# YaqiangCao/cLoops

Hardware: AMD Instinct MI355X
Metric: PETs clustered/sec (whole node) + wall-clock for mode-3 eps x minPts sweep (higher is better)
Workload: dtype int32; 1 GPU; synthetic-200M-23chr-mode3 (BASELINE.json configs[3]); variant=cDBSCAN2, pets=200000000, chromosomes=23, chained_cut=True, final_cut=3871, candidate_loops=3651369, parallelism=23 chromosomes LPT-sharded over 1 GPU(s)

## Files before the change

### cloops_amd/_lib.py

```python
import ctypes
import os

_HERE = os.path.dirname(os.path.abspath(__file__))
SO_PATH = os.path.join(_HERE, "libcloops_hip.so")

CL_OK = 0
CL_ERR_ARG = -1
CL_ERR_HIP = -2
CL_ERR_EMPTY = -3
CL_ERR_DOMAIN = -4
CL_ERR_GRID = -5
CL_ERR_NODEVICE = -6
CL_ERR_HASH = -7
CL_ERR_PARSE = -8

VARIANT_CDBSCAN1 = 1
VARIANT_CDBSCAN2 = 2
VARIANT_BLOCK = 3

CL_TRACK_WASHU, CL_TRACK_JUICE = 0, 1
CL_TRACK_NAME_MAX = 64
CL_CONV_HICPRO, CL_CONV_JUICER, CL_CONV_PAIRS = 0, 1, 2
CL_CONV_E_FIELDS, CL_CONV_E_INT, CL_CONV_E_RANGE, CL_CONV_E_LONG = 1, 2, 3, 4
CL_INGEST_TIMES = 6
CL_INGEST_BEDPE, CL_INGEST_PAIRS = 0, 1
DIST_LOGBINS = 3840
CL_KDE_MAX_GRID = 1024
CL_KDIS_KMAX = 64
CL_KDIS_BINS = 3968
CL_MAT_WMAX = 8192
CL_MAT_CELLS_MAX = 16777216
CL_BAL_BINS_MAX = 16777216
CL_EIG_MAX = 6
CL_EIG_BLOCK = 8
CL_EIG_BINS_MAX = 1048576


class ClBox(ctypes.Structure):
    _fields_ = [("min_x", ctypes.c_int32), ("max_x", ctypes.c_int32), ("min_y", ctypes.c_int32),
                ("max_y", ctypes.c_int32), ("count", ctypes.c_int32)]


class ClTiming(ctypes.Structure):
    _fields_ = [("ms_keys", ctypes.c_float), ("ms_sort", ctypes.c_float), ("ms_region", ctypes.c_float),
                ("ms_union", ctypes.c_float), ("ms_border", ctypes.c_float), ("ms_table", ctypes.c_float),
                ("ms_d2h", ctypes.c_float), ("ms_total", ctypes.c_float), ("n_in", ctypes.c_int64),
                ("n_strips", ctypes.c_int64), ("ms_bracket", ctypes.c_float), ("ms_band", ctypes.c_float),
                ("n_queried", ctypes.c_int64)]


class ClIngestName(ctypes.Structure):
    _fields_ = [("hash", ctypes.c_uint64), ("first", ctypes.c_uint32), ("off", ctypes.c_uint32), ("len", ctypes.c_uint32),
                ("pad", ctypes.c_uint32)]


class ClDsummary(ctypes.Structure):
    _fields_ = [("n_all", ctypes.c_int64 * 2), ("n_pos", ctypes.c_int64 * 2), ("sumx", ctypes.c_double * 2),
                ("sumxx", ctypes.c_double * 2), ("xshift", ctypes.c_double), ("loghist", ctypes.c_uint64 * DIST_LOGBINS),
                ("fine_lo", ctypes.c_int64), ("fine", ctypes.c_uint64 * 2048)]


_int, _i32, _u32, _i64, _vp, _cp = ctypes.c_int, ctypes.c_int32, ctypes.c_uint32, ctypes.c_int64, ctypes.c_void_p, ctypes.c_char_p
_i32p, _i64p, _u64p, _f32p, _vpp = (ctypes.POINTER(t) for t in (_i32, _i64, ctypes.c_uint64, ctypes.c_float, _vp))
_f64, _f64p = ctypes.c_double, ctypes.POINTER(ctypes.c_double)

PROTOTYPES = {
    "cl_last_error": (_cp, []),
    "cl_device_count": (_int, []),
    "cl_version": (_int, []),
    "cl_chrom_create": (_int, [_int, _vp, _vp, _vp, _i64, _int, _vpp]),
    "cl_chrom_destroy": (None, [_vp]),
    "cl_chrom_size": (_i64, [_vp]),
    "cl_chrom_subsample": (_int, [_vp, _vp, _i64, _vpp]),
    "cl_chrom_set_stream": (_int, [_vp, _vp]),
    "cl_chrom_drop_indexes": (_int, [_vp]),
    "cl_cluster": (_int, [_vp, _int, _i32, _i32, _i32, _vp, _i32p, _i32p]),
    "cl_cluster_weighted": (_int, [_vp, _i32, _i32, _i32, _i32, _vp, _i32p, _i32p]),
    "cl_cluster_async": (_int, [_vp, _int, _i32, _i32, _i32, _vp]),
    "cl_cluster_pairs_async": (_int, [_vp, _int, _i32, _i32, _i32, _vp, _i64]),
    "cl_cluster_rowmask_async": (_int, [_vp, _int, _i32, _i32, _i32, _vp, _i64]),
    "cl_cluster_step_async": (_int, [_vp, _int, _i32, _i32, _i32, _i32, _i64]),
    "cl_wait": (_int, [_vp, _i32p, _i32p]),
    "cl_step_result": (_int, [_vp, _i64p, _i64p, ctypes.POINTER(ClDsummary)]),
    "cl_set_pairs_defer": (None, [_vp, _int]),
    "cl_pairs_sync": (_int, [_vp]),
    "cl_last_n_labelled": (_i64, [_vp]),
    "cl_last_n_in": (_i64, [_vp]),
    "cl_last_region_mode": (_int, [_vp]),
    "cl_get_boxes": (_int, [_vp, _vp]),
    "cl_boxes_host": (_vp, [_vp]),
    "cl_labels_device": (_vp, [_vp]),
    "cl_neighbor_counts": (_int, [_vp, _i32, _i32, _vp]),
    "cl_dist_summary": (_int, [_vp, _i32, ctypes.POINTER(ClDsummary)]),
    "cl_dist_bin_hist": (_int, [_vp, _i32, _u32, _u32, _int, _u64p]),
    "cl_dist_collect": (_int, [_vp, _i32, _i64p, _i64p, _i64p]),
    "cl_dist_kde": (_int, [_vp, _int, _f64, _f64, _f64, _int, _f64p]),
    "cl_kde_array": (_int, [_int, _vp, _i64, _f64, _f64, _f64, _int, _f64p]),
    "cl_sig_counts": (_int, [_vp, _i32, _i32, _vp, _vp, _i64p]),
    "cl_quant_counts": (_int, [_vp, _i32, _i32, _vp, _vp, _i64p]),
    "cl_contact_hist": (_int, [_vp, _i32, _i32, _i64, _vp, _vp, _i64p, _i64p, _i64p, _i32p]),
    "cl_anchor_mask": (_int, [_vp, _i64, _vp, _vp, _vp, _i64p, _i64p]),
    "cl_agg_loops": (_int, [_vp, _i32, _i32, _i32, _i32, _i64, _vp, _vp, _vp, _vp, _vp, _i64p]),
    "cl_track_build": (_int, [_vp, _i32, _i64, _i64, _vp, _cp, _cp, _i64p, _i64p]),
    "cl_track_chunks": (_int, [_vp, _i64, _i64, _vp, _vp, _i64p]),
    "cl_track_render": (_int, [_vp, _i64, _vp, _i64, _i64p]),
    "cl_track_free": (_int, [_vp]),
    "cl_cov_build": (_int, [_vp, _i64, _i32, _i64, _i64, _i64p, ctypes.POINTER(_u32), _i64p, _i64p]),
    "cl_cov_runs": (_int, [_vp, _i64, _i64, _vp, _vp, _vp]),
    "cl_cov_text": (_int, [_vp, _cp, _i64, _i64, _i64p]),
    "cl_cov_chunks": (_int, [_vp, _i64, _i64, _vp, _vp, _i64p]),
    "cl_cov_render": (_int, [_vp, _i64, _vp, _i64, _i64p]),
    "cl_cov_free": (_int, [_vp]),
    "cl_peak_sort": (_int, [_vp, _i64, _i32, _i64p, _i64p, _i64p]),
    "cl_peak_call": (_int, [_vp, _i64, _i64, _i64p, _i64p, _i64p]),
    "cl_peak_get": (_int, [_vp, _i64, _i64, _vp, _vp, _vp, _vp]),
    "cl_peak_count": (_int, [_vp, _vp, _vp, _i64, _vp]),
    "cl_peak_summits": (_int, [_vp, _vp, _vp, _i64, _i64, _vp, _vp]),
    "cl_peak_free": (_int, [_vp]),
    "cl_dom_tracks": (_int, [_vp, _i64, _i64, _i64, _i64p, _i64p, _i64p]),
    "cl_dom_get": (_int, [_vp, _i64, _i64, _vp, _vp, _vp]),
    "cl_dom_count": (_int, [_vp, _vp, _vp, _i64, _vp, _vp, _vp]),
    "cl_dom_free": (_int, [_vp]),
    "cl_kdis_build": (_int, [_vp, _i64, _vp, _i32, _i64p]),
    "cl_kdis_get": (_int, [_vp, _i32, _i64, _i64, _vp, _vp, _vp]),
    "cl_kdis_hist": (_int, [_vp, _i32, _vp, _u64p, _u64p]),
    "cl_kdis_free": (_int, [_vp]),
    "cl_mat_window": (_int, [_vp, _i64, _i64, _i64, _i64, _i64, _i64, _i32, _vp, _i64p, _i64p]),
    "cl_mat_cells": (_int, [_vp, _i64, _i64, _i32, _i64p, _i64p, _i64p]),
    "cl_mat_cells_get": (_int, [_vp, _i64, _i64, _vp, _vp, _vp]),
    "cl_mat_v4c": (_int, [_vp, _i64, _i64, _i64, _i64, _i64, _i64, _vp, _i64p, _i64p, _i64p]),
    "cl_mat_free": (_int, [_vp]),
    "cl_bal_marginals": (_int, [_vp, _i32, _i64p, _i64p, _i64p]),
    "cl_bal_marginals_get": (_int, [_vp, _i64, _i64, _vp, _vp]),
    "cl_bal_iterate": (_int, [_vp, _vp, _i32, _f64, _i32p, _i32p, _f64p, _f64p]),
    "cl_bal_weights_get": (_int, [_vp, _i64, _i64, _vp]),
    "cl_bal_cells_get": (_int, [_vp, _i64, _i64, _vp]),
    "cl_bal_free": (_int, [_vp]),
    "cl_exp_diagonals": (_int, [_vp, _vp, _i32, _i64p, _i64p]),
    "cl_exp_diagonals_get": (_int, [_vp, _i64, _i64, _vp, _vp, _vp]),
    "cl_exp_set": (_int, [_vp, _vp, _i64]),
    "cl_exp_cells_get": (_int, [_vp, _i64, _i64, _vp]),
    "cl_exp_free": (_int, [_vp]),
    "cl_eig_build": (_int, [_vp, _f64, _i64, _i64p, _i64p]),
    "cl_eig_apply": (_int, [_vp, _vp, _i32, _vp]),
    "cl_eig_iterate": (_int, [_vp, _i32, _i32, _f64, _i32p, _i32p, _vp, _vp]),
    "cl_eig_vectors_get": (_int, [_vp, _i32, _i64, _i64, _vp]),
    "cl_eig_free": (_int, [_vp]),
    "cl_conv_create": (_int, [_int, _vp, _i32, _i64, _i64, _vpp]),
    "cl_conv_feed": (_int, [_vp, _vp, _i64, _i32, _i64p, _i64p, _i64p]),
    "cl_conv_render": (_int, [_vp, _vp, _i64, _i64p]),
    "cl_conv_error": (_int, [_vp, _i64p, _i32p]),
    "cl_conv_timing": (_int, [_vp, _f32p]),
    "cl_conv_destroy": (_int, [_vp]),
    "cl_ingest_create": (_int, [_int, _vp, _i64, _i64, _i32, _vpp]),
    "cl_ingest_set_format": (_int, [_vp, _i32, _i64]),
    "cl_ingest_feed": (_int, [_vp, _vp, _i64, _i64p, _i64p, _i64p]),
    "cl_ingest_error": (_int, [_vp, _i64p, _i32p]),
    "cl_ingest_headers": (_int, [_vp, _i64p]),
    "cl_ingest_names": (_int, [_vp, _vp, _i64, _i64p]),
    "cl_ingest_commit": (_int, [_vp, _i64, _i64, _vp, _vp, _vp, _vp, _i32, _vp, _i64, _i32, _vp, _i32p]),
    "cl_ingest_finish": (_int, [_vp, _vp, _i32, _i32, _vp, _i64p]),
    "cl_ingest_rows": (_int, [_vp, _i32, _vp, _vp, _i64]),
    "cl_ingest_chrom_arrays": (_int, [_vp, _i32, _i64p, _vpp, _vpp]),
    "cl_ingest_distances": (_int, [_vp, _vp, _i64]),
    "cl_ingest_timing": (_int, [_vp, _f32p]),
    "cl_ingest_destroy": (_int, [_vp]),
    "cl_cand_reset": (_int, [_vp]),
    "cl_cand_append": (_int, [_vp, _i32, _i64p, _i64p]),
    "cl_cand_finish": (_int, [_vp, _i32, _vp, _i64, _i64p]),
    "cl_cand_finish_device": (_int, [_vp, _i32, _vpp, _i64p]),
    "cl_set_table_export": (None, [_vp, _int]),
    "cl_set_device_labels": (None, [_vp, _int]),
    "cl_set_profiling": (None, [_vp, _int]),
    "cl_get_timing": (_int, [_vp, ctypes.POINTER(ClTiming)]),
    "cl_sweep_plan": (_int, [_vp, _i32p, _i32, _i32p, _i32]),
    "cl_set_layout_reuse": (None, [_vp, _int]),
    "cl_set_sort_index": (None, [_vp, _int]),
    "cl_set_count_reuse": (None, [_vp, _int]),
    "cl_set_count_floor": (None, [_vp, _i32]),
    "cl_set_count_thresholds": (None, [_vp, _i32p, _i32]),
    "cl_set_eps_list": (None, [_vp, _i32p, _i32]),
    "cl_set_traversal": (None, [_vp, _int]),
    "cl_stream_create": (_vp, [_int]),
    "cl_stream_destroy": (None, [_vp]),
    "cl_host_alloc": (_vp, [_i64]),
    "cl_host_free": (None, [_vp]),
    "cl_debug_arena_overcommit": (None, [_i64]),
}
SYMBOLS = list(PROTOTYPES)


def bind(lib, table):
    for name, (restype, argtypes) in table.items():
        fn = getattr(lib, name)
        fn.restype, fn.argtypes = restype, argtypes
    return lib


class CloopsHipError(RuntimeError):
    def __init__(self, code, msg):
        RuntimeError.__init__(self, "libcloops_hip error %d: %s" % (code, msg))
        self.code = code


_lib = None


def load():
    global _lib
    if _lib is not None:
        return _lib
    path = SO_PATH
    if os.environ.get("CLOOPS_DEVEL_LIB") == "1":
        path = SO_PATH.replace(".so", "_devel.so")
    if not os.path.exists(path):
        raise ImportError(
            "libcloops_hip.so is missing (%s). Build it with `python -m cloops_amd.build` "
            "(needs hipcc); there is no CPU fallback." % path)
    _lib = bind(ctypes.CDLL(path), PROTOTYPES)
    return _lib


def check(rc):
    if rc != CL_OK:
        msg = load().cl_last_error()
        raise CloopsHipError(rc, msg.decode() if msg else "")


def host_alloc(nbytes):
    p = load().cl_host_alloc(int(nbytes))
    if not p:
        raise MemoryError("no page-locked host memory of %d bytes" % nbytes)
    return p


def stream_create(device):
    s = load().cl_stream_create(int(device))
    if not s:
        raise CloopsHipError(CL_ERR_HIP, (load().cl_last_error() or b"").decode())
    return s
```

### cloops_amd/api.py

```python
import ctypes
import math
import os

import numpy as np

from . import _lib

VARIANTS = {"v1": _lib.VARIANT_CDBSCAN1, "cDBSCAN": _lib.VARIANT_CDBSCAN1, 1: 1,
            "v2": _lib.VARIANT_CDBSCAN2, "cDBSCAN2": _lib.VARIANT_CDBSCAN2, 2: 2,
            "block": _lib.VARIANT_BLOCK, "blockDBSCAN": _lib.VARIANT_BLOCK, 3: 3}

BOX_DTYPE = np.dtype([("min_x", "<i4"), ("max_x", "<i4"), ("min_y", "<i4"), ("max_y", "<i4"), ("count", "<i4")])


TRAVERSAL_OVERRIDE = int(os.environ["CLOOPS_TRAVERSAL"]) if os.environ.get("CLOOPS_TRAVERSAL", "") != "" else None


def device_count():
    return _lib.load().cl_device_count()


def _vp(a):
    return a.ctypes.data_as(ctypes.c_void_p)

# ... 28 lines not shown

    def _open(self, create, *args):
        self._lib = _lib.load()
        self._h = ctypes.c_void_p()
        _lib.check(getattr(self._lib, create)(*args, ctypes.byref(self._h)))

    def close(self):
        if getattr(self, "_h", None) is not None and self._h.value:
            getattr(self._lib, self._DESTROY)(self._h)
            self._h = ctypes.c_void_p()

    def __del__(self):
        try:
            self.close()
        except Exception:
            pass


class Chromosome(_Handle):
    _DESTROY = "cl_chrom_destroy"

    def __init__(self, X, Y, device=0, stream=None):
        X = _as_i32(X, "X")
        Y = _as_i32(Y, "Y")
        if X.shape != Y.shape:
            raise ValueError("X and Y differ in length")
        self._create(X.shape[0], device, "cl_chrom_create", int(device), ctypes.c_void_p(stream), X.ctypes.data_as(ctypes.c_void_p),
                     Y.ctypes.data_as(ctypes.c_void_p), int(X.shape[0]), 0)

    def _create(self, n, device, create, *args):
        self.n = int(n)
        self.device = device
        self._profiling = False
        self._pins = {}
        self._inflight = []
        self._enq = 0
        self._open(create, *args)
        if TRAVERSAL_OVERRIDE is not None:
            self._lib.cl_set_traversal(self._h, int(TRAVERSAL_OVERRIDE))

    @classmethod
    def from_device_pointers(cls, x_ptr, y_ptr, n, device=0, stream=None, keepalive=None):
        self = cls.__new__(cls)
        self._keepalive = keepalive
        self._create(n, device, "cl_chrom_create", int(device), ctypes.c_void_p(stream), ctypes.c_void_p(x_ptr), ctypes.c_void_p(y_ptr),
                     int(n), 1)
        return self

    def subsample(self, rows):
        rows = np.ascontiguousarray(rows, dtype=np.int64)
        new = Chromosome.__new__(Chromosome)
        new._create(rows.shape[0], self.device, "cl_chrom_subsample", self._h, rows.ctypes.data_as(ctypes.c_void_p), int(rows.shape[0]))
        return new

    def close(self):
        _Handle.close(self)
        pins, self._pins = getattr(self, "_pins", {}), {}
        for p, _ in pins.values():
            self._lib.cl_host_free(ctypes.c_void_p(p))

    def _pin(self, kind, slot, nbytes, shape=None):
        e = self._pins.get((kind, slot))
        if e is None:
            p = _lib.host_alloc(nbytes)
            view = None if shape is None else np.ctypeslib.as_array(ctypes.cast(p, ctypes.POINTER(ctypes.c_int32)), shape=shape)
            e = self._pins[kind, slot] = (p, view)
        return e

    def _pinned_labels(self, which=0):
        return self._pin("labels", which, max(4, self.n * 4), (self.n,))[1]

    def set_profiling(self, on=True):
        self._profiling = bool(on)
        self._lib.cl_set_profiling(self._h, 1 if on else 0)

    def set_device_labels(self, on=True):
        self._lib.cl_set_device_labels(self._h, 1 if on else 0)

    def set_table_export(self, on=True):
        if getattr(self, "_export", True) != bool(on):
            self._lib.cl_set_table_export(self._h, 1 if on else 0)
            self._export = bool(on)

    def cand_reset(self):
        _lib.check(self._lib.cl_cand_reset(self._h))

    def cand_append(self, step):
        ni, ns = ctypes.c_int64(0), ctypes.c_int64(0)
        _lib.check(self._lib.cl_cand_append(self._h, int(step), ctypes.byref(ni), ctypes.byref(ns)))
        return int(ni.value), int(ns.value)

    def step_async(self, variant, eps, minPts, cut, step, fine_lo=-1):
        _lib.check(self._lib.cl_cluster_step_async(self._h, VARIANTS[variant], int(eps), int(minPts), int(cut), int(step), int(fine_lo)))
        self._export = False
        self._inflight.append((None, False))
        self._enq += 1

    def step_result(self):
        ni, ns = ctypes.c_int64(0), ctypes.c_int64(0)
        st = _lib.ClDsummary()
        _lib.check(self._lib.cl_step_result(self._h, ctypes.byref(ni), ctypes.byref(ns), ctypes.byref(st)))
        return int(ni.value), int(ns.value), self._summary_dict(st)

    def cand_finish(self, final_cut, capacity):
        buf = getattr(self, "_cand_buf", None)
        if buf is None or len(buf) < capacity:
            buf = self._cand_buf = np.zeros((max(int(capacity) + int(capacity) // 4, 1), 4), dtype=np.int32)
        k = ctypes.c_int64(0)
        _lib.check(self._lib.cl_cand_finish(self._h, int(final_cut), buf.ctypes.data_as(ctypes.c_void_p), int(capacity), ctypes.byref(k)))
        return buf[: int(k.value)].copy()

    def cand_finish_device(self, final_cut):
        ptr, k = ctypes.c_void_p(), ctypes.c_int64(0)
        _lib.check(self._lib.cl_cand_finish_device(self._h, int(final_cut), ctypes.byref(ptr), ctypes.byref(k)))
        return (ptr.value or 0), int(k.value)

    def set_sort_index(self, mode=1):
        self._lib.cl_set_sort_index(self._h, int(mode))

    def set_count_reuse(self, on=True):
        self._lib.cl_set_count_reuse(self._h, 1 if on else 0)

    def sweep_plan(self, eps_list, min_pts_list):
        ev = sorted(set(int(e) for e in eps_list))
        mv = sorted(set(int(m) for m in min_pts_list))
        ea = (ctypes.c_int32 * max(len(ev), 1))(*ev)
        ma = (ctypes.c_int32 * max(len(mv), 1))(*mv)
        _lib.check(self._lib.cl_sweep_plan(self._h, ea, len(ev), ma, len(mv)))

    def drop_indexes(self):
        _lib.check(self._lib.cl_chrom_drop_indexes(self._h))

    def set_traversal(self, level=4):
        self._lib.cl_set_traversal(self._h, int(level))

    def set_count_floor(self, min_pts):
        self._lib.cl_set_count_floor(self._h, int(min_pts))

    def set_count_thresholds(self, min_pts_list):
        vals = [int(m) for m in min_pts_list]
        arr = (ctypes.c_int32 * max(1, len(vals)))(*vals)
        self._lib.cl_set_count_thresholds(self._h, arr, len(vals))

    def set_stream(self, stream):
        _lib.check(self._lib.cl_chrom_set_stream(self._h, ctypes.c_void_p(stream)))

    def set_eps_list(self, eps_list):
        vals = [int(e) for e in eps_list]
        arr = (ctypes.c_int32 * max(1, len(vals)))(*vals)
        self._lib.cl_set_eps_list(self._h, arr, len(vals))

    def last_region_mode(self):
        return int(self._lib.cl_last_region_mode(self._h))

    def set_layout_reuse(self, on=True):
        self._lib.cl_set_layout_reuse(self._h, 1 if on else 0)

    def timing(self):
        t = _lib.ClTiming()
        _lib.check(self._lib.cl_get_timing(self._h, ctypes.byref(t)))
        return {k: getattr(t, k) for k, _ in _lib.ClTiming._fields_}

    def _boxes(self, max_label, copy):
        k = max_label + 1
        if k <= 0:
            return np.zeros(0, dtype=BOX_DTYPE)
        ptr = self._lib.cl_boxes_host(self._h)
        if not ptr:
            raise _lib.CloopsHipError(_lib.CL_ERR_ARG, "the last run has no exported cluster table")
        view = np.ctypeslib.as_array(ctypes.cast(ptr, ctypes.POINTER(ctypes.c_int32)), shape=(k * 5,)).view(BOX_DTYPE)
        return view.copy() if copy else view

    def cluster_async(self, variant, eps, minPts, cut=0, want_labels=True, want_boxes=True):
        v = VARIANTS[variant]
        self.set_table_export(want_boxes)
        labels = self._pinned_labels(self._enq & 1) if want_labels else None
        _lib.check(self._lib.cl_cluster_async(self._h, v, int(eps), int(minPts), int(cut),
                                              labels.ctypes.data_as(ctypes.c_void_p) if want_labels else None))
        self._inflight.append((labels, bool(want_boxes)))
        self._enq += 1

    def cluster_pairs_async(self, variant, eps, minPts, cut=0, want_boxes=True):
        v = VARIANTS[variant]
        self.set_table_export(want_boxes)
        buf = self._pin("pairs", self._enq & 1, max(8, self.n * 8), (self.n, 2))[1]
        _lib.check(self._lib.cl_cluster_pairs_async(self._h, v, int(eps), int(minPts), int(cut), buf.ctypes.data_as(ctypes.c_void_p), self.n))
        self._inflight.append((buf, bool(want_boxes)))
        self._enq += 1

    def wait_pairs(self, copy=False, defer=False):
        buf, exported = self._inflight.pop(0)
        nc, ml = ctypes.c_int32(0), ctypes.c_int32(-1)
        self._lib.cl_set_pairs_defer(self._h, 1 if defer else 0)
        _lib.check(self._lib.cl_wait(self._h, ctypes.byref(nc), ctypes.byref(ml)))
        k = int(self._lib.cl_last_n_labelled(self._h))
        pairs = buf[:k].copy() if copy else buf[:k]
        boxes = self._boxes(ml.value, copy) if exported else None
        return ClusterResult(None, nc.value, ml.value, boxes, self.timing() if self._profiling else None), pairs

    def pairs_sync(self):
        _lib.check(self._lib.cl_pairs_sync(self._h))

    def cluster_rowmask_async(self, variant, eps, minPts, cut=0, want_boxes=True):
        v = VARIANTS[variant]
        self.set_table_export(want_boxes)
        p = self._pin("rowmask", self._enq & 1, 8 * ((self.n + 63) // 64) + 4 * max(self.n, 1))[0]
        _lib.check(self._lib.cl_cluster_rowmask_async(self._h, v, int(eps), int(minPts), int(cut), ctypes.c_void_p(p), max(self.n, 1)))
        self._inflight.append((p, bool(want_boxes)))
        self._enq += 1

    def wait_rowmask(self, copy=False, defer=False):
        p, exported = self._inflight.pop(0)
        nc, ml = ctypes.c_int32(0), ctypes.c_int32(-1)
        self._lib.cl_set_pairs_defer(self._h, 1 if defer else 0)
        _lib.check(self._lib.cl_wait(self._h, ctypes.byref(nc), ctypes.byref(ml)))
        k = int(self._lib.cl_last_n_labelled(self._h))
        nw = (self.n + 63) // 64
        mask = np.ctypeslib.as_array(ctypes.cast(p, ctypes.POINTER(ctypes.c_uint64)), shape=(nw,))
        labels = np.ctypeslib.as_array(ctypes.cast(p + 8 * nw, ctypes.POINTER(ctypes.c_int32)), shape=(max(k, 1),))[:k]
        if copy:
            mask, labels = mask.copy(), labels.copy()
        boxes = self._boxes(ml.value, copy) if exported else None
        return ClusterResult(None, nc.value, ml.value, boxes, self.timing() if self._profiling else None), mask, labels

    def rows_of_mask(self, mask):
        bits = np.unpackbits(np.ascontiguousarray(mask).view(np.uint8), bitorder="little")[: self.n]
        return np.flatnonzero(bits)

    def wait(self, copy=False):
        labels, exported = self._inflight.pop(0)
        nc = ctypes.c_int32(0)
        ml = ctypes.c_int32(-1)
        _lib.check(self._lib.cl_wait(self._h, ctypes.byref(nc), ctypes.byref(ml)))
        boxes = self._boxes(ml.value, copy) if exported else None
        if labels is not None and copy:
            labels = labels.copy()
        return ClusterResult(labels, nc.value, ml.value, boxes, self.timing() if self._profiling else None)

    def cluster(self, variant, eps, minPts, cut=0, want_labels=True, want_boxes=True, pinned=False):
        v = VARIANTS[variant]
        if self._inflight:
            raise RuntimeError("asynchronous runs in flight: call wait() first")
        self.set_table_export(True)
        if want_labels:
            labels = self._pinned_labels(0) if pinned else np.empty(self.n, dtype=np.int32)
        else:
            labels = None
        nc = ctypes.c_int32(0)
        ml = ctypes.c_int32(-1)
        lp = labels.ctypes.data_as(ctypes.c_void_p) if want_labels else None
        _lib.check(self._lib.cl_cluster(self._h, v, int(eps), int(minPts), int(cut), lp,
                                        ctypes.byref(nc), ctypes.byref(ml)))
        boxes = self._boxes(ml.value, copy=not pinned) if want_boxes else None
        return ClusterResult(labels, nc.value, ml.value, boxes, self.timing() if self._profiling else None)

    def cluster_weighted(self, eps, minPts, wx=1, wy=1):
        if self._inflight:
            raise RuntimeError("asynchronous runs in flight: call wait() first")
        self.set_table_export(True)
        labels = np.empty(self.n, dtype=np.int32)
        nc = ctypes.c_int32(0)
        ml = ctypes.c_int32(-1)
        _lib.check(self._lib.cl_cluster_weighted(self._h, int(eps), int(minPts), int(wx), int(wy),
                                                 labels.ctypes.data_as(ctypes.c_void_p), ctypes.byref(nc), ctypes.byref(ml)))
        return ClusterResult(labels, nc.value, ml.value, self._boxes(ml.value, copy=True), self.timing() if self._profiling else None)

    def last_n_in(self):
        return int(self._lib.cl_last_n_in(self._h))

    def dist_summary(self, cut=0):
        st = _lib.ClDsummary()
        _lib.check(self._lib.cl_dist_summary(self._h, int(cut), ctypes.byref(st)))
        return self._summary_dict(st)

    @staticmethod
    def _summary_dict(st):
        return {"n_all": [int(st.n_all[0]), int(st.n_all[1])], "n_pos": [int(st.n_pos[0]), int(st.n_pos[1])],
                "sumx": [float(st.sumx[0]), float(st.sumx[1])], "sumxx": [float(st.sumxx[0]), float(st.sumxx[1])],
                "xshift": float(st.xshift), "loghist": np.ctypeslib.as_array(st.loghist).astype(np.int64),
                "fine_lo": int(st.fine_lo), "fine": np.ctypeslib.as_array(st.fine).astype(np.int64) if st.fine_lo >= 0 else None}

    def dist_bin_hist(self, cut, lo, hi, shift):
        out = np.zeros(2048, dtype=np.uint64)
        _lib.check(self._lib.cl_dist_bin_hist(self._h, int(cut), int(lo), int(hi), int(shift),
                                              out.ctypes.data_as(ctypes.POINTER(ctypes.c_uint64))))
        return out.astype(np.int64)

    def dist_collect(self, cut=0):
        out = [(ctypes.c_int64 * 2)() for _ in range(3)]
        _lib.check(self._lib.cl_dist_collect(self._h, int(cut), *out))
        return {k: [int(a[0]), int(a[1])] for k, a in zip(("n_pos", "dmin", "dmax"), out)}

    def dist_kde(self, group, lo, step, inv_h, gridsize):
        out = np.zeros(max(int(gridsize), 1), dtype=np.float64)
        _lib.check(self._lib.cl_dist_kde(self._h, int(group), float(lo), float(step), float(inv_h), int(gridsize),
                                         out.ctypes.data_as(ctypes.POINTER(ctypes.c_double))))
        return out

    def sig_counts(self, windows, cut=0):
        w = np.ascontiguousarray(windows, dtype=np.int32).reshape(-1, 44)
        out = np.zeros((len(w), 144), dtype=np.int32)
        npets = ctypes.c_int64(0)
        _lib.check(self._lib.cl_sig_counts(self._h, int(cut), len(w), w.ctypes.data_as(ctypes.c_void_p),
                                           out.ctypes.data_as(ctypes.c_void_p), ctypes.byref(npets)))
        return out, int(npets.value)

# ... 552 lines not shown
```

### cloops_amd/csrc/cl_chrom.h

```cpp
#pragma once
#include "cl_common.h"
#include "cl_table.h"
#include "cl_prim.h"
#include "cl_textout.h"

#define BIGTPB 1024
#define AGG_H 512
__device__ __forceinline__ int agg_slot(int* keys, int key)
{
    unsigned h = ((unsigned)key * 2654435761u) >> 23;
    for (int probe = 0; probe < 24; ++probe) {
        const int old = atomicCAS(&keys[h], -1, key);
        if (old == -1 || old == key) return (int)h;
        h = (h + 1) & (AGG_H - 1);
    }
    return -1;
}
#define FLAT_PER 4
struct Stats { int amin, amax, vmin, vmax, xmin, xmax, ymin, ymax; };
__device__ __forceinline__ int je_minus(const int* __restrict__ cstart, int j) { return cstart[j + 1] - cstart[j]; }
static inline int bits_for(unsigned v) { int b = 0; while (v) { ++b; v >>= 1; } return b; }


#define CL_FINE_KMAX 8
#define K7_BLOCKS 2048
#define K7_STEP_BLOCKS 256
#define K7_STEP_THREADS 1024
#define K7_LOGBINS 3840
__device__ __forceinline__ int k7_logbin(unsigned d)
{
    const int e = 31 - __clz((int)d);
    const unsigned m = e >= 7 ? ((d >> (e - 7)) & 127u) : ((d << (7 - e)) & 127u);
    return e * 128 + (int)m;
}
#define K7_FINE 2048
#define K7_XSHIFT 11.0
#define CAND_BLOCK 2048

struct K7Src {
    int sorted;
    int n; int M; int v0;
    const int* dM;
    const int* X; const int* Y; const int* labels;
    const int* sv; const int* slab;
    const int* dh;
};

struct K7Part { double sx[2]; double sxx[2]; long long n_all[2]; long long n_pos[2]; };

struct RunRequest {
    int variant = CL_VARIANT_CDBSCAN1, eps = 0, minPts = 0, cut = 0;
    int32_t* labels_out = nullptr;
    int2* pairs_out = nullptr;
    long long pairs_cap = 0;
    void* mask_out = nullptr;
    long long mask_cap = 0;
    int step = -1;
    long long fine_lo = -1;
    int wx = 0, wy = 0;
};

struct cl_chrom {
    long long tmp_n = -1;
    DevBuf arena;
    int device = 0;
    hipStream_t stream = nullptr;
    bool own_stream = false;
    int64_t n = 0;
    int *d_x = nullptr, *d_y = nullptr;
    bool own_xy = false;
    Stats st{};
    DevBuf keys_in, keys_out, vals_in, vals_out, sort_tmp, scan_tmp;
    DevBuf qb_key, qb_val;
    int qindex_layout = -1;
    struct Fine {
        DevBuf q, sp, row, strip;
        int w = 0;
        int valid_w = 0, layout = -1;
        GridParams g;
        void invalidate() { valid_w = 0; layout = -1; }
    } fine;
    int sort_index_mode = 0;
    long long n_sorts = 0;
    DevBuf sv, sa, strip, cnt, parent, root, head, headidx, cellfirst, compkey, ncore, bsize, owner, state;
    DevBuf flag, rankscan, ulist, lo, hi, recs, counters, chainflag, chainhead, usize, b_cstart, b_ckey, b_nb, b_cx, b_cy, tile_s0;
    int* h_pinned = nullptr;
    struct StripPlan { int layout, eps, maxlen; };
    std::vector<StripPlan> plans;
    struct Run {
        u32* srow = nullptr;
        int *sv = nullptr, *sa = nullptr, *strip = nullptr, *tile = nullptr;
        int* cnt = nullptr;
        WordSrc ws{};
        int init_nclr = 0;
        int level = 0;
        const int* dM = nullptr;
        int m = 0;
        bool m_exact = false;
        bool rows = true;
        bool l4_make_base = false;
        bool l4_cut = false;
        bool l4_band = false;
        bool k2_make = false;
        const int* k_total = nullptr;
        bool hdr_packed = false;
    } run;
    struct Base {
        DevBuf q, sp, row, strip, tile, key;
        bool valid = false; int layout = -1, eps = 0;
        bool key_valid = false;
        void invalidate() { valid = false; key_valid = false; }
    } base;
    DevBuf sel_tmp;
    struct Counts {
        bool valid = false;
        bool cut_on_base = false;
        bool base_space = false;
        int layout = -1, eps = 0, thr = 0 , cap = 0;
        u32 tmask[4] = {0, 0, 0, 0};
        DevBuf cnt, pre, poff, dpre, D, blen;
        void invalidate() { valid = false; }
    } rc;
    bool reuse_counts = true;
    int count_floor = 0;
    u32 count_tmask[4] = {0, 0, 0, 0};
    DevBuf blk_tmp;
    DevBuf rootlist, cflag8;
    DevBuf l_mask, l_rank, l_blk, l_cstrip, l_wpos, l_wenc, l_dist, l_aux;
    DevBuf l_tab, l_fix;
    bool pairs_defer = false, pairs_copy_pending = false;
    bool fuse_chains = true;
    bool l_sup_dirty = false;
    GridParams dbg_g{}; int dbg_nm = 0;
    int traversal = 4;
    int last_k2_mode = 0;
    std::vector<long long> dcum;
    DevBuf dhist;
    long long n_neg = 0;
    bool reuse_layout = true;
    struct Slot {
        DevBuf labels, table;
        bool pending = false;
        int n_strips = 0;
        hipEvent_t ev_done = nullptr, ev_copied = nullptr;
        hipEvent_t ev[10]{};
        bool band_timed = false;
        long long n_queried = 0;
        int* h_hdr = nullptr;
        cl_box* h_boxes = nullptr;
        size_t h_boxes_cap = 0;
        int32_t* labels_out = nullptr;
        DevBuf slab;
        DevBuf pairs;
        int2* pairs_host = nullptr;
        long long pairs_host_cap = 0;
        void* mask_host = nullptr;
        long long mask_host_cap = 0;
        bool exported = true;
        bool step_valid = false;
        bool host_written = false;
        bool wait_done = false;
        long long fine_lo = -1;
        int kmax = 0;
        DevBuf d_step;
        char* h_step = nullptr;
        bool rows_valid = false;
        bool sorted_src = false;
        const int* k7_sv = nullptr;
        const int* k7_lcnt = nullptr;
        int k7_v0 = 0;
    } slot[2];
    bool device_labels = true;
    bool export_table = true;
    struct Cand { DevBuf box, step, keep, out; long long n = 0, cap = 0; } cand;
    DevBuf hdr;
    DevBuf k7_cls, k7_parts;
    struct Kde {
        DevBuf ent, sorted, ctr, tmp, part;
        int run = -1;
        long long cap = 0, cnt[2] = {0, 0};
    } kde;
    struct Sig { DevBuf tx, ty, tmp, sorttmp, m, win, out; bool ready = false; int cut = 0; } sig;
    struct Fp { DevBuf small, keys, sorted, tmp, pairs; } fp;
    struct Anchor { DevBuf s, e, dir, mask, wsum; } an;
    struct Agg {
        DevBuf kin, vin, sx, sy, tmp, m, cx, cy, lkin, lkout, lvin, order, ltmp, sum, stats, mats;
        bool ready = false; int cut = 0, kept = 0;
    } ag;
    struct Track {
        DevBuf tcnt, toff, row, keys, sorted, tmp, ids, names;
        TextOut txt;
        struct State {
            bool built = false, ids = false;
            int kind = 0, la = 0, lb = 0, gbits = 0;
            long long cut = 0, ext = 0;
        } st;
    } tk;
    struct Cov {
        DevBuf kin, key, tmp, dcur, dprev, xr, flag, scan, ctr, start, end, depth, name;
        TextOut txt;
        struct State {
            bool built = false, text = false;
            int la = 0;
            long long R = 0, num = 0, den = 0;
        } st;
    } cv;
    struct Peak {
        DevBuf kin, key, tmp, lo, hi, flag, C, head, H, a, b, start, end, np, nc, ctr, ivs, ive, best, opos, ocnt;
        struct State {
            bool sorted = false, called = false;
            int base = 0;
            long long m = 0, P = 0;
        } st;
    } pk;
    struct Dom {
        DevBuf diff, trk, tmp, rng, ivs, ive, cnt;
        struct State {
            bool ready = false;
            int cut = 0, res = 0, w = 0;
            int pmin = 0, pmax = 0;
            long long bmin = 0, n_bins = 0, n_kept = 0;
        } st;
    } dm;
    struct Kdis {
        DevBuf x, y, d, hist;
        struct State {
            bool ready = false;
            int cut = 0, n_k = 0;
            int ks[8] = {0, 0, 0, 0, 0, 0, 0, 0};
            long long n_kept = 0;
        } st;
    } kd;
    struct Mat {
        DevBuf out, ctr, key, sorted, tmp, flag, scan, start, bx, by, cnt;
        struct State {
            bool ready = false;
            long long n_cells = 0, n_kept = 0, max_count = 0;
            int res = 0; bool fold = false;
        } st;
    } mx;
    struct Bal {
        DevBuf kin, kout, vin, vout, tmp, tby, tbx, tcnt, sum, nnz, valid, w, s, icar, dcar, part, rec, out;
        struct State {
            bool ready = false, iterated = false;
            int ignore_diags = 0;
            long long b0 = 0, nb = 0, n_used = 0, n_cells = 0;
        } st;
    } bl;
    struct Exp {
        DevBuf valid, w, mask, kin, kout, vin, vout, tmp, dk, dx, dc, car, ctr, pairs, cnt, val, exp, out;
        struct State {
            bool ready = false, expected = false;
            int balanced = 0;
            long long nd = 0, n_used = 0;
        } st;
    } ex;
    struct Eig {
        DevBuf val, rows, pl, tot, ctr, q, part, sm, vec, io, ax;
        struct State {
            bool built = false, iterated = false;
            double clip = 0.0;
            long long dmax = 0, n_valid = 0, n_in = 0;
            int n_eigs = 0;
        } st;
    } eg;
    bool k7_classified = false;
    hipStream_t copy_stream = nullptr, aux_stream = nullptr;
    int copy_mode = 0;
    hipStream_t shared_copy = nullptr;
    int enq = 0, deq = 0;
    int cur = 0;
    int last_slot = -1;
    int last_K = 0;
    bool have_result = false;
    long long refused_labelled = -1;
    bool profiling = false;
    cl_timing timing{};
    bool ev_ready = false;
    float ev_bracket_ms = 0.f;
};


#define LAUNCH(kernel, nthreads, ...) \
    hipLaunchKernelGGL(kernel, dim3(nblocks(nthreads)), dim3(TPB), 0, c->stream, __VA_ARGS__)

static inline void run_begin(cl_chrom* c) { c->run = cl_chrom::Run(); }

struct RunGuard {
    cl_chrom* c; bool armed = true;
    explicit RunGuard(cl_chrom* cc) : c(cc) {}
    ~RunGuard()
    {
        if (!armed) return;
        c->rc.invalidate();
        c->l_sup_dirty = true;
        if (c->counters.p) (void)hipMemsetAsync(c->counters.as<int>() + CTR_TICKET_A, 0, 8, c->stream);
        (void)hipGetLastError();
    }
};

static inline bool range_ok(int64_t first, int64_t count, int64_t size)
{
    return first >= 0 && count >= 0 && first <= size && count <= size - first;
}
struct CopyOut { void* dst; const void* src; size_t bytes; };
static inline int read_back(cl_chrom* c, const char* who, std::initializer_list<CopyOut> parts)
{
    hipError_t e = hipSuccess;
    for (const CopyOut& p : parts)
        if (e == hipSuccess) e = hipMemcpyAsync(p.dst, p.src, p.bytes, hipMemcpyDeviceToHost, c->stream);
    const hipError_t e2 = hipStreamSynchronize(c->stream);
    if (e != hipSuccess || e2 != hipSuccess) return fail_at(CL_ERR_HIP, who, "copy", hipGetErrorString(e != hipSuccess ? e : e2));
    return CL_OK;
}

int ensure_workspace(cl_chrom* c, int S);
int ensure_events(cl_chrom* c);
void ev_record(cl_chrom* c, int k);
int ensure_cand_capacity(cl_chrom* c, long long need);
Table make_table_slot(cl_chrom* c, int slot);
Table make_table(cl_chrom* c);
const int* k7_hist_for(cl_chrom* c, int cut);
int finish_enqueue(cl_chrom* c, const RunRequest& req, int n_strips, const int* d_M);
static inline void track_release(cl_chrom* c) { c->tk = cl_chrom::Track(); }
static inline void cov_release(cl_chrom* c) { c->cv = cl_chrom::Cov(); }
static inline void peak_release(cl_chrom* c) { c->pk = cl_chrom::Peak(); }
static inline void dom_release(cl_chrom* c) { c->dm = cl_chrom::Dom(); }
static inline void kdis_release(cl_chrom* c) { c->kd = cl_chrom::Kdis(); }
static inline void eig_release(cl_chrom* c) { c->eg = cl_chrom::Eig(); }
static inline void exp_release(cl_chrom* c) { eig_release(c); c->ex = cl_chrom::Exp(); }
static inline void bal_release(cl_chrom* c) { exp_release(c); c->bl = cl_chrom::Bal(); }
static inline void mat_release(cl_chrom* c) { c->mx = cl_chrom::Mat(); bal_release(c); }
static inline int unit_free(cl_chrom* c, const char* who, void (*release)(cl_chrom*))
{
    if (!c) return fail(CL_ERR_ARG, "null chromosome handle");
    if (c->enq != c->deq) return fail(CL_ERR_ARG, who, "asynchronous runs still in flight");
    HIP_TRY(hipSetDevice(c->device));
    HIP_TRY(hipStreamSynchronize(c->stream));
    release(c);
    return CL_OK;
}
int run_block(cl_chrom* c, const RunRequest& req);
int run_weighted(cl_chrom* c, const RunRequest& req);

__global__ void k_init_table(Table t, const int* __restrict__ rankscan, int n);
__global__ void k_init_arrays(int n, int* __restrict__ parent, int* __restrict__ compkey, int* __restrict__ ncore,
                              int* __restrict__ bsize, int* __restrict__ usize, int* __restrict__ cellfirst,
                              int* __restrict__ flag, int* __restrict__ state, int* __restrict__ counters);
__global__ void k_strip_table(const u64* __restrict__ skeys, int n, int S, int shift, int* __restrict__ strip_start);
__global__ void k_root_labels(GridParams g, const int* __restrict__ strip_start, const int* __restrict__ root,
                              const int* __restrict__ compkey, const int* __restrict__ ncore, const int* __restrict__ bsize,
                              const int* __restrict__ state, const int* __restrict__ rankscan, int* __restrict__ rlabel);
__global__ void k_rank_flags(GridParams g, const int* __restrict__ strip_start, const int* __restrict__ root,
                             const int* __restrict__ compkey, const int* __restrict__ state, int* __restrict__ flag);
__global__ void __launch_bounds__(BIGTPB)
k_flatten(GridParams g, const int* __restrict__ strip_start, const int* __restrict__ cnt,
          const int* __restrict__ chainid, int* parent, const u32* __restrict__ srow,
          const int* __restrict__ head, const int* __restrict__ cellfirst,
          int* __restrict__ root, int* __restrict__ compkey, int* __restrict__ ncore,
          int* __restrict__ rootlist , int* __restrict__ counters);

struct Rec { int pt; int r[4]; };
#define OWNER_CONTESTED 0x40000000
__device__ __forceinline__ int owner_root(int o) { return o < 0 ? -1 : (o & (OWNER_CONTESTED - 1)); }

struct ListRun {
    int npos;
    const int* pstrip;
    const int* lcnt;
    const unsigned long long* cmask; const unsigned long long* wmask;
    const int* cgrank; const int* wgrank;
    int2* cpair; int* cpos; int* ckey; int2* wpair; int* wpos; int* wenc; int* cstrip;
};
int lists_build(cl_chrom* c, const GridParams& g, int nm, ListRun* out);
int lists_build_base(cl_chrom* c, const GridParams& g, int nm, ListRun* out);
int lists_base_keys(cl_chrom* c, const GridParams& g);
int lists_words_to_base(cl_chrom* c, const GridParams& g);
int lists_union_flatten(cl_chrom* c, const GridParams& g, int nm, const ListRun& L);
int lists_scatter_root(cl_chrom* c, int nm, const ListRun& L);
int lists_border(cl_chrom* c, const GridParams& g, int nm, const ListRun& L);
int lists_emit_records(cl_chrom* c, const GridParams& g, int nm, const ListRun& L);
int lists_scatter_owner(cl_chrom* c, int nm, const ListRun& L);
int lists_final(cl_chrom* c, const RunRequest& req, const GridParams& g, int nm, const ListRun& L, bool rows, int* pair_count);
int lists_rowmask(cl_chrom* c, const RunRequest& req, int* total);

__global__ void __launch_bounds__(256)
k_step_classify_count(const int* __restrict__ dK, Table t, signed char* __restrict__ cls, int* __restrict__ bcount, int nb,
                      unsigned long long* __restrict__ zero, int nzero);
__global__ void __launch_bounds__(256)
k_cand_append(const int* __restrict__ dK, const signed char* __restrict__ cls, Table t, const int* __restrict__ boff ,
              const int* __restrict__ bcount, int base, int step, int cap, int4* __restrict__ cbox, int* __restrict__ cstep);
__global__ void __launch_bounds__(TPB)
k7_summary(K7Src s, int cut, const signed char* __restrict__ cls, K7Part* __restrict__ parts, unsigned long long* __restrict__ loghist,
           unsigned fine_lo, unsigned long long* __restrict__ fine );
__global__ void __launch_bounds__(256)
k7_reduce_parts(const K7Part* __restrict__ parts, int nparts, K7Part* out, const int* __restrict__ bcount , int nb,
                long long* totals, const volatile unsigned long long* dev_step , int step_words,
                unsigned long long* __restrict__ host_step, const int* __restrict__ dev_hdr, int* __restrict__ host_hdr);

#define SIG_W 11
struct SigWin { int lo[2 * SIG_W]; int hi[2 * SIG_W]; };

__device__ __forceinline__ int k8_lb(const u64* __restrict__ t, int m, long long v)
{
    const u64 target = v <= -(1ll << 30) ? 0ull : ((u64)(u32)(v + (1 << 30)) << 32);
    int lo = 0, hi = m;
    while (lo < hi) { int mid = (lo + hi) >> 1; if (t[mid] < target) lo = mid + 1; else hi = mid; }
    return lo;
}
__device__ __forceinline__ int k8_ub(const u64* __restrict__ t, int m, long long v)
{
    return k8_lb(t, m, v + 1);
}
int sig_tables(cl_chrom* c, int cut);
int agg_table(cl_chrom* c, int cut);

__device__ __forceinline__ int k19_lb_wave(const u32* __restrict__ sx, int m, u32 t)
{
    const int lane = threadIdx.x & 63;
    int lo = 0, len = m;
    while (len > 0) {
        const int step = len / 65 + 1;
        const long long pos = (long long)lo + (long long)(lane + 1) * step - 1;
        const bool below = pos < (long long)lo + len && sx[pos] < t;
        const int nb = __popcll(__ballot(below));
        const long long nlo = (long long)lo + (long long)nb * step;
        const long long end = (long long)lo + len, nhi = nlo + step - 1 < end ? nlo + step - 1 : end;
        lo = (int)nlo; len = (int)(nhi - nlo);
    }
    return lo;
}


struct K12Div { u32 magic; int sh1, sh2; };
__device__ __forceinline__ u32 k12_div(const K12Div& d, u32 v)
{
    const u32 t1 = __umulhi(d.magic, v);
    return (t1 + ((v - t1) >> d.sh1)) >> d.sh2;
}
// ... 22 lines not shown
```

### cloops_amd/csrc/cloops_hip.hip

```cpp
#include <map>
#include <mutex>
#include "cl_chrom.h"
#include "cl_band.h"

thread_local std::string g_err;



extern "C" const char* cl_last_error(void) { return g_err.c_str(); }
extern "C" int cl_version(void) { return CL_VERSION_NUM; }

extern "C" void* cl_host_alloc(int64_t bytes)
{
    void* p = nullptr;
    if (bytes <= 0) return nullptr;
    if (hipHostMalloc(&p, (size_t)bytes, hipHostMallocDefault) != hipSuccess) { fail(CL_ERR_HIP, "hipHostMalloc"); return nullptr; }
    return p;
}
extern "C" void cl_host_free(void* p) { if (p) (void)hipHostFree(p); }

static std::mutex g_pair_mu;
static std::map<hipStream_t, hipStream_t> g_copy_of;
extern "C" void* cl_stream_create(int device)
{
// ... 59 lines not shown
        amin = min(amin, __shfl_down(amin, off)); amax = max(amax, __shfl_down(amax, off));
        vmin = min(vmin, __shfl_down(vmin, off)); vmax = max(vmax, __shfl_down(vmax, off));
        xmin = min(xmin, __shfl_down(xmin, off)); xmax = max(xmax, __shfl_down(xmax, off));
        ymin = min(ymin, __shfl_down(ymin, off)); ymax = max(ymax, __shfl_down(ymax, off));
    }
    __shared__ int red[TPB / 64][8];
    const int wv = threadIdx.x >> 6;
    if ((threadIdx.x & 63) == 0) {
        red[wv][0] = amin; red[wv][1] = amax; red[wv][2] = vmin; red[wv][3] = vmax;
        red[wv][4] = xmin; red[wv][5] = xmax; red[wv][6] = ymin; red[wv][7] = ymax;
    }
    __syncthreads();
    if (threadIdx.x < 8) {
        const bool is_min = (threadIdx.x & 1) == 0;
        int v = red[0][threadIdx.x];
        for (int w = 1; w < TPB / 64; ++w) v = is_min ? min(v, red[w][threadIdx.x]) : max(v, red[w][threadIdx.x]);
        int* dst = &out->amin + threadIdx.x;
        if (is_min) atomicMin(dst, v); else atomicMax(dst, v);
    }
}

#define DCUM_BINS 65537
#define DH_LOCAL 8192
__global__ void __launch_bounds__(TPB)
k_dhist(const int* __restrict__ X, const int* __restrict__ Y, long long n, int* __restrict__ hist)
{
    __shared__ int lh[DH_LOCAL];
    for (int k = threadIdx.x; k < DH_LOCAL; k += blockDim.x) lh[k] = 0;
    __syncthreads();
    for (long long i = (long long)blockIdx.x * blockDim.x + threadIdx.x; i < n; i += (long long)gridDim.x * blockDim.x) {
        const long long d = (long long)Y[i] - X[i];
        if (d >= 0 && d < DH_LOCAL) atomicAdd(&lh[(int)d], 1);
        else if (d < DCUM_BINS - 1) atomicAdd(&hist[d < 0 ? DCUM_BINS : (int)d], 1);
    }
    __syncthreads();
    for (int k = threadIdx.x; k < DH_LOCAL; k += blockDim.x) { const int v = lh[k]; if (v) atomicAdd(&hist[k], v); }
}

__global__ void k_make_keys(const int* __restrict__ X, const int* __restrict__ Y, int n, GridParams g,
                            u64* __restrict__ keys, u32* __restrict__ vals)
{
    int r = blockIdx.x * blockDim.x + threadIdx.x;
    if (r >= n) return;
    int x = X[r], y = Y[r];
    int a = y - x;
    bool valid = (g.cut <= 0) || (a >= g.cut);
    int v = x + y;
    int prel = (g.swap ? v : a) - g.A0;
    u32 qrel = (u32)((g.swap ? a : v) - g.V0);
    const int sabs = div_eps(g, prel);
    const u32 rem = (u32)(prel - sabs * g.eps);
    const int sh = g.qbits + g.rbits;
    u64 key = valid ? (((u64)(u32)(sabs - g.s0) << sh) | ((u64)qrel << g.rbits) | rem) : ((u64)(u32)g.S << sh);
    keys[r] = key;
    vals[r] = (u32)r;
}

__global__ void k_decode_sorted(int n, GridParams g, const u64* __restrict__ skeys,
                                int* __restrict__ sv, int* __restrict__ sa, int* __restrict__ tile_s0,
                                const u32* __restrict__ rows_in, u32* __restrict__ rows_out)
{
    int i = blockIdx.x * blockDim.x + threadIdx.x;
    if (i >= n) return;
    const u64 k = skeys[i];
    if (rows_out) rows_out[i] = rows_in[i];
    const int sh = g.qbits + g.rbits;
    const int strip = (int)(k >> sh);
    if ((i & 255) == 0) tile_s0[i >> 8] = min(strip, g.S);
    if (strip >= g.S) { sv[i] = INT_MAX; sa[i] = g.S << g.rbits; return; }
    sv[i] = (int)((k >> g.rbits) & ((1ull << g.qbits) - 1ull));
    sa[i] = (strip << g.rbits) | (int)(k & ((1ull << g.rbits) - 1ull));
}

__global__ void k_make_qkeys(const int* __restrict__ X, const int* __restrict__ Y, int n, GridParams g,
                             u32* __restrict__ keyq, u64* __restrict__ val)
{
    int r = blockIdx.x * blockDim.x + threadIdx.x;
    if (r >= n) return;
    const int x = X[r], y = Y[r];
    const int a = y - x, v = x + y;
    const u32 prel = (u32)((g.swap ? v : a) - g.A0);
    keyq[r] = (u32)((g.swap ? a : v) - g.V0);
    val[r] = ((u64)prel << 32) | (u32)r;
}
__global__ void k_make_spkeys(int n, GridParams g, const u32* __restrict__ keyq, const u64* __restrict__ valq,
                              u32* __restrict__ key, u64* __restrict__ val)
{
    int i = blockIdx.x * blockDim.x + threadIdx.x;
    if (i >= n) return;
    const u32 q = keyq[i];
    const u64 pv = valq[i];
    const int prel = (int)(pv >> 32);
    const int a = (g.swap ? (int)q + g.V0 : prel + g.A0);
    const bool valid = (g.cut <= 0) || (a >= g.cut);
    const int sabs = div_eps(g, prel);
    const u32 rem = (u32)(prel - sabs * g.eps);
    key[i] = valid ? (((u32)(sabs - g.s0) << g.rbits) | rem) : ((u32)g.S << g.rbits);
    val[i] = ((u64)q << 32) | (u32)pv;
}
__global__ void k_decode_sp(int n, GridParams g, const u32* __restrict__ skey, const u64* __restrict__ sval,
                            int* __restrict__ sv, int* __restrict__ sa, int* __restrict__ tile_s0, u32* __restrict__ rows_out)
{
    int i = blockIdx.x * blockDim.x + threadIdx.x;
    if (i >= n) return;
    const u32 k = skey[i];
    const u64 v = sval[i];
    rows_out[i] = (u32)v;
    const int strip = (int)(k >> g.rbits);
    if ((i & 255) == 0) tile_s0[i >> 8] = min(strip, g.S);
    if (strip >= g.S) { sv[i] = INT_MAX; sa[i] = g.S << g.rbits; return; }
    sv[i] = (int)(v >> 32);
    sa[i] = (int)k;
}
struct SpKeyOfIndex {
    const u32* keyq; const u64* valq; GridParams g;
    __device__ __forceinline__ u32 operator()(int i) const
    {
        const int prel = (int)(valq[i] >> 32);
        const int sabs = div_eps(g, prel);
        return ((u32)(sabs - g.s0) << g.rbits) | (u32)(prel - sabs * g.eps);
    }
};
struct SpValOfIndex {
    const u32* keyq; const u64* valq;
    __device__ __forceinline__ u64 operator()(int i) const { return ((u64)keyq[i] << 32) | (u32)valq[i]; }
};
struct SplitRef {
    int* q; u32* row;
    __device__ __forceinline__ const SplitRef& operator=(u64 v) const { *q = (int)(v >> 32); *row = (u32)v; return *this; }
    __device__ __forceinline__ operator u64() const { return ((u64)(u32)*q << 32) | *row; }
    __device__ __forceinline__ const SplitRef& operator=(const SplitRef& o) const { *q = *o.q; *row = *o.row; return *this; }
};
struct SplitOut {
    using iterator_category = std::random_access_iterator_tag;
    using value_type = u64;
    using difference_type = std::ptrdiff_t;
    using pointer = void;
    using reference = SplitRef;
    int* q; u32* row;
    __host__ __device__ __forceinline__ SplitRef operator*() const { return SplitRef{q, row}; }
    __host__ __device__ __forceinline__ SplitRef operator[](difference_type i) const { return SplitRef{q + i, row + i}; }
    __host__ __device__ __forceinline__ SplitOut operator+(difference_type d) const { return SplitOut{q + d, row + d}; }
    __host__ __device__ __forceinline__ SplitOut operator-(difference_type d) const { return SplitOut{q - d, row - d}; }
    __host__ __device__ __forceinline__ difference_type operator-(const SplitOut& o) const { return q - o.q; }
    __host__ __device__ __forceinline__ SplitOut& operator+=(difference_type d) { q += d; row += d; return *this; }
    __host__ __device__ __forceinline__ SplitOut& operator-=(difference_type d) { q -= d; row -= d; return *this; }
    __host__ __device__ __forceinline__ SplitOut& operator++() { ++q; ++row; return *this; }
    __host__ __device__ __forceinline__ SplitOut operator++(int) { SplitOut t = *this; ++q; ++row; return t; }
    __host__ __device__ __forceinline__ bool operator==(const SplitOut& o) const { return q == o.q; }
    __host__ __device__ __forceinline__ bool operator!=(const SplitOut& o) const { return q != o.q; }
    __host__ __device__ __forceinline__ bool operator<(const SplitOut& o) const { return q < o.q; }
};

__global__ void k_strips_from_fine(int S, int s0, int k, int F, int f0, const int* __restrict__ fstrip, int n, int* __restrict__ strip_start)
{
    const int s = blockIdx.x * blockDim.x + threadIdx.x;
    if (s > S + 1) return;
    const long long f = (long long)k * ((long long)s + s0) - f0;
    strip_start[s] = s >= S ? n : fstrip[(int)std::min<long long>(std::max<long long>(f, 0), F)];
}
#define LFF_T 1024
#define LFF_CAP 4096
#define LFF_NST 127
#define LFF_PAD 512
__global__ void __launch_bounds__(256)
k_layout_from_fine(int n, GridParams g, GridParams gf, int k, unsigned kmagic, int qb, const int* __restrict__ fq, const int* __restrict__ fsp, const u32* __restrict__ frow,
                   const int* __restrict__ fstrip, int* __restrict__ dq, int* __restrict__ dsp, u32* __restrict__ drow, int* __restrict__ dtile)
{
    __shared__ int lq[LFF_CAP + LFF_PAD];
    const int t0 = blockIdx.x * LFF_T, t1 = min(n, t0 + LFF_T);
    if (t0 >= n) return;
    constexpr int E = LFF_T / 256;
    int q[E], spf[E], fbase[E], r[E], dst[E];
    u32 row[E];
    bool in[E];
#pragma unroll
    for (int e = 0; e < E; ++e) {
        const int i = t0 + e * 256 + (int)threadIdx.x;
        in[e] = i < t1;
        const int ic = in[e] ? i : t0;
        q[e] = fq[ic]; row[e] = frow[ic]; spf[e] = fsp[ic];
    }
    const int sb_first = (((fsp[t0] >> gf.rbits) + gf.s0) / k) * k - gf.s0, sb_last = (((fsp[t1 - 1] >> gf.rbits) + gf.s0) / k) * k - gf.s0;
    const int f_first = max(sb_first, 0), f_end = min(sb_last + k, gf.S);
    const int a = fstrip[f_first], b = fstrip[f_end];
    const bool staged = b - a <= LFF_CAP;
    const bool keyed = staged && qb > 0 && (f_end - f_first) < (1 << (32 - qb)) - 1;
    __shared__ int lst[LFF_NST + 1];
    const bool slice = f_end - f_first <= LFF_NST;
    if (slice) for (int j = threadIdx.x; j <= f_end - f_first; j += 256) lst[j] = fstrip[f_first + j];
    if (keyed) {
        for (int j0 = 0; j0 < b - a; j0 += 8 * 256) {
            int vq[8], vs[8];
#pragma unroll
            for (int u = 0; u < 8; ++u) { const int j = j0 + u * 256 + (int)threadIdx.x; const bool ok = j < b - a; vq[u] = ok ? fq[a + j] : 0; vs[u] = ok ? fsp[a + j] : 0; }
#pragma unroll
            for (int u = 0; u < 8; ++u) { const int j = j0 + u * 256 + (int)threadIdx.x; if (j < b - a) lq[j] = (int)((unsigned)vq[u] | ((unsigned)((vs[u] >> gf.rbits) - f_first) << qb)); }
        }
        for (int j = threadIdx.x; j < LFF_PAD; j += 256) lq[b - a + j] = -1;
    } else if (staged) for (int j = threadIdx.x; j < b - a; j += 256) lq[j] = fq[a + j];
    __syncthreads();
    auto fst = [&](int f) { return slice ? lst[f - f_first] : fstrip[f]; };
#pragma unroll
    for (int e = 0; e < E; ++e) {
        const int i = t0 + e * 256 + (int)threadIdx.x;
        const int f = spf[e] >> gf.rbits;
        const int fabs = f + gf.s0;
        const int sabs = k == 1 ? fabs : (int)__umulhi((unsigned)fabs, kmagic);
        r[e] = fabs - sabs * k;
        fbase[e] = sabs * k - gf.s0;
        dst[e] = in[e] ? fst(max(fbase[e], 0)) + (i - fst(f)) : 0;
    }
#ifdef CLOOPS_DEVEL
    const int kk_abl = (g.dbg2 & (1 << 12)) ? 0 : k;
#else
    const int kk_abl = k;
#endif
    for (int rr = 0; rr < kk_abl; ++rr) {
        int lo[E], len[E], key[E], pos[E];
        int nmax = 0;
#pragma unroll
        for (int e = 0; e < E; ++e) {
            const int ff = fbase[e] + rr;
            const bool on = in[e] && rr != r[e] && ff >= 0 && ff < gf.S;
            lo[e] = on ? fst(ff) : 0; len[e] = on ? fst(ff + 1) - lo[e] : 0;
            key[e] = q[e] + (rr < r[e] ? 1 : 0);
            pos[e] = 0;
            nmax = max(nmax, len[e]);
        }
        nmax = wave_max_i(nmax);
        int nsteps = 0;
        while ((1 << nsteps) <= nmax) ++nsteps;
        if (keyed && (1 << nsteps) <= LFF_PAD) {
            unsigned tk[E];
            int p4[E];
#pragma unroll
            for (int e = 0; e < E; ++e) {
                const bool on = len[e] > 0;
                tk[e] = on ? ((unsigned)key[e] | ((unsigned)(fbase[e] + rr - f_first) << qb)) : 0u;
                p4[e] = on ? (lo[e] - a) * 4 : 0;
            }
            const char* lb = reinterpret_cast<const char*>(lq);
#define LFF_STEP(ST) _Pragma("unroll") for (int e = 0; e < E; ++e) { const unsigned v = *reinterpret_cast<const unsigned*>(lb + p4[e] + ((ST) - 1) * 4); p4[e] = v < tk[e] ? p4[e] + (ST) * 4 : p4[e]; }
            switch (nsteps) {
            case 9: LFF_STEP(256)
            case 8: LFF_STEP(128)
            case 7: LFF_STEP(64)
            case 6: LFF_STEP(32)
            case 5: LFF_STEP(16)
            case 4: LFF_STEP(8)
            case 3: LFF_STEP(4)
            case 2: LFF_STEP(2)
            case 1: LFF_STEP(1)
            default: break;
            }
#undef LFF_STEP
#pragma unroll
            for (int e = 0; e < E; ++e) pos[e] = len[e] > 0 ? (p4[e] >> 2) - (lo[e] - a) : 0;
        } else if (staged && !keyed) {
            for (int step = nsteps > 0 ? 1 << (nsteps - 1) : 0; step >= 1; step >>= 1) {
#pragma unroll
                for (int e = 0; e < E; ++e) {
                    const int p = pos[e] + step - 1;
                    const int v = lq[lo[e] - a + min(p, max(len[e] - 1, 0))];
                    pos[e] = (p < len[e] && v < key[e]) ? pos[e] + step : pos[e];
                }
            }
        } else {
            for (int step = nsteps > 0 ? 1 << (nsteps - 1) : 0; step >= 1; step >>= 1) {
#pragma unroll
                for (int e = 0; e < E; ++e) {
                    const int p = pos[e] + step - 1;
                    const int v = fq[lo[e] + min(p, max(len[e] - 1, 0))];
                    pos[e] = (p < len[e] && v < key[e]) ? pos[e] + step : pos[e];
                }
            }
        }
#pragma unroll
        for (int e = 0; e < E; ++e) dst[e] += pos[e];
    }
#pragma unroll
    for (int e = 0; e < E; ++e) {
        if (!in[e]) continue;
#ifdef CLOOPS_DEVEL
        if (g.dbg2 & (1 << 13)) { if (dst[e] == 0x7fffffff) dq[0] = 1; continue; }
#endif
        const int sabs = k == 1 ? fbase[e] + gf.s0 : (int)__umulhi((unsigned)(fbase[e] + gf.s0), kmagic);
        dq[dst[e]] = q[e];
        dsp[dst[e]] = ((sabs - g.s0) << g.rbits) | (r[e] * gf.eps + (spf[e] & (gf.peps - 1)));
        drow[dst[e]] = row[e];
        if ((dst[e] & 255) == 0) dtile[dst[e] >> 8] = min(sabs - g.s0, g.S);
    }
}

__global__ void k_strip_table32(const u32* __restrict__ skeys, int n, int S, int shift, int* __restrict__ strip_start, int* __restrict__ tile_s0 = nullptr)
{
    int t = blockIdx.x * blockDim.x + threadIdx.x;
    if (tile_s0) for (int u = t; u < (n + 255) / 256; u += gridDim.x * blockDim.x) tile_s0[u] = min((int)(skeys[u * 256] >> shift), S);
    if (t > S + 1) return;
    if (t == S + 1) { strip_start[t] = n; return; }
    const u32 target = (u32)t << shift;
    int lo = 0, hi = n;
    while (lo < hi) {
        int mid = (int)(((unsigned)lo + (unsigned)hi) >> 1);
        if (skeys[mid] < target) lo = mid + 1; else hi = mid;
    }
    strip_start[t] = lo;
}

__global__ void k_strip_table(const u64* __restrict__ skeys, int n, int S, int shift, int* __restrict__ strip_start)
{
    int t = blockIdx.x * blockDim.x + threadIdx.x;
    if (t > S + 1) return;
    if (t == S + 1) { strip_start[t] = n; return; }
    u64 target = (u64)(u32)t << shift;
    int lo = 0, hi = n;
    while (lo < hi) {
        int mid = (int)(((unsigned)lo + (unsigned)hi) >> 1);
        if (skeys[mid] < target) lo = mid + 1; else hi = mid;
    }
    strip_start[t] = lo;
}

#define HS_TPB 256
#define HS_HALO 256
#define HS_WIN (HS_TPB + 2 * HS_HALO)
#define HS_LMAX 256
enum { CTR_MAXLEN = 48, CTR_M = 49 };

__global__ void k_strip_hist(const int* __restrict__ X, const int* __restrict__ Y, int n, GridParams g, int* __restrict__ hist)
{
    int r = blockIdx.x * blockDim.x + threadIdx.x;
    if (r >= n) return;
    const int x = X[r], y = Y[r];
    const int prel = (g.swap ? x + y : y - x) - g.A0;
    atomicAdd(&hist[div_eps(g, prel) - g.s0], 1);
}
__global__ void k_max_int(const int* __restrict__ v, int n, int* __restrict__ out)
{
    __shared__ int red[TPB / 64];
    int m = 0;
    for (int i = blockIdx.x * blockDim.x + threadIdx.x; i < n; i += gridDim.x * blockDim.x) m = max(m, v[i]);
    for (int o = 32; o > 0; o >>= 1) m = max(m, __shfl_down(m, o));
    if ((threadIdx.x & 63) == 0) red[threadIdx.x >> 6] = m;
    __syncthreads();
    if (threadIdx.x == 0) {
        for (int w = 1; w < TPB / 64; ++w) m = max(m, red[w]);
        atomicMax(out, m);
    }
}

__global__ void __launch_bounds__(HS_TPB)
k_strip_sort(int n, GridParams g, const u64* __restrict__ keys, const u32* __restrict__ rows,
             const int* __restrict__ strip_start, int* __restrict__ sv, int* __restrict__ sa, u32* __restrict__ srow,
             int* __restrict__ tile_s0, int* __restrict__ counters)
{
    __shared__ u32 lq[HS_WIN];
    const int t0 = blockIdx.x * HS_TPB, base = t0 - HS_HALO;
    const u64 qmask = (1ull << g.qbits) - 1ull;
    u64 kk[3];
#pragma unroll
    for (int u = 0; u < 3; ++u) {
        const int gi = base + (int)threadIdx.x + u * HS_TPB;
        kk[u] = (gi >= 0 && gi < n) ? keys[gi] : 0ull;
// ... 1241 lines not shown
    flag[compkey[i]] = 1;
}


__global__ void k_root_labels(GridParams g, const int* __restrict__ strip_start, const int* __restrict__ root,
                              const int* __restrict__ compkey, const int* __restrict__ ncore, const int* __restrict__ bsize,
                              const int* __restrict__ state, const int* __restrict__ rankscan, int* __restrict__ rlabel)
{
    const int M = strip_start[g.S];
    int i = blockIdx.x * blockDim.x + threadIdx.x;
    if (i >= M) return;
    if (root[i] != i) return;
    const bool keep = (g.variant == CL_VARIANT_CDBSCAN2) ? (state[i] != ST_DEAD)
                                                         : (ncore[i] + bsize[i] >= g.minPts);
    rlabel[i] = keep ? rankscan[compkey[i]] : -1;
}

__global__ void k_init_table(Table t, const int* __restrict__ rankscan, int n)
{
    const int K = rankscan[n];
    int k = blockIdx.x * blockDim.x + threadIdx.x;
    if (k >= K) return;
    t.count[k] = 0; t.minx[k] = INT_MAX; t.maxx[k] = INT_MIN; t.miny[k] = INT_MAX; t.maxy[k] = INT_MIN;
}

__global__ void __launch_bounds__(256)
k_rank_scan(int nw, const unsigned* __restrict__ bits, int* __restrict__ wloc, int* __restrict__ bsum, int* __restrict__ wboff, int* ticket)
{
    __shared__ int red[4];
    const int w0 = (blockIdx.x * 256 + threadIdx.x) * 4;
    int c[4];
#pragma unroll
    for (int k = 0; k < 4; ++k) c[k] = w0 + k < nw ? __popc(bits[w0 + k]) : 0;
    const int mine = c[0] + c[1] + c[2] + c[3];
    int tot;
    int run = wg256_inclusive_scan(mine, red, tot) - mine;
#pragma unroll
    for (int k = 0; k < 4; ++k) { if (w0 + k < nw) wloc[w0 + k] = run; run += c[k]; }
    scan_tail_last_block(tot, bsum, wboff, ticket, red);
}

__global__ void k_root_labels_bits_l(GridParams g, const int* __restrict__ rootlist, const int* __restrict__ counters,
                                     const int* __restrict__ compkey, const int* __restrict__ ncore, const int* __restrict__ bsize,
                                     const int* __restrict__ state, const unsigned* __restrict__ bits,
                                     const int* __restrict__ wloc, const int* __restrict__ wboff ,
                                     int* __restrict__ rlabel, Table t, int nblkw, int* __restrict__ hdr, const int* __restrict__ d_M)
{
    const int ids = wboff[nblkw];
    if (blockIdx.x == 0 && threadIdx.x == 0) {
        hdr[0] = ids; hdr[1] = counters[CTR_OVERFLOW]; hdr[2] = d_M[0]; hdr[3] = 0; hdr[4] = -1; hdr[5] = 0; hdr[6] = 0;
    }
    const int K = counters[CTR_NROOT];
    for (int k = blockIdx.x * blockDim.x + threadIdx.x; k < K; k += gridDim.x * blockDim.x) {
        const int i = rootlist[k];
        const bool keep = (g.variant == CL_VARIANT_CDBSCAN2) ? (state[i] != ST_DEAD)
                                                             : (ncore[i] + bsize[i] >= g.minPts);
        const int key = compkey[i];
        const int w = key >> 5;
        rlabel[i] = keep ? wloc[w] + wboff[w >> 10] + __popc(bits[w] & ((1u << (key & 31)) - 1u)) : -1;
    }
    for (int k = blockIdx.x * blockDim.x + threadIdx.x; k < ids; k += gridDim.x * blockDim.x) {
        t.count[k] = 0; t.minx[k] = INT_MAX; t.maxx[k] = INT_MIN; t.miny[k] = INT_MAX; t.maxy[k] = INT_MIN;
    }
}

#define FINAL_CHUNKS 4
__global__ void __launch_bounds__(BIGTPB)
k_final_labels(GridParams g, const int* __restrict__ strip_start, const int* __restrict__ sv,
               const int* __restrict__ sa, const u32* __restrict__ srow, const int* __restrict__ owner,
               const int* __restrict__ rlabel, int* __restrict__ labels, int* __restrict__ slab, Table t)
{
    __shared__ TableLds h;
    table_lds_init(h);
    const int M = strip_start[g.S];
    int idx[FINAL_CHUNKS], own[FINAL_CHUNKS], lab[FINAL_CHUNKS], x[FINAL_CHUNKS], y[FINAL_CHUNKS];
#pragma unroll
    for (int ch = 0; ch < FINAL_CHUNKS; ++ch) {
        idx[ch] = (blockIdx.x * FINAL_CHUNKS + ch) * BIGTPB + threadIdx.x;
        own[ch] = idx[ch] < M ? owner_root(owner[idx[ch]]) : -1;
    }
#pragma unroll
    for (int ch = 0; ch < FINAL_CHUNKS; ++ch) lab[ch] = own[ch] >= 0 ? rlabel[own[ch]] : -1;
#ifdef CLOOPS_DEVEL
    if (g.dbg2 & 16) { if (lab[0] == 123456789) slab[0] = 0; return; }
#endif
#pragma unroll
    for (int ch = 0; ch < FINAL_CHUNKS; ++ch) {
        const int i = idx[ch];
        x[ch] = 0; y[ch] = 0;
        if (i < M) {
            slab[i] = lab[ch];
            if (labels) labels[srow[i]] = lab[ch];
            if (lab[ch] >= 0) {
                const int spv = sa[i];
                int pp = ((spv >> g.rbits) + g.s0) * g.eps + (spv & (g.peps - 1)) + g.A0, qq = sv[i] + g.V0;
                int a = g.swap ? qq : pp, v = g.swap ? pp : qq;
                x[ch] = (v - a) / 2; y[ch] = (v + a) / 2;
            }
        }
    }
#ifdef CLOOPS_DEVEL
    if (g.dbg2 & 32) return;
#endif
#pragma unroll
    for (int ch = 0; ch < FINAL_CHUNKS; ++ch) table_accumulate(t, h, lab[ch], x[ch], y[ch]);
    table_flush(t, h);
}


int ensure_cand_capacity(cl_chrom* c, long long need)
{
    if (need <= c->cand.cap) return CL_OK;
    const long long cap = std::max<long long>(std::max<long long>(need, 2 * c->cand.cap), 1 << 20);
    DevBuf nb, ns;
    int rc;
    if ((rc = nb.ensure((size_t)cap * 16)) || (rc = ns.ensure((size_t)cap * 4))) return rc;
    if (c->cand.n > 0) {
        HIP_TRY(hipMemcpyAsync(nb.p, c->cand.box.p, (size_t)c->cand.n * 16, hipMemcpyDeviceToDevice, c->stream));
        HIP_TRY(hipMemcpyAsync(ns.p, c->cand.step.p, (size_t)c->cand.n * 4, hipMemcpyDeviceToDevice, c->stream));
        HIP_TRY(hipStreamSynchronize(c->stream));
    }
    c->cand.box = std::move(nb); c->cand.step = std::move(ns);
    c->cand.cap = cap;
    return CL_OK;
}

static void free_chrom(cl_chrom* c)
{
    if (!c) return;
    (void)hipSetDevice(c->device);
    std::vector<void*> dev, pinned{c->h_pinned};
    std::vector<hipEvent_t> events;
    const hipStream_t streams[3] = {c->copy_stream, c->aux_stream, c->own_stream ? c->stream : nullptr};
    if (c->own_xy) dev = {c->d_x, c->d_y};
    for (auto& sl : c->slot) {
        pinned.push_back(sl.h_boxes);
        events.insert(events.end(), {sl.ev_done, sl.ev_copied});
        if (c->ev_ready) events.insert(events.end(), std::begin(sl.ev), std::end(sl.ev));
    }
    delete c;
    for (void* p : dev) if (p) (void)hipFree(p);
    for (void* p : pinned) if (p) (void)hipHostFree(p);
    for (hipEvent_t e : events) if (e) (void)hipEventDestroy(e);
    for (hipStream_t st : streams) if (st) (void)hipStreamDestroy(st);
}

extern "C" void cl_chrom_destroy(cl_chrom* c) { free_chrom(c); }
extern "C" int64_t cl_chrom_size(const cl_chrom* c) { return c ? c->n : -1; }
extern "C" void cl_set_profiling(cl_chrom* c, int enabled) { if (c) c->profiling = enabled != 0; }
extern "C" void cl_set_layout_reuse(cl_chrom* c, int enabled) { if (c) { c->reuse_layout = enabled != 0; c->base.invalidate(); c->rc.invalidate(); } }
extern "C" void cl_set_count_reuse(cl_chrom* c, int enabled) { if (c) { c->reuse_counts = enabled != 0; c->rc.invalidate(); } }
extern "C" void cl_set_traversal(cl_chrom* c, int level) { if (c) { c->traversal = level < 0 ? 0 : (level > 4 ? 4 : level); c->rc.invalidate(); } }
extern "C" int cl_last_region_mode(const cl_chrom* c) { return c ? c->last_k2_mode : 0; }
extern "C" int cl_chrom_drop_indexes(cl_chrom* c)
{
    if (!c) return fail(CL_ERR_ARG, "null chromosome handle");
    if (c->slot[0].pending || c->slot[1].pending) return fail(CL_ERR_ARG, "cl_chrom_drop_indexes: a run is in flight");
    c->qindex_layout = -1;
    c->fine.invalidate();
    c->base.invalidate();
    c->rc.invalidate();
    return CL_OK;
}
extern "C" void cl_set_count_floor(cl_chrom* c, int32_t min_pts)
{
    if (!c) return;
    c->count_floor = min_pts > 0 ? min_pts : 0;
    for (auto& w : c->count_tmask) w = 0;
}
extern "C" int cl_chrom_set_stream(cl_chrom* c, void* stream)
{
    if (!c || !stream || c->own_stream) return fail(CL_ERR_ARG, "cl_chrom_set_stream: needs a handle on a caller's stream and a stream");
    if (c->slot[0].pending || c->slot[1].pending) return fail(CL_ERR_ARG, "cl_chrom_set_stream: a run is in flight");
    if ((hipStream_t)stream == c->stream) return CL_OK;
    HIP_TRY(hipSetDevice(c->device));
    HIP_TRY(hipStreamSynchronize(c->stream));
    c->stream = (hipStream_t)stream;
    c->shared_copy = nullptr;
    c->copy_mode = library_made_stream(c->stream) ? 2 : 1;
    return CL_OK;
}

extern "C" void cl_set_eps_list(cl_chrom* c, const int32_t* eps, int32_t n)
{
    if (!c) return;
    long long gcd = 0, mx = 0;
    int distinct = 0;
    for (int k = 0; eps && k < n; ++k) {
        if (eps[k] <= 0) { gcd = 0; distinct = 0; break; }
        bool seen = false;
        for (int j = 0; j < k; ++j) seen |= eps[j] == eps[k];
        distinct += seen ? 0 : 1;
        long long a = eps[k], b = gcd;
        while (b) { const long long t = a % b; a = b; b = t; }
        gcd = a; mx = std::max<long long>(mx, eps[k]);
    }
    c->fine.w = (distinct >= 2 && gcd >= 16 && mx / gcd <= CL_FINE_KMAX) ? (int)gcd : 0;
}

extern "C" void cl_set_count_thresholds(cl_chrom* c, const int32_t* min_pts, int32_t n)
{
    if (!c) return;
    c->count_floor = 0;
    for (auto& w : c->count_tmask) w = 0;
    for (int k = 0; min_pts && k < n; ++k)
        if (min_pts[k] >= 2 && min_pts[k] <= 128) c->count_tmask[(min_pts[k] - 1) >> 5] |= 1u << ((min_pts[k] - 1) & 31);
}
extern "C" void cl_set_sort_index(cl_chrom* c, int mode) { if (c) c->sort_index_mode = mode > 0 ? 1 : (mode < 0 ? -1 : 0); }
extern "C" int cl_sweep_plan(cl_chrom* c, const int32_t* eps, int32_t n_eps, const int32_t* min_pts, int32_t n_min_pts)
{
    if (!c) return fail(CL_ERR_ARG, "null chromosome handle");
    if (n_eps < 0 || n_min_pts < 0 || (n_eps > 0 && !eps) || (n_min_pts > 0 && !min_pts)) return fail(CL_ERR_ARG, "cl_sweep_plan: bad lists");
    for (int k = 0; k < n_eps; ++k) if (eps[k] <= 0) return fail(CL_ERR_ARG, "cl_sweep_plan: eps must be positive");
    for (int k = 0; k < n_min_pts; ++k) if (min_pts[k] <= 0) return fail(CL_ERR_ARG, "cl_sweep_plan: minPts must be positive");
    if (c->slot[0].pending || c->slot[1].pending) return fail(CL_ERR_ARG, "cl_sweep_plan: a run is in flight");
    cl_set_count_thresholds(c, min_pts, n_min_pts);
    int distinct = 0;
    for (int k = 0; k < n_eps; ++k) { bool seen = false; for (int j = 0; j < k; ++j) seen |= eps[j] == eps[k]; distinct += seen ? 0 : 1; }
    if (distinct > 1) { cl_set_sort_index(c, 1); cl_set_eps_list(c, eps, n_eps); }
    else cl_set_eps_list(c, nullptr, 0);
    return CL_OK;
}
extern "C" int cl_get_timing(const cl_chrom* c, cl_timing* out)
{
    if (!c || !out) return fail(CL_ERR_ARG, "cl_get_timing: null argument");
    *out = c->timing;
    return CL_OK;
}
extern "C" const int32_t* cl_labels_device(const cl_chrom* c)
{
    return (c && c->last_slot >= 0 && c->slot[c->last_slot].rows_valid) ? (const int32_t*)c->slot[c->last_slot].labels.p : nullptr;
}
extern "C" void cl_set_device_labels(cl_chrom* c, int enabled) { if (c) c->device_labels = enabled != 0; }
extern "C" void cl_set_table_export(cl_chrom* c, int enabled) { if (c) c->export_table = enabled != 0; }


__global__ void k_init_pads(int* __restrict__ svbuf, int* __restrict__ sabuf, long long n)
{
    const int k = blockIdx.x * blockDim.x + threadIdx.x;
    if (k >= 2 * SORT_PAD) return;
    const bool left = k < SORT_PAD;
    const long long idx = left ? k : (long long)SORT_PAD + n + (k - SORT_PAD);
    svbuf[idx] = left ? 0 : INT_MAX;
    sabuf[idx] = left ? INT_MIN : INT_MAX;
}

static int reserve_workspace(cl_chrom* c);
#ifdef CLOOPS_DEVEL
static int skip_mask() { static const int m = getenv("CLOOPS_SKIP") ? atoi(getenv("CLOOPS_SKIP")) : 0; return m; }
#define SKIP(bit) (skip_mask() & (bit))
#else
#define SKIP(bit) 0
#endif

extern "C" int cl_chrom_create(int device, void* stream, const int32_t* x, const int32_t* y, int64_t n,
                               int on_device, cl_chrom** out)
{
    if (!out) return fail(CL_ERR_ARG, "cl_chrom_create: out is null");
    *out = nullptr;
    if (n < 0 || n >= (1LL << 31) - 1024) return fail(CL_ERR_ARG, "cl_chrom_create: n out of range (0 .. 2^31 - 1024)");
    if (n > 0 && (!x || !y)) return fail(CL_ERR_ARG, "cl_chrom_create: null coordinates");
    int ndev = 0;
    if (hipGetDeviceCount(&ndev) != hipSuccess || ndev <= 0) return fail(CL_ERR_NODEVICE, "no HIP device visible");
    if (device < 0 || device >= ndev) return fail(CL_ERR_ARG, "cl_chrom_create: bad device index");
    HIP_TRY(hipSetDevice(device));
    cl_chrom* c = new cl_chrom();
    c->device = device;
    c->n = n;
    int rc = CL_OK;
    do {
        if (stream) c->stream = (hipStream_t)stream;
        else {
            if (hipStreamCreateWithFlags(&c->stream, hipStreamNonBlocking) != hipSuccess) { rc = fail(CL_ERR_HIP, "hipStreamCreate"); break; }
            c->own_stream = true;
        }
        const size_t step_bytes = ((16 + sizeof(K7Part) + K7_LOGBINS * 8 + K7_FINE * 8 + 255) / 256) * 256;
        if (hipHostMalloc((void**)&c->h_pinned, 4096 + 2 * (256 + step_bytes), hipHostMallocDefault) != hipSuccess) { rc = fail(CL_ERR_HIP, "hipHostMalloc"); break; }
        {
            int prio_lo = 0, prio_hi = 0;
            (void)hipDeviceGetStreamPriorityRange(&prio_lo, &prio_hi);
            c->copy_mode = c->own_stream ? 0 : 1;
            if (!c->own_stream) {
                if (library_made_stream(c->stream)) c->copy_mode = 2;
#ifdef CLOOPS_DEVEL
                if (getenv("CLOOPS_COPY_IN_STREAM")) c->copy_mode = 1;
#endif
            }
            if (hipStreamCreateWithPriority(&c->copy_stream, hipStreamNonBlocking, prio_hi) != hipSuccess ||
                hipStreamCreateWithPriority(&c->aux_stream, hipStreamNonBlocking, prio_hi) != hipSuccess) { rc = fail(CL_ERR_HIP, "hipStreamCreate(copy)"); break; }
        }
        bool okslots = true;
        int kslot = 0;
        for (auto& sl : c->slot) {
            okslots = okslots && hipEventCreateWithFlags(&sl.ev_done, hipEventDisableTiming) == hipSuccess;
            okslots = okslots && hipEventCreateWithFlags(&sl.ev_copied, hipEventDisableTiming) == hipSuccess;
            char* base = (char*)c->h_pinned + 4096 + (size_t)kslot * (256 + step_bytes);
            sl.h_hdr = (int*)base;
            sl.h_step = base + 256;
            ++kslot;
        }
        if (!okslots) { rc = fail(CL_ERR_HIP, "result slot setup"); break; }
        if (on_device) { c->d_x = (int*)x; c->d_y = (int*)y; }
        else if (n > 0) {
            c->own_xy = true;
            if (hipMalloc((void**)&c->d_x, n * 4) != hipSuccess || hipMalloc((void**)&c->d_y, n * 4) != hipSuccess) { rc = fail(CL_ERR_HIP, "hipMalloc X/Y"); break; }
            if (hipMemcpyAsync(c->d_x, x, n * 4, hipMemcpyHostToDevice, c->stream) != hipSuccess ||
                hipMemcpyAsync(c->d_y, y, n * 4, hipMemcpyHostToDevice, c->stream) != hipSuccess) { rc = fail(CL_ERR_HIP, "hipMemcpy X/Y"); break; }
        }
        if (n > 0) {
            if ((rc = c->counters.ensure(256))) break;
            if (hipMemsetAsync(c->counters.p, 0, 256, c->stream) != hipSuccess) { rc = fail(CL_ERR_HIP, "counters memset"); break; }
            Stats init = {INT_MAX, INT_MIN, INT_MAX, INT_MIN, INT_MAX, INT_MIN, INT_MAX, INT_MIN};
            Stats* hs = (Stats*)c->h_pinned;
            *hs = init;
            if (hipMemcpyAsync(c->counters.p, hs, sizeof(Stats), hipMemcpyHostToDevice, c->stream) != hipSuccess) { rc = fail(CL_ERR_HIP, "stats init"); break; }
            int grid = std::min(nblocks(n), 512);
            hipLaunchKernelGGL(k_stats, dim3(grid), dim3(TPB), 0, c->stream, c->d_x, c->d_y, (long long)n, (Stats*)c->counters.p);
            if (hipMemcpyAsync(hs, c->counters.p, sizeof(Stats), hipMemcpyDeviceToHost, c->stream) != hipSuccess) { rc = fail(CL_ERR_HIP, "stats readback"); break; }
            hipError_t e = hipStreamSynchronize(c->stream);
            if (e != hipSuccess) { rc = fail(CL_ERR_HIP, "stats sync", hipGetErrorString(e)); break; }
            c->st = *hs;
            {
                if ((rc = c->dhist.ensure((size_t)(DCUM_BINS + 1) * 4))) break;
                std::vector<int> hh(DCUM_BINS + 1);
                if (hipMemsetAsync(c->dhist.p, 0, (size_t)(DCUM_BINS + 1) * 4, c->stream) != hipSuccess) { rc = fail(CL_ERR_HIP, "dhist memset"); break; }
                hipLaunchKernelGGL(k_dhist, dim3(std::min(nblocks(n), 2048)), dim3(TPB), 0, c->stream, c->d_x, c->d_y, (long long)n, c->dhist.as<int>());
                if (hipMemcpyAsync(hh.data(), c->dhist.p, (size_t)(DCUM_BINS + 1) * 4, hipMemcpyDeviceToHost, c->stream) != hipSuccess ||
                    hipStreamSynchronize(c->stream) != hipSuccess) { rc = fail(CL_ERR_HIP, "dhist readback"); break; }
                c->dcum.assign(DCUM_BINS, 0);
                c->n_neg = hh[DCUM_BINS];
                long long run = c->n_neg;
                for (int k = 0; k < DCUM_BINS; ++k) { c->dcum[k] = run; run += hh[k]; }
            }
            const int LIM = 1 << 29;
            if (c->st.xmin <= -LIM || c->st.xmax >= LIM || c->st.ymin <= -LIM || c->st.ymax >= LIM) {
                rc = fail(CL_ERR_DOMAIN, "coordinates must satisfy |X|,|Y| < 2^29");
                break;
            }
        }
    } while (0);
    if (rc != CL_OK) { std::string keep = g_err; free_chrom(c); g_err = keep; return rc; }
    (void)reserve_workspace(c);
    *out = c;
    return CL_OK;
}

__global__ void k_gather_rows(const int* __restrict__ X, const int* __restrict__ Y, const int* __restrict__ rows, int m,
                              int* __restrict__ xo, int* __restrict__ yo)
{
    const int i = blockIdx.x * blockDim.x + threadIdx.x;
    if (i >= m) return;
    const int r = rows[i];
    xo[i] = X[r]; yo[i] = Y[r];
}
extern "C" int cl_chrom_subsample(cl_chrom* src, const int64_t* rows, int64_t m, cl_chrom** out)
{
    if (!src || !out) return fail(CL_ERR_ARG, "cl_chrom_subsample: null argument");
    *out = nullptr;
    if (m < 0 || m >= (1LL << 31) - 1024 || (m > 0 && !rows)) return fail(CL_ERR_ARG, "cl_chrom_subsample: bad row list");
    if (src->enq != src->deq) return fail(CL_ERR_ARG, "cl_chrom_subsample: asynchronous runs still in flight on the source, call cl_wait first");
    HIP_TRY(hipSetDevice(src->device));
    std::vector<int> r32((size_t)m);
    for (int64_t i = 0; i < m; ++i) {
        if (rows[i] < 0 || rows[i] >= src->n) return fail(CL_ERR_ARG, "cl_chrom_subsample: row index out of range");
        r32[(size_t)i] = (int)rows[i];
    }
    int *dx = nullptr, *dy = nullptr, *dr = nullptr;
    int rc = CL_OK;
    if (m > 0) {
        if (hipMalloc((void**)&dx, (size_t)m * 4) != hipSuccess || hipMalloc((void**)&dy, (size_t)m * 4) != hipSuccess ||
            hipMalloc((void**)&dr, (size_t)m * 4) != hipSuccess) rc = fail(CL_ERR_HIP, "hipMalloc (subsample)");
        if (rc == CL_OK && hipMemcpyAsync(dr, r32.data(), (size_t)m * 4, hipMemcpyHostToDevice, src->stream) != hipSuccess) rc = fail(CL_ERR_HIP, "hipMemcpy (row list)");
        if (rc == CL_OK) {
            hipLaunchKernelGGL(k_gather_rows, dim3(nblocks(m)), dim3(TPB), 0, src->stream, (const int*)src->d_x, (const int*)src->d_y, (const int*)dr, (int)m, dx, dy);
            if (hipStreamSynchronize(src->stream) != hipSuccess) rc = fail(CL_ERR_HIP, "gather (subsample)");
        }
        if (dr) (void)hipFree(dr);
    }
    if (rc == CL_OK) rc = cl_chrom_create(src->device, nullptr, dx, dy, m, 1, out);
    if (rc != CL_OK) { std::string keep = g_err; if (dx) (void)hipFree(dx); if (dy) (void)hipFree(dy); g_err = keep; return rc; }
    (*out)->own_xy = true;
    return CL_OK;
}

#define CMP_TPB 256
#define CMP_PER 8
#define CMP_BLOCK (CMP_TPB * CMP_PER)
__global__ void __launch_bounds__(256)
k_cut_strips(int S, int thr, const int* __restrict__ bstrip, const int* __restrict__ bq,
             int* __restrict__ sloc ,
             int* __restrict__ bsum, int* __restrict__ boff , int* ticket,
             int* __restrict__ src0 ,
             int* __restrict__ pre_out , const int* __restrict__ pre_ref ,
             int* __restrict__ dpre_out , int2* __restrict__ blen_out , int bandq, int eps,
             int* __restrict__ clr , int nclr, int* __restrict__ counters,
             int4* __restrict__ tab_out ,
             const u32* __restrict__ brow , GridParams g, int2* __restrict__ fix_out )
{
    __shared__ int red[4];
    const int s = blockIdx.x * blockDim.x + threadIdx.x;
    if (clr) {
        for (int u = s; u < nclr; u += gridDim.x * blockDim.x) clr[u] = 0;
        if (s < 16) counters[s] = 0;
    }
    int kv = 0;
    if (s == S) { if (pre_out) pre_out[S] = 0; if (pre_ref) dpre_out[S] = 0; }
    if (s < S) {
        const int b = bstrip[s];
        int lo = b;
        const int e = bstrip[s + 1];
        int hi = e;
        if (!pre_ref) {
            while (lo < hi) { const int mid = (int)(((unsigned)lo + (unsigned)hi) >> 1); if (bq[mid] < thr) lo = mid + 1; else hi = mid; }
        } else {
            int l1 = b, h1 = e, l2 = b, h2 = e;
            const int q2 = bandq + eps;
            while ((lo < hi) | (l1 < h1) | (l2 < h2)) {
                const int m0 = (int)(((unsigned)lo + (unsigned)hi) >> 1), m1 = (int)(((unsigned)l1 + (unsigned)h1) >> 1), m2 = (int)(((unsigned)l2 + (unsigned)h2) >> 1);
                const int v0 = bq[m0], v1 = bq[m1], v2 = bq[m2];
                if (lo < hi) { if (v0 < thr) lo = m0 + 1; else hi = m0; }
                if (l1 < h1) { if (v1 < bandq) l1 = m1 + 1; else h1 = m1; }
                if (l2 < h2) { if (v2 < q2) l2 = m2 + 1; else h2 = m2; }
            }
            dpre_out[s] = (lo - b) - pre_ref[s];
            blen_out[s] = make_int2(l1 - lo, l2 - lo);
        }
        kv = e - lo;
        src0[s] = lo;
        if (pre_out) pre_out[s] = lo - b;
        if (tab_out) tab_out[s] = make_int4(lo, pre_ref ? lo + blen_out[s].x : lo, lo - b, 0);
        if (fix_out) {
            int2 fx = make_int2(lo, INT_MAX);
            if (lo < e && lo > b) {
                const int q0 = div_eps(g, bq[lo]) * g.eps;
                if (bq[lo - 1] >= q0) {
                    const int qend = q0 + g.eps;
                    int k = lo, m = INT_MAX;
                    bool on = true;
                    while (on) {
                        int qv[4]; u32 rv[4];
#pragma unroll
                        for (int u = 0; u < 4; ++u) { const int kk = min(k + u, e - 1); qv[u] = bq[kk]; rv[u] = brow[kk]; }
#pragma unroll
                        for (int u = 0; u < 4; ++u) {
                            if (on && k + u < e && qv[u] < qend) m = min(m, (int)rv[u]); else if (on) { on = false; k += u; }
                        }
                        if (on) k += 4;
                    }
                    fx = make_int2(k, m);
                }
            }
            fix_out[s] = fx;
        }
    }
    if (s == S && tab_out) tab_out[S] = make_int4(bstrip[S], bstrip[S], 0, 0);
    int tot;
    const int incl = wg256_inclusive_scan(kv, red, tot);
    if (s <= S) sloc[s] = incl - kv;
    scan_tail_last_block(tot, bsum, boff, ticket, red);
}
template <bool BAND>
__global__ void __launch_bounds__(CMP_TPB)
k_cut_copy(int n, int S, int rbits, int thr, const int* __restrict__ bq, const int* __restrict__ bsp, const u32* __restrict__ brow,
           const int* __restrict__ src0, const int* __restrict__ sloc, const int* __restrict__ sboffs ,
           int* __restrict__ strip_start ,
           int* __restrict__ sv, int* __restrict__ sa, u32* __restrict__ srow, int* __restrict__ tile_s0, int* __restrict__ d_M,
           int expect_m, int* __restrict__ counters, int* __restrict__ poff_out ,
           const int* __restrict__ poff_ref , int* __restrict__ D_out ,
           int nbb, const int2* __restrict__ blen, int* __restrict__ band_words, int eps, int minPts, int dbg)
{
    if (BAND) {
        __shared__ int2 l_band[CMP_TPB / 64][KB_CAP];
        if ((int)blockIdx.x < nbb) {
            const int wv = threadIdx.x >> 6;
            band_wave(blockIdx.x * (CMP_TPB / 64) + wv, threadIdx.x & 63, l_band[wv], S, eps, 1 << rbits, minPts, bq, bsp, src0,
                      sloc, sboffs, blen, band_words, dbg);
            return;
        }
    }
    const int cb = (int)blockIdx.x - (BAND ? nbb : 0), ncb = (int)gridDim.x - (BAND ? nbb : 0);
    const int M = sloc[S] + sboffs[S >> 8];
    const int base = cb * CMP_BLOCK;
    int q[CMP_PER], sp[CMP_PER], d0[CMP_PER], s0[CMP_PER]; u32 row[CMP_PER]; bool keep[CMP_PER];
#pragma unroll
    for (int k = 0; k < CMP_PER; ++k) {
        const int i = base + k * CMP_TPB + (int)threadIdx.x;
        q[k] = i < n ? bq[i] : INT_MIN;
        keep[k] = i < n && q[k] >= thr;
    }
#pragma unroll
    for (int k = 0; k < CMP_PER; ++k) {
        const int i = base + k * CMP_TPB + (int)threadIdx.x;
        sp[k] = keep[k] ? bsp[i] : 0;
        row[k] = keep[k] ? brow[i] : 0u;
    }
#pragma unroll
    for (int k = 0; k < CMP_PER; ++k) {
        const int st = sp[k] >> rbits;
        d0[k] = keep[k] ? sloc[st] + sboffs[st >> 8] : 0;
        s0[k] = keep[k] ? src0[st] : 0;
    }
#pragma unroll
    for (int k = 0; k < CMP_PER; ++k) {
        if (keep[k]) {
            const int i = base + k * CMP_TPB + (int)threadIdx.x;
            const int dst = d0[k] + (i - s0[k]);
            sv[dst] = q[k]; sa[dst] = sp[k]; srow[dst] = row[k];
            if ((dst & 255) == 0) tile_s0[dst >> 8] = sp[k] >> rbits;
        }
    }
    for (int u = cb * CMP_TPB + (int)threadIdx.x; u <= S; u += ncb * CMP_TPB) {
        const int st = sloc[u] + sboffs[u >> 8];
        strip_start[u] = st;
        if (poff_out || poff_ref) {
            const int po = (u < S ? src0[u] : n) - st;
            if (poff_out) poff_out[u] = po; else D_out[u] = po - poff_ref[u];
        }
    }
    const int t = cb * CMP_TPB + (int)threadIdx.x;
    for (int u = t; u <= n / 256; u += ncb * CMP_TPB) if (u * 256 >= M) tile_s0[u] = S;
    for (int u = t; u < SORT_PAD; u += ncb * CMP_TPB) if (M + u < n) { sv[M + u] = INT_MAX; sa[M + u] = S << rbits; }
    if (t == 0) {
        d_M[0] = M;
        strip_start[S + 1] = n;
        if (expect_m >= 0 && expect_m != M) counters[CTR_OVERFLOW] = 8;
    }
}

__global__ void __launch_bounds__(CMP_TPB)
k_band(int S, int rbits, int eps, int minPts, const int* __restrict__ bq, const int* __restrict__ bsp, const int* __restrict__ src0,
       const int* __restrict__ sloc, const int* __restrict__ sboffs, const int2* __restrict__ blen, int* __restrict__ band_words,
       int* __restrict__ d_M, int expect_m, int* __restrict__ counters, int dbg)
{
    __shared__ int2 l_band[CMP_TPB / 64][KB_CAP];
    const int wv = threadIdx.x >> 6;
    if (blockIdx.x == 0 && threadIdx.x == 0) {
        const int M = sloc[S] + sboffs[S >> 8];
        d_M[0] = M;
        if (expect_m >= 0 && expect_m != M) counters[CTR_OVERFLOW] = 8;
    }
    band_wave<true>(blockIdx.x * (CMP_TPB / 64) + wv, threadIdx.x & 63, l_band[wv], S, eps, 1 << rbits, minPts, bq, bsp, src0, sloc, sboffs, blen, band_words, dbg);
}
__global__ void k_store_m(int S, const int* __restrict__ sloc, const int* __restrict__ sboffs, int* __restrict__ d_M, int expect_m, int* __restrict__ counters)
{
    const int M = sloc[S] + sboffs[S >> 8];
    d_M[0] = M;
    if (expect_m >= 0 && expect_m != M) counters[CTR_OVERFLOW] = 8;
}

#define WORKSPACE_WANTS(c, n) \
    struct Want { DevBuf* b; size_t bytes; }; \
    const Want wants[] = { \
        {&c->keys_in, n * 8}, {&c->keys_out, n * 8}, {&c->vals_in, n * 4}, {&c->vals_out, n * 4}, \
        {&c->sv, (n + 2 * SORT_PAD) * 4}, {&c->sa, (n + 2 * SORT_PAD) * 4}, {&c->cnt, n * 4}, \
        {&c->parent, n * 4}, {&c->root, n * 4}, {&c->head, n * 4}, {&c->cellfirst, n * 4}, \
        {&c->compkey, n * 4}, {&c->ncore, n * 4}, {&c->bsize, n * 4}, {&c->owner, n * 4}, {&c->state, n * 4}, \
        {&c->flag, (n + 1) * 4}, {&c->rankscan, (n + 1) * 4}, {&c->hdr, 256}, \
        {&c->slot[0].labels, n * 4}, {&c->slot[0].table, (n + 1) * sizeof(cl_box)}, {&c->slot[0].slab, n * 4}, \
        {&c->slot[1].labels, n * 4}, {&c->slot[1].table, (n + 1) * sizeof(cl_box)}, {&c->slot[1].slab, n * 4}, \
        {&c->ulist, n * 4}, {&c->lo, n * 4}, {&c->hi, n * 4}, {&c->recs, n * sizeof(Rec)}, \
        {&c->chainflag, n * 4}, {&c->chainhead, n * 4}, {&c->usize, n * 4}, {&c->tile_s0, (n / 256 + 2) * 4}, \
        {&c->base.q, (n + 2 * SORT_PAD) * 4}, {&c->base.sp, (n + 2 * SORT_PAD) * 4}, {&c->base.row, n * 4}, {&c->base.tile, (n / 256 + 2) * 4}, \
        {&c->fine.q, n * 4}, {&c->fine.sp, n * 4}, {&c->fine.row, n * 4}, \
        {&c->qb_key, n * 4}, {&c->qb_val, n * 8}, {&c->k7_cls, n + 16}, {&c->rc.cnt, n * 4}, {&c->rootlist, n * 4}, {&c->cflag8, n + 16}, \
        {&c->slot[0].d_step, 16 + sizeof(K7Part) + K7_LOGBINS * 8 + K7_FINE * 8 + K7_BLOCKS * sizeof(K7Part)}, \
        {&c->slot[1].d_step, 16 + sizeof(K7Part) + K7_LOGBINS * 8 + K7_FINE * 8 + K7_BLOCKS * sizeof(K7Part)}, \
    };

static int workspace_tmp_sizes(cl_chrom* c, size_t* sort_out, size_t* scan_out)
{
    const size_t n = (size_t)c->n;
    size_t sort_bytes = 0, scan_bytes = 0, scan2 = 0, scan3 = 0, sb2 = 0;
    hipError_t e = rocprim::radix_sort_pairs<SortConfig>(nullptr, sort_bytes, (u64*)nullptr, (u64*)nullptr, (u32*)nullptr, (u32*)nullptr,
                                                         n, 0, 64, c->stream);
    if (e != hipSuccess) return fail(CL_ERR_HIP, "radix_sort_pairs size query", hipGetErrorString(e));
    e = rocprim::radix_sort_pairs<SortConfig>(nullptr, sb2, (u32*)nullptr, (u32*)nullptr, (u64*)nullptr, (u64*)nullptr, n, 0, 32, c->stream);
    if (e != hipSuccess) return fail(CL_ERR_HIP, "radix_sort_pairs size query (q index)", hipGetErrorString(e));
    e = rocprim::inclusive_scan(nullptr, scan_bytes, (int*)nullptr, (int*)nullptr, n, rocprim::maximum<int>(), c->stream);
    if (e != hipSuccess) return fail(CL_ERR_HIP, "inclusive_scan size query", hipGetErrorString(e));
    e = rocprim::exclusive_scan(nullptr, scan2, (int*)nullptr, (int*)nullptr, 0, n + 1, rocprim::plus<int>(), c->stream);
    if (e != hipSuccess) return fail(CL_ERR_HIP, "exclusive_scan size query", hipGetErrorString(e));
    e = rocprim::inclusive_scan_by_key(nullptr, scan3, rocprim::make_reverse_iterator((int*)nullptr), rocprim::make_reverse_iterator((int*)nullptr),
                                       rocprim::make_reverse_iterator((int*)nullptr), n, rocprim::minimum<int>(), rocprim::equal_to<int>(), c->stream);
    if (e != hipSuccess) return fail(CL_ERR_HIP, "inclusive_scan_by_key size query", hipGetErrorString(e));
    size_t sb3 = 0;
    {
        GridParams g0{};
        const auto kin = rocprim::make_transform_iterator(rocprim::counting_iterator<int>(0), SpKeyOfIndex{nullptr, nullptr, g0});
        const auto vin = rocprim::make_transform_iterator(rocprim::counting_iterator<int>(0), SpValOfIndex{nullptr, nullptr});
        e = rocprim::radix_sort_pairs<SortConfig>(nullptr, sb3, kin, (u32*)nullptr, vin, SplitOut{nullptr, nullptr}, n, 0, 32, c->stream);
        if (e != hipSuccess) return fail(CL_ERR_HIP, "radix_sort_pairs size query (layout)", hipGetErrorString(e));
    }
    *sort_out = std::max<size_t>(std::max(std::max(sort_bytes, sb2), sb3), 16);
    *scan_out = std::max<size_t>(std::max(std::max(scan_bytes, scan2), scan3), 16);
    return CL_OK;
}

static size_t g_arena_overcommit = 0;
extern "C" void cl_debug_arena_overcommit(int64_t extra_bytes) { g_arena_overcommit = extra_bytes > 0 ? (size_t)extra_bytes : 0; }

static int reserve_workspace(cl_chrom* c)
{
    const size_t n = (size_t)c->n;
    WORKSPACE_WANTS(c, n);
    if (!c->arena.p && n > 0) {
        const std::string keep_err = g_err;
        size_t sort_bytes = 16, scan_bytes = 16;
        if (workspace_tmp_sizes(c, &sort_bytes, &scan_bytes) != CL_OK) { (void)hipGetLastError(); g_err = keep_err; return CL_OK; }
        const size_t s_guess = (size_t)(((long long)c->st.vmax - c->st.vmin) / 1000 + 64);
        const long long cand0 = std::max<long long>((long long)n / 8, std::min<long long>(1 << 20, (long long)n + 1024));
        std::vector<Want> all(std::begin(wants), std::end(wants));
        all.push_back({&c->sort_tmp, sort_bytes}); all.push_back({&c->scan_tmp, scan_bytes});
        all.push_back({&c->strip, (s_guess + 2) * 4}); all.push_back({&c->base.strip, (s_guess + 2) * 4}); all.push_back({&c->sel_tmp, (s_guess + 2) * 8 + (s_guess / 256 + 4) * 8 + 64});
        all.push_back({&c->blk_tmp, (n / 32 / 1024 + 4) * 8});
        all.push_back({&c->cand.box, (size_t)cand0 * 16}); all.push_back({&c->cand.step, (size_t)cand0 * 4});
        bool untouched = true;
        size_t total = 0;
        for (const Want& w : all) { untouched = untouched && w.b->p == nullptr; total += ((w.bytes + 255) / 256) * 256 + 256; }
        total += g_arena_overcommit;
        if (untouched && c->arena.ensure(total) != CL_OK) { (void)hipGetLastError(); g_err = keep_err; }
        else if (untouched) {
            char* at = (char*)c->arena.p;
            for (const Want& w : all) { const size_t sz = ((w.bytes + 255) / 256) * 256 + 256; w.b->adopt(at, sz); at += sz; }
            c->cand.cap = cand0;
        }
    }
    return CL_OK;
}

int ensure_workspace(cl_chrom* c, int S)
{
    const size_t n = (size_t)c->n;
    int rc;
    WORKSPACE_WANTS(c, n);
    if (!c->arena.p) (void)reserve_workspace(c);
    const cl_chrom::Slot* other = &c->slot[1 - c->cur];
    for (const Want& w : wants) if (w.b != &other->labels && w.b != &other->table && w.b != &other->slab && w.b != &c->slot[0].d_step && w.b != &c->slot[1].d_step && w.b != &c->base.q && w.b != &c->base.sp && w.b != &c->base.row && w.b != &c->base.tile && w.b != &c->qb_key &&
                                    w.b != &c->qb_val && w.b != &c->fine.q && w.b != &c->fine.sp && w.b != &c->fine.row && w.b != &c->k7_cls && w.b != &c->rc.cnt && w.b != &c->rootlist && w.b != &c->cflag8 && (rc = w.b->ensure(w.bytes))) return rc;
    if ((rc = c->strip.ensure(((size_t)S + 2) * 4)) || (rc = c->counters.ensure(256))) return rc;
    if (c->sv.fresh || c->sa.fresh) {
        hipLaunchKernelGGL(k_init_pads, dim3(nblocks(2 * SORT_PAD)), dim3(TPB), 0, c->stream, c->sv.as<int>(), c->sa.as<int>(), (long long)n);
        c->sv.fresh = c->sa.fresh = false;
    }
    size_t sort_bytes = 16, scan_bytes = 16;
    if (c->sort_tmp.bytes < 16 || c->scan_tmp.bytes < 16 || c->tmp_n != c->n) {
        if ((rc = workspace_tmp_sizes(c, &sort_bytes, &scan_bytes))) return rc;
        if ((rc = c->sort_tmp.ensure(sort_bytes)) || (rc = c->scan_tmp.ensure(scan_bytes))) return rc;
        c->tmp_n = c->n;
    }
    return CL_OK;
}


static int make_grid(cl_chrom* c, int variant, int eps, int minPts, int cut, GridParams* g)
{
    g->eps = eps; g->minPts = minPts; g->cut = cut; g->variant = variant;
    g->dbg = 0; g->dbg2 = 0;
    for (auto& w : g->tmask) w = 0;
    if (minPts >= 1 && minPts <= 128) g->tmask[(minPts - 1) >> 5] = 1u << ((minPts - 1) & 31);
    g->tgap = minPts - 1;
    g->qmin = INT_MIN;
#ifdef CLOOPS_DEVEL
    { const char* e = getenv("CLOOPS_DBG"); g->dbg = e ? atoi(e) : 0; }
    { const char* e = getenv("CLOOPS_DBG2"); g->dbg2 = e ? atoi(e) : 0; }
#endif
    g->swap = (g->dbg & 16) ? 0 : 1;
    {
        const unsigned d = (unsigned)eps;
        int l = 0; while ((1ull << l) < d) ++l;
        g->magic = (u32)((((1ull << 32) * ((1ull << l) - d)) / d) + 1);
        g->sh1 = l < 1 ? l : 1; g->sh2 = l > 1 ? l - 1 : 0;
    }
    if (variant == CL_VARIANT_CDBSCAN2) {
        if (c->st.amin < 0 || c->st.xmin < 0) return fail(CL_ERR_DOMAIN, "variant 2 (cDBSCAN2) needs 0 <= X <= Y for every PET");
        g->A0 = 0; g->V0 = 0;
    } else {
        g->A0 = g->swap ? c->st.vmin : c->st.amin; g->V0 = g->swap ? c->st.amin : c->st.vmin;
    }
    const int pmin = g->swap ? c->st.vmin : c->st.amin, pmax = g->swap ? c->st.vmax : c->st.amax;
    long long lo = ((long long)pmin - g->A0) / eps;
    long long hi = ((long long)pmax - g->A0) / eps;
    long long S = hi - lo + 1;
    if (S > (1LL << 28)) return fail(CL_ERR_GRID, "eps too small for the coordinate extent (strip table > 2^28 rows)");
    g->s0 = (int)lo; g->S = (int)S;
    const int qmin = g->swap ? c->st.amin : c->st.vmin, qmax = g->swap ? c->st.amax : c->st.vmax;
    (void)qmin;
    g->qbits = std::max(1, bits_for((unsigned)((long long)qmax - g->V0)));
    g->qtop = (int)std::min<long long>((long long)qmax - g->V0, INT_MAX);
    g->rbits = bits_for((unsigned)(eps - 1));
    g->peps = 1 << g->rbits;
    if ((S + 2) << g->rbits > (long long)INT_MAX)
        return fail(CL_ERR_GRID, "coordinate extent too large for this eps (X+Y range + 2*eps must stay below 2^30)");
    return CL_OK;
}


void ev_record(cl_chrom* c, int k)
{
    if (c->profiling) (void)hipEventRecord(c->slot[c->cur].ev[k], c->stream);
}

static int strip_maxlen(cl_chrom* c, const GridParams& g, int* out)
{
    const int layout = (g.variant == CL_VARIANT_CDBSCAN2 ? 2 : 0) | (g.swap ? 1 : 0);
    for (const auto& pl : c->plans)
        if (pl.layout == layout && pl.eps == g.eps) { *out = pl.maxlen; return CL_OK; }
    const int n = (int)c->n;
    int* hist = c->strip.as<int>();
    int* dmax = c->counters.as<int>() + CTR_MAXLEN;
    HIP_TRY(hipMemsetAsync(hist, 0, ((size_t)g.S + 2) * 4, c->stream));
    HIP_TRY(hipMemsetAsync(dmax, 0, 4, c->stream));
    LAUNCH(k_strip_hist, n, c->d_x, c->d_y, n, g, hist);
    hipLaunchKernelGGL(k_max_int, dim3(std::min(nblocks(g.S), 1024)), dim3(TPB), 0, c->stream, hist, g.S, dmax);
    int* h = c->h_pinned + 128;
    HIP_TRY(hipMemcpyAsync(h, dmax, 4, hipMemcpyDeviceToHost, c->stream));
    HIP_TRY(hipStreamSynchronize(c->stream));
    if (c->plans.size() >= 64) c->plans.erase(c->plans.begin());
    c->plans.push_back({layout, g.eps, *h});
    *out = *h;
    return CL_OK;
}

static int sort_layout(cl_chrom* c, const GridParams& g, int* dsv, int* dsa, u32* drow ,
                       int* dstrip, int* dtile)
{
    const int n = (int)c->n;
    const int sh = g.qbits + g.rbits, strip_bits = std::max(1, bits_for((unsigned)g.S));
    const int layout = (g.variant == CL_VARIANT_CDBSCAN2 ? 2 : 0) | (g.swap ? 1 : 0);
    const bool use_index = c->sort_index_mode > 0 || (c->sort_index_mode == 0 && (c->n_sorts >= 1 || c->qindex_layout == layout));
    ++c->n_sorts;
    bool hybrid = false;
    if (!use_index && !(g.dbg & 256) && (g.qbits + strip_bits + 8) / 9 - (strip_bits + 8) / 9 >= 2 && (long long)n <= 64LL * g.S) {
        int maxlen = 0, rc;
        if ((rc = strip_maxlen(c, g, &maxlen))) return rc;
        hybrid = maxlen <= HS_LMAX;
    }
    if (use_index) {
        int rc;
        u32* k32_in = c->vals_in.as<u32>(); u32* k32_out = c->vals_out.as<u32>();
        u64* v64_in = c->keys_in.as<u64>(); u64* v64_out = c->keys_out.as<u64>();
        if (c->qindex_layout != layout) {
            if ((rc = c->qb_key.ensure((size_t)n * 4)) || (rc = c->qb_val.ensure((size_t)n * 8))) return rc;
            LAUNCH(k_make_qkeys, n, c->d_x, c->d_y, n, g, k32_in, v64_in);
            size_t tb = c->sort_tmp.bytes;
            hipError_t e = rocprim::radix_sort_pairs<SortConfig>(c->sort_tmp.p, tb, k32_in, c->qb_key.as<u32>(), v64_in, c->qb_val.as<u64>(),
                                                                 (size_t)n, 0, g.qbits, c->stream);
            if (e != hipSuccess) return fail(CL_ERR_HIP, "radix_sort_pairs(q index)", hipGetErrorString(e));
            c->qindex_layout = layout;
        }
        ev_record(c, 0);
        if (g.cut <= 0) {
            ev_record(c, 1);
            u32* rows = drow ? drow : k32_in;
            auto strip_sort = [&](const GridParams& gx, int* osa, int* osv, u32* orow, int* ostrip, int* otile) -> int {
                const int sbits = std::max(1, bits_for((unsigned)gx.S));
                const auto kin = rocprim::make_transform_iterator(rocprim::counting_iterator<int>(0), SpKeyOfIndex{c->qb_key.as<u32>(), c->qb_val.as<u64>(), gx});
                const auto vin = rocprim::make_transform_iterator(rocprim::counting_iterator<int>(0), SpValOfIndex{c->qb_key.as<u32>(), c->qb_val.as<u64>()});
                size_t need = 0;
                hipError_t e = rocprim::radix_sort_pairs<SortConfig>(nullptr, need, kin, (u32*)osa, vin, SplitOut{osv, orow}, (size_t)n, gx.rbits, gx.rbits + sbits, c->stream);
                if (e != hipSuccess) return fail(CL_ERR_HIP, "radix_sort_pairs(strips) size query", hipGetErrorString(e));
                int rc2;
                if (need > c->sort_tmp.bytes && (rc2 = c->sort_tmp.ensure(need))) return rc2;
                size_t tb = c->sort_tmp.bytes;
                e = rocprim::radix_sort_pairs<SortConfig>(c->sort_tmp.p, tb, kin, (u32*)osa, vin, SplitOut{osv, orow}, (size_t)n, gx.rbits, gx.rbits + sbits, c->stream);
                if (e != hipSuccess) return fail(CL_ERR_HIP, "radix_sort_pairs(strips)", hipGetErrorString(e));
                LAUNCH(k_strip_table32, gx.S + 2, (const u32*)osa, n, gx.S, gx.rbits, ostrip, otile);
                return CL_OK;
            };
            const int fw = c->fine.w;
            if (fw > 0 && g.eps % fw == 0 && g.eps / fw <= CL_FINE_KMAX) {
                if (c->fine.valid_w != fw || c->fine.layout != layout) {
                    GridParams gf;
                    if (make_grid(c, g.variant, fw, 1, 0, &gf) != CL_OK) c->fine.w = 0;
                    else {
                        gf.dbg = g.dbg; gf.dbg2 = g.dbg2;
                        if ((rc = c->fine.q.ensure((size_t)n * 4)) || (rc = c->fine.sp.ensure((size_t)n * 4)) || (rc = c->fine.row.ensure((size_t)n * 4)) ||
                            (rc = c->fine.strip.ensure(((size_t)gf.S + 2) * 4))) return rc;
                        if ((rc = strip_sort(gf, c->fine.sp.as<int>(), c->fine.q.as<int>(), c->fine.row.as<u32>(), c->fine.strip.as<int>(), (int*)nullptr))) return rc;
                        c->fine.g = gf; c->fine.valid_w = fw; c->fine.layout = layout;
                    }
                }
                if (c->fine.w > 0) {
                    const GridParams& gf = c->fine.g;
                    const int k = g.eps / fw;
                    LAUNCH(k_strips_from_fine, g.S + 2, g.S, g.s0, k, gf.S, gf.s0, (const int*)c->fine.strip.as<int>(), n, dstrip);
                    int qb = bits_for((unsigned)std::min<long long>((long long)gf.qtop + 1, 0x7fffffffLL));
                    if (qb > 28) qb = 0;
                    hipLaunchKernelGGL(k_layout_from_fine, dim3(nblocks(n, LFF_T)), dim3(256), 0, c->stream, n, g, gf, k, (unsigned)(((1ull << 32) + (unsigned)k - 1ull) / (unsigned)k), qb, (const int*)c->fine.q.as<int>(),
                                       (const int*)c->fine.sp.as<int>(), (const u32*)c->fine.row.as<u32>(), (const int*)c->fine.strip.as<int>(), dsv, dsa, rows, dtile);
                    HIP_TRY(hipGetLastError());
                    c->run.srow = rows;
                    return CL_OK;
                }
            }
            if ((rc = strip_sort(g, dsa, dsv, rows, dstrip, dtile))) return rc;
            c->run.srow = rows;
            return CL_OK;
        }
        LAUNCH(k_make_spkeys, n, n, g, (const u32*)c->qb_key.as<u32>(), (const u64*)c->qb_val.as<u64>(), k32_in, v64_in);
        ev_record(c, 1);
        size_t tb = c->sort_tmp.bytes;
        hipError_t e = rocprim::radix_sort_pairs<SortConfig>(c->sort_tmp.p, tb, k32_in, k32_out, v64_in, v64_out, (size_t)n, g.rbits, g.rbits + strip_bits, c->stream);
        if (e != hipSuccess) return fail(CL_ERR_HIP, "radix_sort_pairs(strips)", hipGetErrorString(e));
        LAUNCH(k_strip_table32, g.S + 2, (const u32*)k32_out, n, g.S, g.rbits, dstrip, (int*)nullptr);
        u32* rows = drow ? drow : k32_in;
        LAUNCH(k_decode_sp, n, n, g, (const u32*)k32_out, (const u64*)v64_out, dsv, dsa, dtile, rows);
        c->run.srow = rows;
        return CL_OK;
    }
    ev_record(c, 0);
    LAUNCH(k_make_keys, n, c->d_x, c->d_y, n, g, c->keys_in.as<u64>(), c->vals_in.as<u32>());
    ev_record(c, 1);
    size_t tmp_bytes = c->sort_tmp.bytes;
    const int end_bit = sh + strip_bits;
    hipError_t e = rocprim::radix_sort_pairs<SortConfig>(c->sort_tmp.p, tmp_bytes, c->keys_in.as<u64>(), c->keys_out.as<u64>(),
                                             c->vals_in.as<u32>(), c->vals_out.as<u32>(), (size_t)n, hybrid ? sh : g.rbits, end_bit, c->stream);
    if (e != hipSuccess) return fail(CL_ERR_HIP, "radix_sort_pairs", hipGetErrorString(e));
    LAUNCH(k_strip_table, g.S + 2, c->keys_out.as<u64>(), n, g.S, sh, dstrip);
    if (hybrid) {
        u32* rows = drow ? drow : c->vals_in.as<u32>();
        hipLaunchKernelGGL(k_strip_sort, dim3(nblocks(n, HS_TPB)), dim3(HS_TPB), 0, c->stream, n, g, c->keys_out.as<u64>(),
                           c->vals_out.as<u32>(), dstrip, dsv, dsa, rows, dtile, c->counters.as<int>());
        c->run.srow = rows;
    } else {
        LAUNCH(k_decode_sorted, n, n, g, c->keys_out.as<u64>(), dsv, dsa, dtile, c->vals_out.as<u32>(), drow);
        c->run.srow = drow ? drow : c->vals_out.as<u32>();
    }
    return CL_OK;
}

static int run_sort_and_count(cl_chrom* c, const GridParams& g, bool exact, int level_cap)
{
    const int n = (int)c->n;
    int rc;
    c->run.m = n; c->run.m_exact = g.cut <= 0;
    if (g.cut > 0 && g.cut < DCUM_BINS && !c->dcum.empty()) { c->run.m = (int)(n - c->dcum[g.cut]); c->run.m_exact = true; }
    int* wsv = c->sv.as<int>() + SORT_PAD;
    int* wsa = c->sa.as<int>() + SORT_PAD;
    c->run.cnt = c->cnt.as<int>();
    c->last_k2_mode = 0;
    GridParams gk = g;
    bool k2_band = false, k2_skip = false;
    c->run.ws = WordSrc{c->cnt.as<int>(), nullptr, nullptr, nullptr, 0, g.rbits};
    c->run.level = exact ? 0 : std::min(level_cap, 3);
    c->slot[c->cur].band_timed = false; c->slot[c->cur].n_queried = 0;
    if (!c->reuse_layout) {
        if ((rc = sort_layout(c, g, wsv, wsa, nullptr, c->strip.as<int>(), c->tile_s0.as<int>()))) return rc;
        c->run.sv = wsv; c->run.sa = wsa; c->run.strip = c->strip.as<int>(); c->run.tile = c->tile_s0.as<int>();
    } else {
        const int layout = (g.variant == CL_VARIANT_CDBSCAN2 ? 2 : 0) | (g.swap ? 1 : 0);
        if (!c->base.valid || c->base.layout != layout || c->base.eps != g.eps) {
            c->base.invalidate();
            c->rc.invalidate();
            if ((rc = c->base.q.ensure(((size_t)n + 2 * SORT_PAD) * 4)) || (rc = c->base.sp.ensure(((size_t)n + 2 * SORT_PAD) * 4)) ||
                (rc = c->base.row.ensure((size_t)n * 4)) || (rc = c->base.strip.ensure(((size_t)g.S + 2) * 4)) ||
                (rc = c->base.tile.ensure(((size_t)n / 256 + 2) * 4))) return rc;
            if (c->base.q.fresh || c->base.sp.fresh) {
                hipLaunchKernelGGL(k_init_pads, dim3(nblocks(2 * SORT_PAD)), dim3(TPB), 0, c->stream, c->base.q.as<int>(), c->base.sp.as<int>(), (long long)n);
                c->base.q.fresh = c->base.sp.fresh = false;
            }
            GridParams g0 = g;
            g0.cut = 0;
            if ((rc = sort_layout(c, g0, c->base.q.as<int>() + SORT_PAD, c->base.sp.as<int>() + SORT_PAD, c->base.row.as<u32>(),
                                  c->base.strip.as<int>(), c->base.tile.as<int>()))) return rc;
            c->base.valid = true; c->base.layout = layout; c->base.eps = g.eps;
        } else {
            ev_record(c, 0);
            ev_record(c, 1);
        }
        const long long dmin = g.swap ? c->st.amin : 0;
        const bool on_base = g.cut <= 0 || (g.swap && (long long)g.cut <= dmin);
        const int m1 = g.minPts - 1;
        const bool cacheable = !exact && c->reuse_counts && g.swap && m1 >= 1 && m1 <= 127;
        const int thr_new = on_base ? 0 : g.cut - g.V0;
        enum { RC_NONE, RC_MAKE, RC_SAME, RC_REMAP } rcmode = RC_NONE;
        const bool want4 = level_cap >= 4 && cacheable;
        if (cacheable) {
            const bool serves = c->rc.valid && c->rc.layout == layout && c->rc.eps == g.eps && g.minPts <= c->rc.cap &&
                                ((c->rc.tmask[m1 >> 5] >> (m1 & 31)) & 1u) && c->rc.base_space == want4;
            if (serves && thr_new == c->rc.thr && !(c->rc.cut_on_base && thr_new != 0)) rcmode = RC_SAME;
            else if (serves && !on_base && (long long)g.S <= 8LL * n) rcmode = RC_REMAP;
            else rcmode = RC_MAKE;
            if ((rc = c->rc.cnt.ensure((size_t)n * 4)) || (rc = c->rc.pre.ensure(((size_t)g.S + 2) * 4)) ||
                (rc = c->rc.poff.ensure(((size_t)g.S + 2) * 4)) || (rc = c->rc.dpre.ensure(((size_t)g.S + 2) * 4)) ||
                (rc = c->rc.D.ensure(((size_t)g.S + 2) * 4)) || (rc = c->rc.blen.ensure(((size_t)g.S + 2) * 8))) return rc;
        }
        c->run.level = want4 ? 4 : std::min(level_cap, 3);
        if (exact) c->run.level = 0;
        if (c->run.level == 4 && g.variant == CL_VARIANT_CDBSCAN2 && !c->base.key_valid) {
            if ((rc = lists_base_keys(c, g))) return rc;
            c->base.key_valid = true;
        }
        if (rcmode == RC_MAKE) {
            c->rc.valid = true; c->rc.layout = layout; c->rc.eps = g.eps; c->rc.thr = thr_new; c->rc.cap = g.minPts; c->rc.base_space = want4;
            c->rc.cut_on_base = false;
            for (int k = 0; k < 4; ++k) c->rc.tmask[k] = 0;
            for (int t = 2; t < g.minPts; ++t) {
                const bool in = ((c->count_tmask[(t - 1) >> 5] >> ((t - 1) & 31)) & 1u) || (c->count_floor > 0 && t >= c->count_floor);
                if (in) c->rc.tmask[(t - 1) >> 5] |= 1u << ((t - 1) & 31);
            }
            c->rc.tmask[m1 >> 5] |= 1u << (m1 & 31);
            for (int k = 0; k < 4; ++k) gk.tmask[k] = c->rc.tmask[k];
            gk.tgap = 0;
            for (int t = 2, prev = 1; t <= g.minPts; ++t)
                if ((c->rc.tmask[(t - 1) >> 5] >> ((t - 1) & 31)) & 1u) { gk.tgap = std::max(gk.tgap, t - prev); prev = t; }
            c->run.cnt = c->rc.cnt.as<int>();
            if (want4 && !on_base) c->run.cnt = c->cnt.as<int>();
            c->run.ws.rc = c->run.cnt;
            if (on_base) {
                HIP_TRY(hipMemsetAsync(c->rc.pre.p, 0, ((size_t)g.S + 2) * 4, c->stream));
                HIP_TRY(hipMemsetAsync(c->rc.poff.p, 0, ((size_t)g.S + 2) * 4, c->stream));
            }
            if (want4 && !on_base && (long long)g.S <= 8LL * n) {
                HIP_TRY(hipMemsetAsync(c->rc.pre.p, 0, ((size_t)g.S + 2) * 4, c->stream));
                HIP_TRY(hipMemsetAsync(c->rc.poff.p, 0, ((size_t)g.S + 2) * 4, c->stream));
                c->run.l4_make_base = true;
                c->rc.thr = thr_new;
                c->rc.cut_on_base = true;
                c->run.cnt = c->rc.cnt.as<int>();
                rcmode = RC_REMAP;
                c->run.k2_make = true;
            }
        }
        if (rcmode == RC_SAME) {
            c->run.cnt = c->rc.cnt.as<int>();
            c->run.ws.rc = c->run.cnt;
            k2_skip = true;
            c->last_k2_mode = 1;
        } else if (rcmode == RC_REMAP) {
            c->run.ws = WordSrc{c->rc.cnt.as<int>(), c->cnt.as<int>(), c->rc.D.as<int>(), c->rc.dpre.as<int>(), std::max(thr_new, c->rc.thr) + g.eps, g.rbits};
            k2_band = true;
            c->last_k2_mode = c->run.k2_make ? 0 : 2;
        }
        if (on_base) {
            c->run.sv = c->base.q.as<int>() + SORT_PAD; c->run.sa = c->base.sp.as<int>() + SORT_PAD; c->run.srow = c->base.row.as<u32>();
            c->run.strip = c->base.strip.as<int>(); c->run.tile = c->base.tile.as<int>();
        } else {
            if (!g.swap) return fail(CL_ERR_ARG, "internal: layout reuse needs the v-band layout");
            const int nb = nblocks(n, CMP_BLOCK);
            const int nblk = nblocks(g.S + 1, 256);
            if ((rc = c->sel_tmp.ensure(((size_t)g.S + 2) * 8 + ((size_t)nblk + 2) * 8 + 64))) return rc;
            int* sloc = c->sel_tmp.as<int>();
            int* src0 = sloc + g.S + 2;
            int* bsum = src0 + g.S + 2;
            int* sboffs = bsum + nblk + 2;
            int* d_M = c->counters.as<int>() + CTR_M;
            const int thr = g.cut - g.V0;
            const int* bq = c->base.q.as<int>() + SORT_PAD;
            const bool l4 = c->run.level == 4;
            c->run.l4_cut = true; c->run.l4_band = rcmode == RC_REMAP;
            if (l4 && ((rc = c->l_tab.ensure(((size_t)g.S + 2) * 16)) || (rc = c->l_fix.ensure(((size_t)g.S + 2) * 8)))) return rc;
            LAUNCH(k_cut_strips, g.S + 1, g.S, thr, (const int*)c->base.strip.as<int>(), bq, sloc, bsum, sboffs, c->counters.as<int>() + CTR_TICKET_A, src0,
                   rcmode == RC_MAKE ? c->rc.pre.as<int>() : (int*)nullptr,
                   rcmode == RC_REMAP ? (const int*)c->rc.pre.as<int>() : (const int*)nullptr,
                   rcmode == RC_REMAP ? c->rc.dpre.as<int>() : (int*)nullptr, rcmode == RC_REMAP ? c->rc.blen.as<int2>() : (int2*)nullptr,
                   c->run.ws.bandq, g.eps, c->run.init_nclr > 0 ? c->flag.as<int>() : (int*)nullptr, c->run.init_nclr, c->counters.as<int>(),
                   l4 ? c->l_tab.as<int4>() : (int4*)nullptr, (const u32*)c->base.row.as<u32>(), g,
                   (l4 && g.variant == CL_VARIANT_CDBSCAN2) ? c->l_fix.as<int2>() : (int2*)nullptr);
            c->run.init_nclr = 0;
            if (l4 && rcmode == RC_REMAP) {
                const int nbb = nblocks(nblocks(g.S, KB_SB), CMP_TPB / 64);
                if (c->profiling) { (void)hipEventRecord(c->slot[c->cur].ev[8], c->stream); c->slot[c->cur].band_timed = true; }
                hipLaunchKernelGGL(k_band, dim3(nbb), dim3(CMP_TPB), 0, c->stream, g.S, g.rbits, g.eps, g.minPts, bq, (const int*)(c->base.sp.as<int>() + SORT_PAD),
                                   (const int*)src0, (const int*)sloc, (const int*)sboffs, (const int2*)c->rc.blen.as<int2>(), c->cnt.as<int>(), d_M,
                                   c->run.m_exact ? c->run.m : -1, c->counters.as<int>(), g.dbg);
                if (c->profiling) (void)hipEventRecord(c->slot[c->cur].ev[9], c->stream);
                c->run.dM = d_M;
            } else if (l4 && rcmode == RC_SAME) {
                hipLaunchKernelGGL(k_store_m, dim3(1), dim3(1), 0, c->stream, g.S, (const int*)sloc, (const int*)sboffs, d_M, c->run.m_exact ? c->run.m : -1, c->counters.as<int>());
                c->run.dM = d_M;
            } else
            if (rcmode == RC_REMAP) {
                const int nbb = nblocks(nblocks(g.S, KB_SB), CMP_TPB / 64);
                hipLaunchKernelGGL(k_cut_copy<true>, dim3(nbb + nb), dim3(CMP_TPB), 0, c->stream, n, g.S, g.rbits, thr, bq, (const int*)(c->base.sp.as<int>() + SORT_PAD),
                                   (const u32*)c->base.row.as<u32>(), (const int*)src0, (const int*)sloc, (const int*)sboffs, c->strip.as<int>(), wsv, wsa, c->vals_out.as<u32>(), c->tile_s0.as<int>(),
                                   d_M, c->run.m_exact ? c->run.m : -1, c->counters.as<int>(), (int*)nullptr, (const int*)c->rc.poff.as<int>(), c->rc.D.as<int>(),
                                   nbb, (const int2*)c->rc.blen.as<int2>(), c->cnt.as<int>(), g.eps, g.minPts, g.dbg);
            } else
            hipLaunchKernelGGL(k_cut_copy<false>, dim3(nb), dim3(CMP_TPB), 0, c->stream, n, g.S, g.rbits, thr, bq, (const int*)(c->base.sp.as<int>() + SORT_PAD),
                               (const u32*)c->base.row.as<u32>(), (const int*)src0, (const int*)sloc, (const int*)sboffs, c->strip.as<int>(), wsv, wsa, c->vals_out.as<u32>(), c->tile_s0.as<int>(),
                               d_M, c->run.m_exact ? c->run.m : -1, c->counters.as<int>(), rcmode == RC_MAKE ? c->rc.poff.as<int>() : (int*)nullptr,
                               (const int*)nullptr, (int*)nullptr, 0, (const int2*)nullptr, (int*)nullptr, 0, 0, 0);
            c->run.sv = wsv; c->run.sa = wsa; c->run.srow = c->vals_out.as<u32>();
            c->run.strip = c->strip.as<int>(); c->run.tile = c->tile_s0.as<int>();
            if (!c->run.dM) c->run.dM = d_M;
        }
    }
    ev_record(c, 2);
    rc = CL_OK;
    if (c->run.l4_make_base) {
        GridParams g0 = gk;
        g0.cut = 0;
        g0.qmin = c->rc.thr;
        rc = cl_launch_region(c->stream, g0, n, n, false, c->base.q.as<int>() + SORT_PAD, c->base.sp.as<int>() + SORT_PAD, c->base.strip.as<int>(), c->base.tile.as<int>(),
                              c->rc.cnt.as<int>());
        c->slot[c->cur].n_queried = c->run.m;
    } else if (!k2_skip && !k2_band && !SKIP(256)) {
        rc = cl_launch_region(c->stream, gk, n, c->run.m, exact, c->run.sv, c->run.sa, c->run.strip, c->run.tile, c->run.cnt);
        c->slot[c->cur].n_queried = c->run.m;
    }
    if (rc) return rc;
    if (c->run.level == 4 && c->run.l4_cut && !k2_skip && !k2_band && (rc = lists_words_to_base(c, g))) return rc;
    ev_record(c, 3);
    HIP_TRY(hipGetLastError());
    return CL_OK;
}

__global__ void k_nop() {}

int ensure_events(cl_chrom* c)
{
    if (c->profiling && !c->ev_ready) {
        for (auto& sl : c->slot) for (auto& e : sl.ev) HIP_TRY(hipEventCreate(&e));
        c->ev_ready = true;
        float v[9];
        hipEvent_t a = c->slot[0].ev[0], b = c->slot[0].ev[1];
        for (int r = 0; r < 9; ++r) {
            HIP_TRY(hipEventRecord(a, c->stream));
            hipLaunchKernelGGL(k_nop, dim3(1), dim3(64), 0, c->stream);
            HIP_TRY(hipEventRecord(b, c->stream));
            HIP_TRY(hipEventSynchronize(b));
            (void)hipEventElapsedTime(&v[r], a, b);
        }
        std::sort(v, v + 9);
        c->ev_bracket_ms = v[4];
    }
    return CL_OK;
}

static int check_args(cl_chrom* c, int eps, int minPts, int cut)
{
    if (!c) return fail(CL_ERR_ARG, "null chromosome handle");
    if (eps <= 0) return fail(CL_ERR_ARG, "eps must be > 0 (the reference divides by it: ZeroDivisionError)");
    if (eps >= (1 << 30)) return fail(CL_ERR_ARG, "eps must be < 2^30");
    if (minPts < 0) return fail(CL_ERR_ARG, "minPts must be >= 0");
    (void)cut;
    return CL_OK;
}

extern "C" int cl_neighbor_counts(cl_chrom* c, int32_t eps, int32_t cut, int32_t* counts_out)
{
    int rc = check_args(c, eps, 1, cut);
    if (rc) return rc;
    if (c->n == 0) return CL_OK;
    if (!counts_out) return fail(CL_ERR_ARG, "counts_out is null");
    HIP_TRY(hipSetDevice(c->device));
    GridParams g;
    run_begin(c);
    if ((rc = make_grid(c, CL_VARIANT_CDBSCAN1, eps, 1, cut, &g))) return rc;
    if ((rc = ensure_workspace(c, g.S))) return rc;
    if ((rc = ensure_events(c))) return rc;
    if ((rc = run_sort_and_count(c, g, true, c->traversal))) return rc;
    const int n = (int)c->n;
    HIP_TRY(hipMemsetAsync(c->slot[c->cur].labels.p, 0xFF, (size_t)n * 4, c->stream));
    LAUNCH(k_scatter_counts, n, c->run.strip, g.S, c->run.srow, c->cnt.as<int>(), c->slot[c->cur].labels.as<int>());
    HIP_TRY(hipMemcpyAsync(counts_out, c->slot[c->cur].labels.p, (size_t)n * 4, hipMemcpyDeviceToHost, c->stream));
    HIP_TRY(hipStreamSynchronize(c->stream));
    if (c->profiling) {
        memset(&c->timing, 0, sizeof(c->timing));
        hipEvent_t* ev = c->slot[c->cur].ev;
        (void)hipEventElapsedTime(&c->timing.ms_keys, ev[0], ev[1]);
        (void)hipEventElapsedTime(&c->timing.ms_sort, ev[1], ev[2]);
        (void)hipEventElapsedTime(&c->timing.ms_region, ev[2], ev[3]);
        c->timing.n_strips = g.S + 2;
    }
    c->have_result = false;
    return CL_OK;
}

__global__ void k_pack_header(int* __restrict__ hdr, const int* __restrict__ rankscan_total, const int* __restrict__ counters,
                              const int* __restrict__ d_M)
{
    if (threadIdx.x == 0 && blockIdx.x == 0) {
        hdr[0] = rankscan_total[0];
        hdr[1] = counters[CTR_OVERFLOW];
        hdr[2] = d_M[0];
        hdr[3] = 0;
        hdr[4] = -1;
        hdr[5] = 0;
    }
}

__global__ void k_export_table(int* __restrict__ hdr, Table t, cl_box* __restrict__ host_rows, int cap)
{
    const int K = hdr[0];
    const bool store = cap >= 0;
    const int lim = store ? min(K, cap) : K;
    int nc = 0, ml = -1;
    for (int k = blockIdx.x * blockDim.x + threadIdx.x; k < lim; k += gridDim.x * blockDim.x) {
        if (store) {
            cl_box b = t.get(k);
            if (b.count > 0) { ++nc; ml = k; } else { b.min_x = b.max_x = b.min_y = b.max_y = 0; }
            host_rows[k] = b;
        } else if (t.count[k] > 0) { ++nc; ml = k; }
    }
    for (int o = 32; o > 0; o >>= 1) { nc += __shfl_down(nc, o); ml = max(ml, __shfl_down(ml, o)); }
    if ((threadIdx.x & 63) == 0) {
        if (nc) atomicAdd(&hdr[3], nc);
        if (ml >= 0) atomicMax(&hdr[4], ml);
    }
    if (blockIdx.x == 0 && threadIdx.x == 0 && store && K > cap) hdr[5] = 1;
}

Table make_table_slot(cl_chrom* c, int slot)
{
    Table t;
    int* base = c->slot[slot].table.as<int>();
    const size_t stride = (size_t)c->n + 1;
    t.count = base; t.minx = base + stride; t.maxx = base + 2 * stride; t.miny = base + 3 * stride; t.maxy = base + 4 * stride;
    return t;
}
Table make_table(cl_chrom* c) { return make_table_slot(c, c->cur); }

const int* k7_hist_for(cl_chrom* c, int cut)
{
    return (cut > 0 && cut < DCUM_BINS && c->n_neg == 0 && !c->dcum.empty() && c->dhist.p) ? c->dhist.as<int>() : (const int*)nullptr;
}

int finish_enqueue(cl_chrom* c, const RunRequest& req, int n_strips, const int* d_M)
{
    const int n = (int)c->n;
    int32_t* const labels_out = req.labels_out;
    cl_chrom::Slot& sl = c->slot[c->cur];
    int* dh = c->hdr.as<int>() + 16 * c->cur;
    if (sl.h_boxes_cap == 0 && c->export_table && req.step < 0) {
        const size_t cap = (size_t)n / 16 + 65536;
        HIP_TRY(hipHostMalloc((void**)&sl.h_boxes, cap * sizeof(cl_box), hipHostMallocDefault));
        sl.h_boxes_cap = cap;
    }
    if (!c->run.hdr_packed)
        hipLaunchKernelGGL(k_pack_header, dim3(1), dim3(64), 0, c->stream, dh, c->run.k_total ? c->run.k_total : c->rankscan.as<int>() + n, c->counters.as<int>(), d_M);
    const bool exported = c->export_table && req.step < 0;
    if (req.step < 0)
        hipLaunchKernelGGL(k_export_table, dim3(256), dim3(TPB), 0, c->stream, dh, make_table(c), sl.h_boxes,
                           exported ? (int)std::min<size_t>(sl.h_boxes_cap, 0x7fffffff) : -1);
    sl.exported = exported;
    sl.step_valid = false;
    sl.host_written = false;
    if (req.step >= 0) {
        int rc;
        if ((rc = c->k7_cls.ensure((size_t)n + 16))) return rc;
        const int kmax = std::max(1, std::min(sl.kmax, n));
        if ((rc = ensure_cand_capacity(c, c->cand.n + kmax))) return rc;
        const size_t out_bytes = 16 + sizeof(K7Part) + K7_LOGBINS * 8 + K7_FINE * 8;
        if ((rc = sl.d_step.ensure(out_bytes + K7_BLOCKS * sizeof(K7Part)))) return rc;
        const int nb = nblocks(kmax, CAND_BLOCK);
        if ((rc = c->sel_tmp.ensure((size_t)nb * 12 + 64))) return rc;
        int* bcount = c->sel_tmp.as<int>();
// ... 506 lines not shown
```

### cloops_amd/csrc/k_lists.hip

```cpp
#include "cl_chrom.h"

#ifdef CLOOPS_DEVEL
#define L_ABL(bit) (g.dbg2 & (bit))
#else
#define L_ABL(bit) 0
#endif
#ifdef CLOOPS_DEVEL
__device__ unsigned long long g_lstat[32];
__device__ __forceinline__ void lstat_add(int slot, int v)
{
    int t = v;
    for (int o = 32; o > 0; o >>= 1) t += __shfl_down(t, o);
    if ((threadIdx.x & 63) == 0 && t) atomicAdd(&g_lstat[slot], (unsigned long long)t);
}
extern "C" void cl_debug_lstats(unsigned long long* out)
{
    (void)hipDeviceSynchronize();
    (void)hipMemcpyFromSymbol(out, HIP_SYMBOL(g_lstat), sizeof(g_lstat));
    unsigned long long z[32] = {0};
    (void)hipMemcpyToSymbol(HIP_SYMBOL(g_lstat), z, sizeof(z));
}
#define LSTAT_ON (g.dbg2 & (1 << 30))
#define LSTAT(slot, v) do { if (LSTAT_ON) lstat_add((slot), (v)); } while (0)
#else
// ... 1634 lines not shown
        idx[ch] = (blockIdx.x * LF_CHUNKS + ch) * LF_TPB + threadIdx.x;
        const int k = idx[ch];
        own[ch] = -1; pos[ch] = 0; pr[ch] = make_int2(0, 0);
        if (k < C) { own[ch] = croot[k]; pr[ch] = cpair[k]; pos[ch] = (labels || pairs) ? cpos[k] : 0; }
        else if (k < L) { own[ch] = owner_root(wowner[k - C]); pr[ch] = wpair[k - C]; pos[ch] = (labels || pairs) ? wpos[k - C] : 0; }
    }
#pragma unroll
    for (int ch = 0; ch < LF_CHUNKS; ++ch) lab[ch] = own[ch] >= 0 ? rlabel[own[ch]] : -1;
#pragma unroll
    for (int ch = 0; ch < LF_CHUNKS; ++ch) {
        const int k = idx[ch];
        x[ch] = 0; y[ch] = 0;
        if (k < L) {
            llab[k] = lab[ch];
            ldist[k] = pr[ch].x;
            if (lab[ch] >= 0) {
                if (labels) labels[srow[pos[ch]]] = lab[ch];
                const int spv = pr[ch].y;
                const int pp = ((spv >> g.rbits) + g.s0) * g.eps + (spv & (g.peps - 1)) + g.A0, qq = pr[ch].x + g.V0;
                const int a = g.swap ? qq : pp, v = g.swap ? pp : qq;
                x[ch] = (v - a) / 2; y[ch] = (v + a) / 2;
            }
        }
    }
    if (pairs) {
        __shared__ int l_pc[LF_CHUNKS * (LF_TPB / 64)];
        __shared__ int l_pbase;
        const int lane = threadIdx.x & 63, wv = threadIdx.x >> 6;
        unsigned long long bals[LF_CHUNKS];
#pragma unroll
        for (int ch = 0; ch < LF_CHUNKS; ++ch) {
            bals[ch] = __ballot(lab[ch] >= 0);
            if (lane == 0) l_pc[ch * (LF_TPB / 64) + wv] = __popcll(bals[ch]);
        }
        __syncthreads();
        if (threadIdx.x == 0) {
            int tot = 0;
            for (int k = 0; k < LF_CHUNKS * (LF_TPB / 64); ++k) { const int v = l_pc[k]; l_pc[k] = tot; tot += v; }
            l_pbase = tot ? atomicAdd(pair_count, tot) : 0;
        }
        __syncthreads();
#pragma unroll
        for (int ch = 0; ch < LF_CHUNKS; ++ch) {
            if (lab[ch] < 0) continue;
            const int at = l_pbase + l_pc[ch * (LF_TPB / 64) + wv] + lane_rank(bals[ch]);
            if (at < pairs_cap) pairs[at] = make_int2((int)srow[pos[ch]], lab[ch]);
        }
    }
    if (L_ABL(1 << 10)) return;
#pragma unroll
    for (int ch = 0; ch < LF_CHUNKS; ++ch) table_accumulate(t, h, lab[ch], x[ch], y[ch]);
    if (L_ABL(1 << 9)) return;
    table_flush(t, h);
}

struct ListBufs {
    unsigned long long *cmask, *wmask, *hmask;
    int *cgloc, *wgloc, *cgrank, *wgrank;
    int *bsum, *sup, *lcnt;
    int nsup2;
};
static int list_bufs(cl_chrom* c, const GridParams& g, int nm, ListBufs* b)
{
    const size_t n = (size_t)c->n;
    const size_t ngrp_cap = n / 64 + LG + 4;
    const size_t nblk_cap = n / LT + 4;
    int rc;
    if ((rc = c->l_mask.ensure(3 * ngrp_cap * 8)) || (rc = c->l_rank.ensure(4 * ngrp_cap * 4)) ||
        (rc = c->l_blk.ensure((2 * (nblk_cap + 1) + 2 * (nblk_cap / 16 + 4) + 16) * 4)) || (rc = c->l_cstrip.ensure(((size_t)g.S + 4) * 4)) ||
        (rc = c->l_wpos.ensure(n * 4)) || (rc = c->l_wenc.ensure(n * 4)) || (rc = c->l_dist.ensure(n * 4)) ||
        (c->traversal < 3 && (rc = c->l_aux.ensure(n * 4)))) return rc;
    b->cmask = c->l_mask.as<unsigned long long>(); b->wmask = b->cmask + ngrp_cap; b->hmask = b->wmask + ngrp_cap;
    b->cgloc = c->l_rank.as<int>(); b->wgloc = b->cgloc + ngrp_cap; b->cgrank = b->wgloc + ngrp_cap; b->wgrank = b->cgrank + ngrp_cap;
    const int nblk = nblocks(nm, LT);
    const size_t nsup_cap = nblk_cap / 16 + 4;
    if (c->l_blk.fresh) {
        HIP_TRY(hipMemsetAsync(c->l_blk.p, 0, c->l_blk.bytes, c->stream));
        c->l_blk.fresh = false;
    }
    b->lcnt = c->l_blk.as<int>();
    b->sup = b->lcnt + 8;
    b->bsum = b->sup + 2 * nsup_cap;
    b->nsup2 = 2 * ((nblk + 63) / 64 + 1);
    return CL_OK;
}

static void launch_classify(cl_chrom* c, const GridParams& g, int nblk, const ListBufs& b)
{
#define LA_ARGS g, (const int*)c->run.sv, (const int*)c->run.sa, (const int*)c->run.strip, c->run.ws, (const u32*)c->run.srow, b.cmask, b.wmask, b.hmask, b.cgloc, b.wgloc, b.bsum, b.sup, c->cellfirst.as<int>()
    if (g.variant == CL_VARIANT_CDBSCAN2) hipLaunchKernelGGL(k_classify<true>, dim3(nblk), dim3(256), 0, c->stream, LA_ARGS);
    else hipLaunchKernelGGL(k_classify<false>, dim3(nblk), dim3(256), 0, c->stream, LA_ARGS);
#undef LA_ARGS
}
static void launch_make_lists(cl_chrom* c, const GridParams& g, int nblk, const ListBufs& b, const ListRun& L)
{
#define LM_ARGS g, (const int*)c->run.sv, (const int*)c->run.sa, (const int*)c->run.strip, c->run.ws, (const u32*)c->run.srow, (const unsigned long long*)b.cmask,                   \
                (const unsigned long long*)b.wmask, (const unsigned long long*)b.hmask, (const int*)b.cgloc, (const int*)b.wgloc, (const int*)b.bsum, (const int*)b.sup,  \
                (const int*)c->cellfirst.as<int>(), b.cgrank, b.wgrank, L.cpair, L.cpos, L.ckey, L.wpair, L.wpos, L.wenc, b.lcnt
    if (g.variant == CL_VARIANT_CDBSCAN2) hipLaunchKernelGGL(k_make_lists<true>, dim3(nblk), dim3(256), 0, c->stream, LM_ARGS);
    else hipLaunchKernelGGL(k_make_lists<false>, dim3(nblk), dim3(256), 0, c->stream, LM_ARGS);
#undef LM_ARGS
}
static void list_views(cl_chrom* c, const ListBufs& b, ListRun* L)
{
    L->lcnt = b.lcnt; L->cmask = b.cmask; L->wmask = b.wmask; L->cgrank = b.cgrank; L->wgrank = b.wgrank;
    L->cpair = c->keys_in.as<int2>(); L->wpair = c->keys_out.as<int2>();
    L->cpos = c->head.as<int>(); L->ckey = c->hi.as<int>();
    L->wpos = c->l_wpos.as<int>(); L->wenc = c->l_wenc.as<int>(); L->cstrip = c->l_cstrip.as<int>();
}

static inline void fuse_knob(cl_chrom* c)
{
#ifdef CLOOPS_DEVEL
    const char* e = getenv("CLOOPS_FUSE");
    if (e) c->fuse_chains = atoi(e) != 0;
#else
    (void)c;
#endif
}

int lists_build(cl_chrom* c, const GridParams& g, int nm, ListRun* out)
{
    ListBufs b;
    int rc = list_bufs(c, g, nm, &b);
    if (rc) return rc;
    const int nblk = nblocks(nm, LT);
    ListRun L{};
    list_views(c, b, &L);
    if (c->l_sup_dirty) HIP_TRY(hipMemsetAsync(b.sup, 0, (size_t)b.nsup2 * 4, c->stream));
    c->l_sup_dirty = true;
    launch_classify(c, g, nblk, b);
    launch_make_lists(c, g, nblk, b, L);
    fuse_knob(c);
    if (c->fuse_chains)
        hipLaunchKernelGGL(k_prep_c, dim3(nblocks(std::max(std::max(nm, g.S + 2), b.nsup2))), dim3(TPB), 0, c->stream, g, (const int*)L.lcnt, (const int*)c->run.strip,
                           (const unsigned long long*)L.cmask, (const int*)L.cgrank, L.cstrip, b.sup, b.nsup2, c->parent.as<int>());
#ifdef CLOOPS_DEVEL
    else
    hipLaunchKernelGGL(k_chain_c, dim3(nblocks(nm, 256 * CH_PER)), dim3(256), 0, c->stream, g, L.lcnt, (const int2*)L.cpair, c->chainflag.as<int>(),
                       c->parent.as<int>(), c->compkey.as<int>(), c->ncore.as<int>(), c->bsize.as<int>(), c->usize.as<int>(), c->state.as<int>(),
                       c->cellfirst.as<int>() , (const int*)c->run.strip, L.cmask, L.cgrank, L.cstrip, b.sup, b.nsup2, (int*)nullptr);
#else
    { }
#endif
    L.npos = nm; L.pstrip = c->run.strip;
    *out = L;
    HIP_TRY(hipGetLastError());
    c->l_sup_dirty = false;
    return CL_OK;
}

int lists_base_keys(cl_chrom* c, const GridParams& g)
{
    const int n = (int)c->n;
    int rc = c->base.key.ensure((size_t)n * 4);
    if (rc) return rc;
    hipLaunchKernelGGL(k_base_keys, dim3(nblocks(n, LT)), dim3(256), 0, c->stream, g, n, (const int*)(c->base.q.as<int>() + SORT_PAD),
                       (const int*)(c->base.sp.as<int>() + SORT_PAD), (const u32*)c->base.row.as<u32>(), c->base.key.as<int>());
    HIP_TRY(hipGetLastError());
    return CL_OK;
}

int lists_build_base(cl_chrom* c, const GridParams& g, int nm, ListRun* out)
{
    fuse_knob(c);
    const int n = (int)c->n;
    ListBufs b;
    int rc = list_bufs(c, g, n, &b);
    if (rc) return rc;
    const int nblk = nblocks(n, LT);
    const bool v2 = g.variant == CL_VARIANT_CDBSCAN2;
    ListRun L{};
    list_views(c, b, &L);
    L.npos = n; L.pstrip = c->base.strip.as<int>();
    unsigned long long* sup64 = (unsigned long long*)b.sup;
    const int nsup_ints = 2 * (nblk / 16 + 2);
    if (c->l_sup_dirty) HIP_TRY(hipMemsetAsync(b.sup, 0, (size_t)std::max(nsup_ints, b.nsup2) * 4, c->stream));
    c->l_sup_dirty = true;
    const int* bq = c->base.q.as<int>() + SORT_PAD;
    const int* bsp = c->base.sp.as<int>() + SORT_PAD;
    const u32* brow = c->base.row.as<u32>();
    c->run.srow = c->base.row.as<u32>();
    const int* words = c->rc.cnt.as<int>();
    const int* band = c->cnt.as<int>();
    const int thr = c->run.l4_cut ? g.cut - g.V0 : INT_MIN;
    const int bandq = c->run.ws.bandq;
#define LCQ_ARGS g, n, thr, bandq, bq, words, band, b.cmask, b.wmask, b.cgloc, b.wgloc, b.bsum, sup64
    if (!c->run.l4_cut) hipLaunchKernelGGL((k_classify_q<false, false>), dim3(nblk), dim3(256), 0, c->stream, LCQ_ARGS);
    else if (c->run.l4_band) hipLaunchKernelGGL((k_classify_q<true, true>), dim3(nblk), dim3(256), 0, c->stream, LCQ_ARGS);
    else hipLaunchKernelGGL((k_classify_q<true, false>), dim3(nblk), dim3(256), 0, c->stream, LCQ_ARGS);
#undef LCQ_ARGS
#define LMQ_ARGS g, n, bandq, bq, bsp, brow, (const int*)c->base.key.as<int>(), (const int2*)c->l_fix.as<int2>(), words, band, (const unsigned long long*)b.cmask,                  \
                 (const unsigned long long*)b.wmask, (const int*)b.cgloc, (const int*)b.wgloc, (const int*)b.bsum, (const unsigned long long*)sup64, b.cgrank, b.wgrank, L.cpair,  \
                 c->run.rows ? L.cpos : (int*)nullptr, L.ckey, L.wpair, L.wpos, L.wenc, b.lcnt, c->fuse_chains ? c->parent.as<int>() : (int*)nullptr
    if (v2) {
        if (!c->run.l4_cut) hipLaunchKernelGGL((k_make_lists_q<true, false, false>), dim3(nblk), dim3(256), 0, c->stream, LMQ_ARGS);
        else if (c->run.l4_band) hipLaunchKernelGGL((k_make_lists_q<true, true, true>), dim3(nblk), dim3(256), 0, c->stream, LMQ_ARGS);
        else hipLaunchKernelGGL((k_make_lists_q<true, true, false>), dim3(nblk), dim3(256), 0, c->stream, LMQ_ARGS);
    } else {
        if (c->run.l4_band) hipLaunchKernelGGL((k_make_lists_q<false, true, true>), dim3(nblk), dim3(256), 0, c->stream, LMQ_ARGS);
        else hipLaunchKernelGGL((k_make_lists_q<false, false, false>), dim3(nblk), dim3(256), 0, c->stream, LMQ_ARGS);
    }
#undef LMQ_ARGS
    fuse_knob(c);
    if (c->fuse_chains)
        hipLaunchKernelGGL(k_prep_c, dim3(nblocks(std::max(g.S + 2, std::max(nsup_ints, b.nsup2)))), dim3(TPB), 0, c->stream, g, (const int*)L.lcnt,
                           (const int*)L.pstrip, (const unsigned long long*)L.cmask, (const int*)L.cgrank, L.cstrip, b.sup, std::max(nsup_ints, b.nsup2), (int*)nullptr);
#ifdef CLOOPS_DEVEL
    else
    hipLaunchKernelGGL(k_chain_c, dim3(nblocks(nm, 256 * CH_PER)), dim3(256), 0, c->stream, g, L.lcnt, (const int2*)L.cpair, c->chainflag.as<int>(),
                       c->parent.as<int>(), c->compkey.as<int>(), c->ncore.as<int>(), c->bsize.as<int>(), c->usize.as<int>(), c->state.as<int>(),
                       c->cellfirst.as<int>() , L.pstrip, L.cmask, L.cgrank, L.cstrip, b.sup, std::max(nsup_ints, b.nsup2), v2 ? L.ckey : (int*)nullptr);
#else
    { }
#endif
    *out = L;
    HIP_TRY(hipGetLastError());
    c->l_sup_dirty = false;
    return CL_OK;
}

int lists_words_to_base(cl_chrom* c, const GridParams& g)
{
    const int n = (int)c->n;
    LAUNCH(k_words_to_base, n, g, n, (const int*)(c->base.sp.as<int>() + SORT_PAD), (const int4*)c->l_tab.as<int4>(), (const int*)c->rc.poff.as<int>(),
           (const int*)c->cnt.as<int>(), c->rc.cnt.as<int>());
    HIP_TRY(hipGetLastError());
    return CL_OK;
}

static int* croot_of(cl_chrom* c) { return c->run.level >= 2 ? c->root.as<int>() : c->l_aux.as<int>(); }

int lists_union_flatten(cl_chrom* c, const GridParams& g, int nm, const ListRun& L)
{
    constexpr int UNT = 512;
    const int nt = nblocks(nm, UNT);
    const HeadReset hr{c->compkey.as<int>(), c->ncore.as<int>(), c->bsize.as<int>(), c->usize.as<int>(), c->state.as<int>()};
    int* prune = (c->run.level >= 4 && g.variant == CL_VARIANT_CDBSCAN2) ? L.ckey : (int*)nullptr;
#define LU_ARGS g, nt, L.lcnt, (const int2*)L.cpair, c->chainflag.as<int>(), (const int*)L.cstrip, c->cellfirst.as<int>() , \
                c->parent.as<int>(), hr, prune, c->ulist.as<int>() , c->counters.as<int>()
    constexpr int UK = 4;
    const bool big = (long long)c->n > 80LL * g.S;
#define LU_LAUNCH(HALO_, FUSE_, UK_) hipLaunchKernelGGL((k_union_c<UNT, HALO_, FUSE_, UK_>), dim3(ltile_grid(nt)), dim3(256), 0, c->stream, LU_ARGS)
    bool wide = false;
#ifdef CLOOPS_DEVEL
    { const char* e = getenv("CLOOPS_UNION_K"); wide = e && atoi(e) == 8; }
#endif
    if (c->fuse_chains) {
        if (!wide) { if (big) LU_LAUNCH(512, true, UK); else LU_LAUNCH(128, true, UK); }
#ifdef CLOOPS_DEVEL
        else { if (big) LU_LAUNCH(512, true, 8); else LU_LAUNCH(128, true, 8); }
#endif
        hipLaunchKernelGGL(k_union_overflow, dim3(1024), dim3(256), 0, c->stream, g, (const int*)c->counters.as<int>(), (const int*)c->ulist.as<int>(), (const int2*)L.cpair,
                           (const int*)c->chainflag.as<int>(), (const int*)L.cstrip, (const int*)c->cellfirst.as<int>(), c->parent.as<int>());
    }
#ifdef CLOOPS_DEVEL
    else { if (big) LU_LAUNCH(512, false, UK); else LU_LAUNCH(128, false, UK); }
#endif
#undef LU_LAUNCH
#undef LU_ARGS
    hipLaunchKernelGGL(k_flatten_c, dim3(nblocks(nm, FLC_TPB * FLC_PER)), dim3(FLC_TPB), 0, c->stream, L.lcnt, (const int*)c->chainflag.as<int>(),
                       (const int*)c->parent.as<int>(), (const int*)L.ckey, croot_of(c),
                       c->compkey.as<int>(), c->ncore.as<int>(), c->rootlist.as<int>(), c->counters.as<int>(), (int)g.dbg2);
    HIP_TRY(hipGetLastError());
    return CL_OK;
}

int lists_scatter_root(cl_chrom* c, int nm, const ListRun& L)
{
    HIP_TRY(hipMemsetAsync(c->root.p, 0xFF, (size_t)nm * 4, c->stream));
    LAUNCH(k_scatter_by_pos, nm, L.lcnt, (const int*)L.cpos, (const int*)croot_of(c), c->root.as<int>());
    return CL_OK;
}

int lists_border(cl_chrom* c, const GridParams& g, int nm, const ListRun& L)
{
    constexpr int BNT = 2048, BHC = 256, BNQ = 1024, BHQ = 254;
    (void)nm;
    int kcap = 2, bqg = 16;
    bool queued = true;
#ifdef CLOOPS_DEVEL
    { const char* e = getenv("CLOOPS_BCAP"); if (e) kcap = atoi(e); queued = kcap > 0; e = getenv("CLOOPS_BQG"); if (e) bqg = atoi(e); }
#endif
    const int nt = nblocks(L.npos, (g.variant == CL_VARIANT_CDBSCAN1 || !queued) ? BNT : BNQ);
#define LB_ARGS g, nt, L.npos, L.lcnt, L.cmask, L.cgrank, L.wgrank, (const int2*)L.cpair, (const int*)croot_of(c), (const int*)c->cellfirst.as<int>(),    \
                (const int*)L.ckey, (const int*)L.cstrip, (const int2*)L.wpair, (const int*)L.wpos, (const int*)L.wenc, (const int*)c->compkey.as<int>(),                    \
                (const int*)c->ncore.as<int>(), c->owner.as<int>(), c->bsize.as<int>(), c->usize.as<int>(), c->chainflag.as<int>() ,  \
                c->counters.as<int>()
    if (g.variant == CL_VARIANT_CDBSCAN1) hipLaunchKernelGGL((k_border_w<BNT, BHC, true>), dim3(ltile_grid(nt)), dim3(256), 0, c->stream, LB_ARGS);
#ifdef CLOOPS_DEVEL
    else if (!queued) hipLaunchKernelGGL((k_border_w<BNT, BHC, false>), dim3(ltile_grid(nt)), dim3(256), 0, c->stream, LB_ARGS);
#endif
#define LBQ_ARGS g, nt, L.npos, kcap, L.lcnt, L.cmask, L.cgrank, L.wgrank, (const int2*)L.cpair, (const int*)croot_of(c), (const int*)c->cellfirst.as<int>(),           \
                 (const int*)L.cstrip, (const int2*)L.wpair, (const int*)L.wpos, (const int*)L.wenc, (const int*)c->compkey.as<int>(), (const int*)c->ncore.as<int>(),        \
                 c->owner.as<int>(), c->bsize.as<int>(), c->usize.as<int>(), c->chainflag.as<int>(), c->counters.as<int>()
#ifdef CLOOPS_DEVEL
    else if (bqg == 8) hipLaunchKernelGGL((k_border_q<BNQ, BHQ, 8>), dim3(ltile_grid(nt)), dim3(256), 0, c->stream, LBQ_ARGS);
    else if (bqg == 32) hipLaunchKernelGGL((k_border_q<BNQ, BHQ, 32>), dim3(ltile_grid(nt)), dim3(256), 0, c->stream, LBQ_ARGS);
#endif
    else hipLaunchKernelGGL((k_border_q<BNQ, BHQ, 16>), dim3(ltile_grid(nt)), dim3(256), 0, c->stream, LBQ_ARGS);
    (void)bqg;
#undef LBQ_ARGS
#undef LB_ARGS
    HIP_TRY(hipGetLastError());
    return CL_OK;
}

int lists_emit_records(cl_chrom* c, const GridParams& g, int nm, const ListRun& L)
{
    (void)nm;
    hipLaunchKernelGGL(k_emit_records_w, dim3(2048), dim3(TPB), 0, c->stream, g, L.lcnt, L.cmask, L.cgrank, (const int2*)L.cpair, (const int*)croot_of(c),
                       (const int*)L.cstrip, (const int2*)L.wpair, (const int*)L.wpos, (const int*)L.wenc, (const int*)c->compkey.as<int>(),
                       (const int*)c->state.as<int>(), (const int*)c->owner.as<int>(), c->recs.as<Rec>(), (int)c->n, c->counters.as<int>(),
                       (const int*)c->chainflag.as<int>());
    HIP_TRY(hipGetLastError());
    return CL_OK;
}

int lists_scatter_owner(cl_chrom* c, int nm, const ListRun& L)
{
    int* opos = c->l_aux.as<int>();
    HIP_TRY(hipMemsetAsync(opos, 0xFF, (size_t)nm * 4, c->stream));
    LAUNCH(k_scatter_by_pos, nm, L.lcnt, (const int*)L.cpos, (const int*)croot_of(c), opos);
    LAUNCH(k_scatter_by_pos, nm, L.lcnt + 1, (const int*)L.wpos, (const int*)c->owner.as<int>(), opos);
    return CL_OK;
}

int lists_final(cl_chrom* c, const RunRequest& req, const GridParams& g, int nm, const ListRun& L, bool rows, int* pair_count)
{
    cl_chrom::Slot& sl = c->slot[c->cur];
    hipLaunchKernelGGL(k_final_lists, dim3(nblocks(nm, LF_TPB * LF_CHUNKS)), dim3(LF_TPB), 0, c->stream, g, L.lcnt, (const int2*)L.cpair, (const int*)L.cpos,
                       (const int*)croot_of(c), (const int2*)L.wpair, (const int*)L.wpos, (const int*)c->owner.as<int>(), (const int*)c->chainhead.as<int>(),
                       (const u32*)c->run.srow, (rows && !req.pairs_out) ? sl.labels.as<int>() : (int*)nullptr, sl.slab.as<int>(), c->l_dist.as<int>(), make_table(c),
                       req.pairs_out ? sl.pairs.as<int2>() : (int2*)nullptr, (int)std::min<long long>(req.pairs_cap, INT_MAX), pair_count);
    HIP_TRY(hipGetLastError());
    return CL_OK;
}

#define RM_T 2048
__global__ void __launch_bounds__(256)
k_rowmask_count(int n, const int* __restrict__ labels, unsigned long long* __restrict__ mask, int* __restrict__ tsum,
                unsigned long long* __restrict__ sup)
{
    __shared__ int l_c[4];
    const int t0 = (int)blockIdx.x * RM_T;
    const int lane = threadIdx.x & 63, wv = threadIdx.x >> 6;
    int lab[8];
#pragma unroll
    for (int u = 0; u < 8; ++u) { const int r = t0 + u * 256 + (int)threadIdx.x; lab[u] = r < n ? labels[r] : -1; }
    int cnt = 0;
#pragma unroll
    for (int u = 0; u < 8; ++u) {
        const unsigned long long bal = __ballot(lab[u] >= 0);
        if (lane == 0 && t0 + u * 256 + wv * 64 < n) mask[(t0 >> 6) + u * 4 + wv] = bal;
        cnt += __popcll(bal);
    }
    if (lane == 0) l_c[wv] = cnt;
    __syncthreads();
    if (threadIdx.x == 0) {
        const int tot = l_c[0] + l_c[1] + l_c[2] + l_c[3];
        tsum[blockIdx.x] = tot;
        if (tot) atomicAdd(&sup[blockIdx.x >> 4], (unsigned long long)tot);
    }
}
__global__ void __launch_bounds__(256)
k_rowmask_write(int n, const int* __restrict__ labels, const unsigned long long* __restrict__ mask, const int* __restrict__ tsum,
                const unsigned long long* __restrict__ sup, int* __restrict__ out, long long cap, int* __restrict__ total)
{
    __shared__ long long l_red[4];
    __shared__ int l_goff[RM_T / 64];
    const int blk = (int)blockIdx.x, t0 = blk * RM_T;
    const int lane = threadIdx.x & 63, wv = threadIdx.x >> 6;
    int lab[8];
#pragma unroll
    for (int u = 0; u < 8; ++u) { const int r = t0 + u * 256 + (int)threadIdx.x; lab[u] = r < n ? labels[r] : -1; }
    long long pc = 0;
    const int sb = blk >> 4;
    for (int k = threadIdx.x; k < sb; k += 256) pc += (long long)sup[k];
    if (threadIdx.x < 16) { const int k = sb * 16 + (int)threadIdx.x; if (k < blk) pc += tsum[k]; }
#pragma unroll
    for (int o = 32; o > 0; o >>= 1) pc += __shfl_down(pc, o);
    if (lane == 0) l_red[wv] = pc;
    if (threadIdx.x < 64) {
        const int k = lane & 31;
        const int gi = (t0 >> 6) + k;
        const int v = (lane < 32 && (long long)gi * 64 < n) ? __popcll(mask[gi]) : 0;
        int incl = v;
#pragma unroll
        for (int d = 1; d < 32; d <<= 1) { const int t = __shfl_up(incl, d, 32); incl += k >= d ? t : 0; }
        if (lane < 32) l_goff[k] = incl - v;
    }
    __syncthreads();
    const long long base = l_red[0] + l_red[1] + l_red[2] + l_red[3];
    if (blk == (int)gridDim.x - 1 && threadIdx.x == 0) *total = (int)(base + tsum[blk]);
#pragma unroll
    for (int u = 0; u < 8; ++u) {
        const unsigned long long bal = __ballot(lab[u] >= 0);
        if (lab[u] >= 0) {
            const long long dst = base + l_goff[u * 4 + wv] + __popcll(bal & low_mask(lane));
            if (dst < cap) out[dst] = lab[u];
        }
    }
}
int lists_rowmask(cl_chrom* c, const RunRequest& req, int* total)
{
    cl_chrom::Slot& sl = c->slot[c->cur];
    const long long n = c->n;
    const size_t nw = (size_t)((n + 63) / 64), ntile = (size_t)((n + RM_T - 1) / RM_T), nsup = ntile / 16 + 1;
    const size_t cap = (size_t)std::max<long long>(req.mask_cap, 1);
    const size_t o_lab = nw * 8, o_tsum = ((o_lab + cap * 4 + 255) / 256) * 256, o_sup = ((o_tsum + ntile * 4 + 255) / 256) * 256;
    int rc = sl.pairs.ensure(o_sup + nsup * 8 + 256);
    if (rc) return rc;
    char* p = (char*)sl.pairs.p;
    HIP_TRY(hipMemsetAsync(p + o_sup, 0, nsup * 8, c->stream));
    hipLaunchKernelGGL(k_rowmask_count, dim3((unsigned)ntile), dim3(256), 0, c->stream, (int)n, (const int*)sl.labels.as<int>(), (unsigned long long*)p,
                       (int*)(p + o_tsum), (unsigned long long*)(p + o_sup));
    hipLaunchKernelGGL(k_rowmask_write, dim3((unsigned)ntile), dim3(256), 0, c->stream, (int)n, (const int*)sl.labels.as<int>(), (const unsigned long long*)p,
                       (const int*)(p + o_tsum), (const unsigned long long*)(p + o_sup), (int*)(p + o_lab), (long long)req.mask_cap, total);
    HIP_TRY(hipGetLastError());
    return CL_OK;
}

#ifdef CLOOPS_DEVEL
extern "C" int cl_debug_time_lists(cl_chrom* c, int which, int reps, float* ms_out)
{
    if (!c || !ms_out || c->dbg_nm <= 0) return fail(CL_ERR_ARG, "cl_debug_time_lists: no rotated run on this handle");
    HIP_TRY(hipSetDevice(c->device));
    GridParams g = c->dbg_g;
    { const char* e = getenv("CLOOPS_DBG2"); g.dbg2 = e ? atoi(e) : 0; }
    const int nm = c->dbg_nm;
    ListBufs b;
    int rc = list_bufs(c, g, nm, &b);
    if (rc) return rc;
    const int nblk = nblocks(nm, LT);
    ListRun L{};
    list_views(c, b, &L);
    hipEvent_t e0, e1;
    HIP_TRY(hipEventCreate(&e0)); HIP_TRY(hipEventCreate(&e1));
    HIP_TRY(hipStreamSynchronize(c->stream));
    HIP_TRY(hipEventRecord(e0, c->stream));
    for (int r = 0; r < reps; ++r) {
        if (which == 0) {
            HIP_TRY(hipMemsetAsync(b.sup, 0, (size_t)b.nsup2 * 4, c->stream));
            launch_classify(c, g, nblk, b);
        } else if (which == 1) {
            launch_make_lists(c, g, nblk, b, L);
        } else if (which == 6 || which == 7) {
            const int n = (int)c->n;
            ListBufs bb;
            if ((rc = list_bufs(c, g, n, &bb))) return rc;
            const int nb4 = nblocks(n, LT);
            unsigned long long* sup64 = (unsigned long long*)bb.sup;
            const int* bq = c->base.q.as<int>() + SORT_PAD; const int* bsp = c->base.sp.as<int>() + SORT_PAD;
            const int thr = g.cut - g.V0, bandq = c->run.ws.bandq;
            if (which == 6) {
                HIP_TRY(hipMemsetAsync(bb.sup, 0, (size_t)2 * (nb4 / 16 + 2) * 4, c->stream));
                hipLaunchKernelGGL((k_classify_q<true, true>), dim3(nb4), dim3(256), 0, c->stream, g, n, thr, bandq, bq, (const int*)c->rc.cnt.as<int>(), (const int*)c->cnt.as<int>(),
                                   bb.cmask, bb.wmask, bb.cgloc, bb.wgloc, bb.bsum, sup64);
            } else {
                hipLaunchKernelGGL((k_make_lists_q<true, true, true>), dim3(nb4), dim3(256), 0, c->stream, g, n, bandq, bq, bsp, (const u32*)c->base.row.as<u32>(), (const int*)c->base.key.as<int>(),
                                   (const int2*)c->l_fix.as<int2>(), (const int*)c->rc.cnt.as<int>(), (const int*)c->cnt.as<int>(), (const unsigned long long*)bb.cmask,
                                   (const unsigned long long*)bb.wmask, (const int*)bb.cgloc, (const int*)bb.wgloc, (const int*)bb.bsum, (const unsigned long long*)sup64, bb.cgrank, bb.wgrank,
                                   L.cpair, (int*)nullptr, L.ckey, L.wpair, L.wpos, L.wenc, bb.lcnt, (int*)nullptr);
            }
        } else if (which == 4 || which == 3 || which == 5) {
            ListRun L2 = L;
            c->run.level = c->traversal >= 4 ? 4 : 3;
            if (c->run.level == 4) { ListBufs bb; if ((rc = list_bufs(c, g, (int)c->n, &bb))) return rc; list_views(c, bb, &L2); L2.npos = (int)c->n; L2.pstrip = c->base.strip.as<int>(); }
            else { L2.npos = nm; L2.pstrip = c->run.strip; }
            if (which == 4) { if ((rc = lists_border(c, g, nm, L2))) return rc; }
            else if (which == 3) {
                ListBufs bb; if ((rc = list_bufs(c, g, c->run.level == 4 ? (int)c->n : nm, &bb))) return rc;
                fuse_knob(c);
                if (c->fuse_chains)
                    hipLaunchKernelGGL(k_prep_c, dim3(nblocks(std::max(nm, g.S + 2))), dim3(TPB), 0, c->stream, g, (const int*)L2.lcnt, (const int*)L2.pstrip,
                                       (const unsigned long long*)L2.cmask, (const int*)L2.cgrank, L2.cstrip, bb.sup, 2, c->parent.as<int>());
#ifdef CLOOPS_DEVEL
                else
                hipLaunchKernelGGL(k_chain_c, dim3(nblocks(nm, 256 * CH_PER)), dim3(256), 0, c->stream, g, L2.lcnt, (const int2*)L2.cpair, c->chainflag.as<int>(),
                                   c->parent.as<int>(), c->compkey.as<int>(), c->ncore.as<int>(), c->bsize.as<int>(), c->usize.as<int>(), c->state.as<int>(),
                                   c->cellfirst.as<int>(), L2.pstrip, L2.cmask, L2.cgrank, L2.cstrip, bb.sup, 2, (int*)nullptr);
#else
    { }
#endif
                HIP_TRY(hipMemsetAsync(c->counters.p, 0, 64, c->stream));
                if ((rc = lists_union_flatten(c, g, nm, L2))) return rc;
            } else { if ((rc = lists_final(c, RunRequest(), g, nm, L2, false, c->counters.as<int>() + 40))) return rc; }
        } else return fail(CL_ERR_ARG, "cl_debug_time_lists: kernel not supported on its own");
    }
    HIP_TRY(hipEventRecord(e1, c->stream));
    HIP_TRY(hipEventSynchronize(e1));
    if (which == 1 || which == 7) HIP_TRY(hipMemsetAsync(b.sup, 0, c->l_blk.bytes - 64, c->stream));
    float ms = 0.f;
    (void)hipEventElapsedTime(&ms, e0, e1);
    *ms_out = ms / (float)std::max(1, reps);
    (void)hipEventDestroy(e0); (void)hipEventDestroy(e1);
    return CL_OK;
}
#endif
```

### include/cloops_hip.h

```cpp
#ifndef CLOOPS_HIP_H
#define CLOOPS_HIP_H

#include <stdint.h>

#ifdef __cplusplus
extern "C" {
#endif

#define CL_OK             0
#define CL_ERR_ARG       -1
#define CL_ERR_HIP       -2
#define CL_ERR_EMPTY     -3
#define CL_ERR_DOMAIN    -4
#define CL_ERR_GRID      -5
#define CL_ERR_NODEVICE  -6
#define CL_ERR_HASH      -7

#define CL_VARIANT_CDBSCAN1  1
#define CL_VARIANT_CDBSCAN2  2
#define CL_VARIANT_BLOCK     3

typedef struct cl_chrom cl_chrom;

typedef struct {
// ... 73 lines not shown

int cl_agg_loops(cl_chrom* c, int32_t cut, int32_t res, int32_t w, int32_t corner, int64_t n_loops, const int32_t* cx,
                 const int32_t* cy, int64_t* sum_out, int32_t* stats_out, int32_t* mats_out, int64_t* n_kept);

#define CL_TRACK_WASHU 0
#define CL_TRACK_JUICE 1
#define CL_TRACK_NAME_MAX 64
int cl_track_build(cl_chrom* c, int32_t kind, int64_t cut, int64_t ext, const int64_t* ids, const char* name_a,
                   const char* name_b, int64_t* n_records, int64_t* n_bytes);
int cl_track_chunks(cl_chrom* c, int64_t budget, int64_t cap, int64_t* rec_bounds, int64_t* byte_bounds, int64_t* n_chunks);
int cl_track_render(cl_chrom* c, int64_t chunk, char* out, int64_t cap, int64_t* n_bytes);
int cl_track_free(cl_chrom* c);

int cl_cov_build(cl_chrom* c, int64_t cut, int32_t ends, int64_t ext, int64_t res, int64_t* n_runs, uint32_t* max_depth,
                 int64_t* n_ends, int64_t* area);
int cl_cov_runs(cl_chrom* c, int64_t first, int64_t count, int32_t* start_out, int32_t* end_out, uint32_t* depth_out);
int cl_cov_text(cl_chrom* c, const char* name, int64_t scale_num, int64_t scale_den, int64_t* n_bytes);
int cl_cov_chunks(cl_chrom* c, int64_t budget, int64_t cap, int64_t* run_bounds, int64_t* byte_bounds, int64_t* n_chunks);
int cl_cov_render(cl_chrom* c, int64_t chunk, char* out, int64_t cap, int64_t* n_bytes);
int cl_cov_free(cl_chrom* c);

int cl_peak_sort(cl_chrom* c, int64_t cut, int32_t ends, int64_t* n_ends, int64_t* vmin, int64_t* vmax);
int cl_peak_call(cl_chrom* c, int64_t eps, int64_t min_pts, int64_t* n_peaks, int64_t* n_cores, int64_t* n_clustered);
int cl_peak_get(cl_chrom* c, int64_t first, int64_t count, int32_t* start, int32_t* end, uint32_t* n_points, uint32_t* n_cores);
int cl_peak_count(cl_chrom* c, const int64_t* starts, const int64_t* ends, int64_t n, uint32_t* counts);
int cl_peak_summits(cl_chrom* c, const int64_t* starts, const int64_t* ends, int64_t n, int64_t w, int32_t* pos, uint32_t* cnt);
int cl_peak_free(cl_chrom* c);

int cl_dom_tracks(cl_chrom* c, int64_t cut, int64_t res, int64_t w, int64_t* n_bins, int64_t* bin0, int64_t* n_kept);
int cl_dom_get(cl_chrom* c, int64_t first, int64_t count, uint32_t* cross, uint32_t* up, uint32_t* down);
int cl_dom_count(cl_chrom* c, const int64_t* starts, const int64_t* ends, int64_t n, uint32_t* intra, uint32_t* nx, uint32_t* ny);
int cl_dom_free(cl_chrom* c);

#define CL_KDIS_KMAX 64
#define CL_KDIS_BINS 3968
int cl_kdis_build(cl_chrom* c, int64_t cut, const int32_t* ks, int32_t n_k, int64_t* n_kept);
int cl_kdis_get(cl_chrom* c, int32_t which, int64_t first, int64_t count, int32_t* x, int32_t* y, int32_t* d);
int cl_kdis_hist(cl_chrom* c, int32_t which, uint64_t* hist, uint64_t* n_zero, uint64_t* n_none);
int cl_kdis_free(cl_chrom* c);

#define CL_MAT_WMAX 8192
#define CL_MAT_CELLS_MAX 16777216
int cl_mat_window(cl_chrom* c, int64_t cut, int64_t res, int64_t bx0, int64_t by0, int64_t nx, int64_t ny, int32_t mirror,
                  uint32_t* out, int64_t* n_in, int64_t* n_kept);
int cl_mat_cells(cl_chrom* c, int64_t cut, int64_t res, int32_t fold, int64_t* n_cells, int64_t* n_kept, int64_t* max_count);
int cl_mat_cells_get(cl_chrom* c, int64_t first, int64_t count, int32_t* bx, int32_t* by, uint32_t* cnt);
int cl_mat_v4c(cl_chrom* c, int64_t cut, int64_t res, int64_t v0, int64_t v1, int64_t b0, int64_t nb, uint32_t* out, int64_t* n_x,
               int64_t* n_y, int64_t* n_kept);
int cl_mat_free(cl_chrom* c);

#define CL_BAL_BINS_MAX 16777216
int cl_bal_marginals(cl_chrom* c, int32_t ignore_diags, int64_t* b0, int64_t* nb, int64_t* n_used);
int cl_bal_marginals_get(cl_chrom* c, int64_t first, int64_t count, uint64_t* sum, uint32_t* nnz);
int cl_bal_iterate(cl_chrom* c, const uint32_t* valid, int32_t max_iters, double tol, int32_t* iters, int32_t* converged, double* var,
                   double* scale);
int cl_bal_weights_get(cl_chrom* c, int64_t first, int64_t count, double* weight);
int cl_bal_cells_get(cl_chrom* c, int64_t first, int64_t count, double* balanced);
int cl_bal_free(cl_chrom* c);

int cl_exp_diagonals(cl_chrom* c, const uint32_t* valid, int32_t balanced, int64_t* nd, int64_t* n_used);
int cl_exp_diagonals_get(cl_chrom* c, int64_t first, int64_t count, int64_t* n_pairs, uint64_t* cnt_sum, double* val_sum);
int cl_exp_set(cl_chrom* c, const double* expected, int64_t count);
int cl_exp_cells_get(cl_chrom* c, int64_t first, int64_t count, double* oe);
int cl_exp_free(cl_chrom* c);

#define CL_EIG_MAX 6
#define CL_EIG_BLOCK 8
#define CL_EIG_BINS_MAX 1048576
int cl_eig_build(cl_chrom* c, double clip, int64_t dmax, int64_t* n_valid, int64_t* n_in);
int cl_eig_apply(cl_chrom* c, const double* x, int32_t n_vec, double* y);
int cl_eig_iterate(cl_chrom* c, int32_t n_eigs, int32_t max_iters, double tol, int32_t* iters, int32_t* converged, double* eigval,
                   double* resid);
int cl_eig_vectors_get(cl_chrom* c, int32_t which, int64_t first, int64_t count, double* v);
int cl_eig_free(cl_chrom* c);

typedef struct cl_conv cl_conv;
#define CL_ERR_PARSE        -8
#define CL_CONV_HICPRO       0
#define CL_CONV_JUICER       1
#define CL_CONV_PAIRS        2
#define CL_CONV_E_FIELDS     1
#define CL_CONV_E_INT        2
#define CL_CONV_E_RANGE      3
#define CL_CONV_E_LONG       4
#define CL_CONV_BUDGET_MAX   (1LL << 30)
int cl_conv_create(int device, void* stream, int32_t format, int64_t ext, int64_t budget, cl_conv** out);
int cl_conv_feed(cl_conv* c, const char* bytes, int64_t n, int32_t last, int64_t* consumed, int64_t* n_lines,
                 int64_t* n_bytes);
int cl_conv_render(cl_conv* c, char* out, int64_t cap, int64_t* n_bytes);
int cl_conv_error(cl_conv* c, int64_t* line, int32_t* kind);
int cl_conv_timing(cl_conv* c, float* ms);
int cl_conv_destroy(cl_conv* c);

typedef struct cl_ingest cl_ingest;
typedef struct cl_ingest_name {
    uint64_t hash;
    uint32_t first, off, len, pad;
} cl_ingest_name;
#define CL_INGEST_TIMES 6
#define CL_INGEST_BEDPE 0
#define CL_INGEST_PAIRS 1
int cl_ingest_create(int device, void* stream, int64_t budget, int64_t cut, int32_t want_distances, cl_ingest** out);
int cl_ingest_set_format(cl_ingest* c, int32_t format, int64_t ext);
int cl_ingest_feed(cl_ingest* c, const char* bytes, int64_t n, int64_t* n_lines, int64_t* first_exotic, int64_t* n_names);
int cl_ingest_error(cl_ingest* c, int64_t* line, int32_t* kind);
int cl_ingest_headers(cl_ingest* c, int64_t* n);
int cl_ingest_names(cl_ingest* c, cl_ingest_name* out, int64_t cap, int64_t* n);
int cl_ingest_commit(cl_ingest* c, int64_t chunk, int64_t line0, const uint64_t* hashes, const int32_t* ids,
                     const uint32_t* name_off, const uint32_t* name_len, int32_t n_table, const char* names,
                     int64_t names_bytes, int32_t n_ids, int64_t* counts, int32_t* status);
int cl_ingest_finish(cl_ingest* c, cl_ingest* other, int32_t n_ids, int32_t unique, int64_t* n_rows, int64_t* n_distances);
int cl_ingest_rows(cl_ingest* c, int32_t id, int64_t* a, int64_t* b, int64_t cap);
int cl_ingest_chrom_arrays(cl_ingest* c, int32_t id, int64_t* n, void** x, void** y);
int cl_ingest_distances(cl_ingest* c, int64_t* out, int64_t cap);
int cl_ingest_timing(cl_ingest* c, float* ms);
int cl_ingest_destroy(cl_ingest* c);

const int32_t* cl_labels_device(const cl_chrom* c);

int cl_cand_reset(cl_chrom* c);
int cl_cluster_pairs_async(cl_chrom* c, int variant, int32_t eps, int32_t min_pts, int32_t cut, int32_t* pinned_pairs_out,
                           int64_t capacity_pairs);
int64_t cl_last_n_labelled(const cl_chrom* c);
int cl_cluster_rowmask_async(cl_chrom* c, int variant, int32_t eps, int32_t min_pts, int32_t cut, void* pinned_out,
                             int64_t capacity_labels);
void cl_set_pairs_defer(cl_chrom* c, int enabled);
int cl_pairs_sync(cl_chrom* c);

int cl_cluster_step_async(cl_chrom* c, int variant, int32_t eps, int32_t min_pts, int32_t cut, int32_t step, int64_t fine_lo);
int cl_step_result(cl_chrom* c, int64_t* n_inter, int64_t* n_self, cl_dsummary* out);
int cl_cand_append(cl_chrom* c, int32_t step, int64_t* n_inter, int64_t* n_self);
int cl_cand_finish(cl_chrom* c, int32_t final_cut, int32_t* boxes_out, int64_t capacity, int64_t* n_out);
int cl_cand_finish_device(cl_chrom* c, int32_t final_cut, const int32_t** dev_rows_out, int64_t* n_out);

void cl_set_table_export(cl_chrom* c, int enabled);

void cl_set_device_labels(cl_chrom* c, int enabled);

void cl_set_profiling(cl_chrom* c, int enabled);
int cl_get_timing(const cl_chrom* c, cl_timing* out);

int cl_sweep_plan(cl_chrom* c, const int32_t* eps, int32_t n_eps, const int32_t* min_pts, int32_t n_min_pts);

void cl_set_layout_reuse(cl_chrom* c, int enabled);

void cl_set_sort_index(cl_chrom* c, int mode);

void cl_set_eps_list(cl_chrom* c, const int32_t* eps, int32_t n);
int cl_chrom_drop_indexes(cl_chrom* c);
void cl_set_count_reuse(cl_chrom* c, int enabled);
void cl_set_count_floor(cl_chrom* c, int32_t min_pts);
void cl_set_count_thresholds(cl_chrom* c, const int32_t* min_pts, int32_t n);
int cl_last_region_mode(const cl_chrom* c);

void cl_set_traversal(cl_chrom* c, int level);

void* cl_stream_create(int device);
int cl_chrom_set_stream(cl_chrom* c, void* stream);
void cl_stream_destroy(void* stream);

void* cl_host_alloc(int64_t bytes);
void cl_host_free(void* p);

int cl_chrom_subsample(cl_chrom* src, const int64_t* rows, int64_t m, cl_chrom** out);

void cl_debug_arena_overcommit(int64_t extra_bytes);

int cl_version(void);

#ifdef __cplusplus
}
#endif
#endif
```

Before: 15.61 billion PETs/s.

## Floor the cached base layout to drop rows below half the first cut

When a sweep is planned and the fine layout applies, the base layout built for reuse across cut thresholds now excludes PETs whose distance falls below half the current cut. A per-fine-strip dead count plus exclusive scan shifts strip starts and destinations, and all base-consuming kernels (cut copy, region counting, list building, word mapping) use the reduced row count. This shrinks memory traffic and work in every later sweep step on the base layout. The layout is rebuilt if a later cut drops below the floor, and the change adds bookkeeping that must stay consistent across many call sites.

```diff
diff --git a/cloops_amd/_lib.py b/cloops_amd/_lib.py
--- a/cloops_amd/_lib.py
+++ b/cloops_amd/_lib.py
@@ -87,6 +87,7 @@
     "cl_last_n_labelled": (_i64, [_vp]),
     "cl_last_n_in": (_i64, [_vp]),
     "cl_last_region_mode": (_int, [_vp]),
+    "cl_base_rows": (_i64, [_vp]),
     "cl_get_boxes": (_int, [_vp, _vp]),
     "cl_boxes_host": (_vp, [_vp]),
     "cl_labels_device": (_vp, [_vp]),
diff --git a/cloops_amd/api.py b/cloops_amd/api.py
--- a/cloops_amd/api.py
+++ b/cloops_amd/api.py
@@ -204,6 +204,9 @@
 
     def last_region_mode(self):
         return int(self._lib.cl_last_region_mode(self._h))
+
+    def base_rows(self):
+        return int(self._lib.cl_base_rows(self._h))
 
     def set_layout_reuse(self, on=True):
         self._lib.cl_set_layout_reuse(self._h, 1 if on else 0)
diff --git a/cloops_amd/csrc/cl_chrom.h b/cloops_amd/csrc/cl_chrom.h
--- a/cloops_amd/csrc/cl_chrom.h
+++ b/cloops_amd/csrc/cl_chrom.h
@@ -75,6 +75,7 @@
     int qindex_layout = -1;
     struct Fine {
         DevBuf q, sp, row, strip;
+        DevBuf dead;
         int w = 0;
         int valid_w = 0, layout = -1;
         GridParams g;
@@ -109,8 +110,12 @@
         DevBuf q, sp, row, strip, tile, key;
         bool valid = false; int layout = -1, eps = 0;
         bool key_valid = false;
-        void invalidate() { valid = false; key_valid = false; }
+        int floor_q = 0;
+        int rows = 0;
+        long long pad_rows = -1;
+        void invalidate() { valid = false; key_valid = false; floor_q = 0; }
     } base;
+    bool sweep_planned = false;
     DevBuf sel_tmp;
     struct Counts {
         bool valid = false;
@@ -285,6 +290,9 @@
     hipLaunchKernelGGL(kernel, dim3(nblocks(nthreads)), dim3(TPB), 0, c->stream, __VA_ARGS__)
 
 static inline void run_begin(cl_chrom* c) { c->run = cl_chrom::Run(); }
+static inline int base_rows(const cl_chrom* c) { return c->base.valid ? c->base.rows : (int)c->n; }
+#define CL_FLOOR_NUM 1
+#define CL_FLOOR_DEN 2
 
 struct RunGuard {
     cl_chrom* c; bool armed = true;
diff --git a/cloops_amd/csrc/cloops_hip.hip b/cloops_amd/csrc/cloops_hip.hip
--- a/cloops_amd/csrc/cloops_hip.hip
+++ b/cloops_amd/csrc/cloops_hip.hip
@@ -235,12 +235,26 @@
     __host__ __device__ __forceinline__ bool operator<(const SplitOut& o) const { return q < o.q; }
 };
 
-__global__ void k_strips_from_fine(int S, int s0, int k, int F, int f0, const int* __restrict__ fstrip, int n, int* __restrict__ strip_start)
+__global__ void k_fine_dead(int F, int floor_q, const int* __restrict__ fstrip, const int* __restrict__ fq, int* __restrict__ dead)
+{
+    const int f = blockIdx.x * blockDim.x + threadIdx.x;
+    if (f > F) return;
+    int lo = 0, b = 0;
+    if (f < F) {
+        b = lo = fstrip[f];
+        int hi = fstrip[f + 1];
+        while (lo < hi) { const int mid = (int)(((unsigned)lo + (unsigned)hi) >> 1); if (fq[mid] < floor_q) lo = mid + 1; else hi = mid; }
+    }
+    dead[f] = lo - b;
+}
+__global__ void k_strips_from_fine(int S, int s0, int k, int F, int f0, const int* __restrict__ fstrip, int rows, int* __restrict__ strip_start,
+                                   const int* __restrict__ deadpre )
 {
     const int s = blockIdx.x * blockDim.x + threadIdx.x;
     if (s > S + 1) return;
     const long long f = (long long)k * ((long long)s + s0) - f0;
-    strip_start[s] = s >= S ? n : fstrip[(int)std::min<long long>(std::max<long long>(f, 0), F)];
+    const int fc = (int)std::min<long long>(std::max<long long>(f, 0), F);
+    strip_start[s] = s >= S ? rows : fstrip[fc] - (deadpre ? deadpre[fc] : 0);
 }
 #define LFF_T 1024
 #define LFF_CAP 4096
@@ -248,7 +262,8 @@
 #define LFF_PAD 512
 __global__ void __launch_bounds__(256)
 k_layout_from_fine(int n, GridParams g, GridParams gf, int k, unsigned kmagic, int qb, const int* __restrict__ fq, const int* __restrict__ fsp, const u32* __restrict__ frow,
-                   const int* __restrict__ fstrip, int* __restrict__ dq, int* __restrict__ dsp, u32* __restrict__ drow, int* __restrict__ dtile)
+                   const int* __restrict__ fstrip, int* __restrict__ dq, int* __restrict__ dsp, u32* __restrict__ drow, int* __restrict__ dtile,
+                   int floor_q, const int* __restrict__ deadpre )
 {
     __shared__ int lq[LFF_CAP + LFF_PAD];
     const int t0 = blockIdx.x * LFF_T, t1 = min(n, t0 + LFF_T);
@@ -263,6 +278,7 @@
         in[e] = i < t1;
         const int ic = in[e] ? i : t0;
         q[e] = fq[ic]; row[e] = frow[ic]; spf[e] = fsp[ic];
+        in[e] = in[e] && q[e] >= floor_q;
     }
     const int sb_first = (((fsp[t0] >> gf.rbits) + gf.s0) / k) * k - gf.s0, sb_last = (((fsp[t1 - 1] >> gf.rbits) + gf.s0) / k) * k - gf.s0;
     const int f_first = max(sb_first, 0), f_end = min(sb_last + k, gf.S);
@@ -293,6 +309,7 @@
         r[e] = fabs - sabs * k;
         fbase[e] = sabs * k - gf.s0;
         dst[e] = in[e] ? fst(max(fbase[e], 0)) + (i - fst(f)) : 0;
+        if (deadpre && in[e]) dst[e] -= deadpre[min(fbase[e] + k, gf.S)];
     }
 #ifdef CLOOPS_DEVEL
     const int kk_abl = (g.dbg2 & (1 << 12)) ? 0 : k;
@@ -1840,6 +1857,7 @@
 extern "C" void cl_set_count_reuse(cl_chrom* c, int enabled) { if (c) { c->reuse_counts = enabled != 0; c->rc.invalidate(); } }
 extern "C" void cl_set_traversal(cl_chrom* c, int level) { if (c) { c->traversal = level < 0 ? 0 : (level > 4 ? 4 : level); c->rc.invalidate(); } }
 extern "C" int cl_last_region_mode(const cl_chrom* c) { return c ? c->last_k2_mode : 0; }
+extern "C" int64_t cl_base_rows(const cl_chrom* c) { return c ? (int64_t)base_rows(c) : -1; }
 extern "C" int cl_chrom_drop_indexes(cl_chrom* c)
 {
     if (!c) return fail(CL_ERR_ARG, "null chromosome handle");
@@ -1903,6 +1921,7 @@
     for (int k = 0; k < n_min_pts; ++k) if (min_pts[k] <= 0) return fail(CL_ERR_ARG, "cl_sweep_plan: minPts must be positive");
     if (c->slot[0].pending || c->slot[1].pending) return fail(CL_ERR_ARG, "cl_sweep_plan: a run is in flight");
     cl_set_count_thresholds(c, min_pts, n_min_pts);
+    c->sweep_planned = n_eps > 0;
     int distinct = 0;
     for (int k = 0; k < n_eps; ++k) { bool seen = false; for (int j = 0; j < k; ++j) seen |= eps[j] == eps[k]; distinct += seen ? 0 : 1; }
     if (distinct > 1) { cl_set_sort_index(c, 1); cl_set_eps_list(c, eps, n_eps); }
@@ -2149,7 +2168,7 @@
 }
 template <bool BAND>
 __global__ void __launch_bounds__(CMP_TPB)
-k_cut_copy(int n, int S, int rbits, int thr, const int* __restrict__ bq, const int* __restrict__ bsp, const u32* __restrict__ brow,
+k_cut_copy(int n , int nbase , int S, int rbits, int thr, const int* __restrict__ bq, const int* __restrict__ bsp, const u32* __restrict__ brow,
            const int* __restrict__ src0, const int* __restrict__ sloc, const int* __restrict__ sboffs ,
            int* __restrict__ strip_start ,
            int* __restrict__ sv, int* __restrict__ sa, u32* __restrict__ srow, int* __restrict__ tile_s0, int* __restrict__ d_M,
@@ -2173,8 +2192,8 @@
 #pragma unroll
     for (int k = 0; k < CMP_PER; ++k) {
         const int i = base + k * CMP_TPB + (int)threadIdx.x;
-        q[k] = i < n ? bq[i] : INT_MIN;
-        keep[k] = i < n && q[k] >= thr;
+        q[k] = i < nbase ? bq[i] : INT_MIN;
+        keep[k] = i < nbase && q[k] >= thr;
     }
 #pragma unroll
     for (int k = 0; k < CMP_PER; ++k) {
@@ -2201,7 +2220,7 @@
         const int st = sloc[u] + sboffs[u >> 8];
         strip_start[u] = st;
         if (poff_out || poff_ref) {
-            const int po = (u < S ? src0[u] : n) - st;
+            const int po = (u < S ? src0[u] : nbase) - st;
             if (poff_out) poff_out[u] = po; else D_out[u] = po - poff_ref[u];
         }
     }
@@ -2410,8 +2429,9 @@
 }
 
 static int sort_layout(cl_chrom* c, const GridParams& g, int* dsv, int* dsa, u32* drow ,
-                       int* dstrip, int* dtile)
-{
+                       int* dstrip, int* dtile, int floor_q = 0, int floor_rows = 0, bool* floored = nullptr)
+{
+    if (floored) *floored = false;
     const int n = (int)c->n;
     const int sh = g.qbits + g.rbits, strip_bits = std::max(1, bits_for((unsigned)g.S));
     const int layout = (g.variant == CL_VARIANT_CDBSCAN2 ? 2 : 0) | (g.swap ? 1 : 0);
@@ -2471,11 +2491,28 @@
                 if (c->fine.w > 0) {
                     const GridParams& gf = c->fine.g;
                     const int k = g.eps / fw;
-                    LAUNCH(k_strips_from_fine, g.S + 2, g.S, g.s0, k, gf.S, gf.s0, (const int*)c->fine.strip.as<int>(), n, dstrip);
+                    int rows_kept = n;
+                    const int* deadpre = nullptr;
+                    if (floor_q > 0 && floored) {
+                        const size_t nf = (size_t)gf.S + 1;
+                        if ((rc = c->fine.dead.ensure(2 * nf * 4))) return rc;
+                        int* dead = c->fine.dead.as<int>();
+                        int* dpre = dead + nf;
+                        size_t need = 0;
+                        hipError_t e = rocprim::exclusive_scan(nullptr, need, dead, dpre, 0, nf, rocprim::plus<int>(), c->stream);
+                        if (e != hipSuccess) return fail(CL_ERR_HIP, "exclusive_scan size query (layout floor)", hipGetErrorString(e));
+                        if (need > c->scan_tmp.bytes && (rc = c->scan_tmp.ensure(need))) return rc;
+                        LAUNCH(k_fine_dead, gf.S + 1, gf.S, floor_q, (const int*)c->fine.strip.as<int>(), (const int*)c->fine.q.as<int>(), dead);
+                        size_t tb = c->scan_tmp.bytes;
+                        e = rocprim::exclusive_scan(c->scan_tmp.p, tb, dead, dpre, 0, nf, rocprim::plus<int>(), c->stream);
+                        if (e != hipSuccess) return fail(CL_ERR_HIP, "exclusive_scan (layout floor)", hipGetErrorString(e));
+                        deadpre = dpre; rows_kept = floor_rows; *floored = true;
+                    }
+                    LAUNCH(k_strips_from_fine, g.S + 2, g.S, g.s0, k, gf.S, gf.s0, (const int*)c->fine.strip.as<int>(), rows_kept, dstrip, deadpre);
                     int qb = bits_for((unsigned)std::min<long long>((long long)gf.qtop + 1, 0x7fffffffLL));
                     if (qb > 28) qb = 0;
                     hipLaunchKernelGGL(k_layout_from_fine, dim3(nblocks(n, LFF_T)), dim3(256), 0, c->stream, n, g, gf, k, (unsigned)(((1ull << 32) + (unsigned)k - 1ull) / (unsigned)k), qb, (const int*)c->fine.q.as<int>(),
-                                       (const int*)c->fine.sp.as<int>(), (const u32*)c->fine.row.as<u32>(), (const int*)c->fine.strip.as<int>(), dsv, dsa, rows, dtile);
+                                       (const int*)c->fine.sp.as<int>(), (const u32*)c->fine.row.as<u32>(), (const int*)c->fine.strip.as<int>(), dsv, dsa, rows, dtile, deadpre ? floor_q : 0, deadpre);
                     HIP_TRY(hipGetLastError());
                     c->run.srow = rows;
                     return CL_OK;
@@ -2537,30 +2574,44 @@
         c->run.sv = wsv; c->run.sa = wsa; c->run.strip = c->strip.as<int>(); c->run.tile = c->tile_s0.as<int>();
     } else {
         const int layout = (g.variant == CL_VARIANT_CDBSCAN2 ? 2 : 0) | (g.swap ? 1 : 0);
-        if (!c->base.valid || c->base.layout != layout || c->base.eps != g.eps) {
+        const long long dmin = g.swap ? c->st.amin : 0;
+        const bool on_base = g.cut <= 0 || (g.swap && (long long)g.cut <= dmin);
+        const int thr_new = on_base ? 0 : g.cut - g.V0;
+        const bool same_base = c->base.valid && c->base.layout == layout && c->base.eps == g.eps;
+        if (!same_base || thr_new < c->base.floor_q) {
             c->base.invalidate();
             c->rc.invalidate();
             if ((rc = c->base.q.ensure(((size_t)n + 2 * SORT_PAD) * 4)) || (rc = c->base.sp.ensure(((size_t)n + 2 * SORT_PAD) * 4)) ||
                 (rc = c->base.row.ensure((size_t)n * 4)) || (rc = c->base.strip.ensure(((size_t)g.S + 2) * 4)) ||
                 (rc = c->base.tile.ensure(((size_t)n / 256 + 2) * 4))) return rc;
-            if (c->base.q.fresh || c->base.sp.fresh) {
-                hipLaunchKernelGGL(k_init_pads, dim3(nblocks(2 * SORT_PAD)), dim3(TPB), 0, c->stream, c->base.q.as<int>(), c->base.sp.as<int>(), (long long)n);
-                c->base.q.fresh = c->base.sp.fresh = false;
+            int floor_q = 0, floor_rows = n;
+            const long long fd = (long long)g.cut * CL_FLOOR_NUM / CL_FLOOR_DEN;
+            const int fw = c->fine.w;
+            if (!same_base && !on_base && !exact && c->sweep_planned && g.swap && fw > 0 && g.eps % fw == 0 && g.eps / fw <= CL_FINE_KMAX &&
+                fd < DCUM_BINS && !c->dcum.empty() && fd - g.V0 > 0) {
+                floor_q = (int)(fd - g.V0);
+                floor_rows = (int)(n - c->dcum[(size_t)fd]);
             }
             GridParams g0 = g;
             g0.cut = 0;
+            bool floored = false;
             if ((rc = sort_layout(c, g0, c->base.q.as<int>() + SORT_PAD, c->base.sp.as<int>() + SORT_PAD, c->base.row.as<u32>(),
-                                  c->base.strip.as<int>(), c->base.tile.as<int>()))) return rc;
+                                  c->base.strip.as<int>(), c->base.tile.as<int>(), floor_q, floor_rows, &floored))) return rc;
+            c->base.floor_q = floored ? floor_q : 0;
+            c->base.rows = floored ? floor_rows : n;
+            if (c->base.q.fresh || c->base.sp.fresh || c->base.pad_rows != c->base.rows) {
+                hipLaunchKernelGGL(k_init_pads, dim3(nblocks(2 * SORT_PAD)), dim3(TPB), 0, c->stream, c->base.q.as<int>(), c->base.sp.as<int>(), (long long)c->base.rows);
+                c->base.q.fresh = c->base.sp.fresh = false;
+                c->base.pad_rows = c->base.rows;
+            }
             c->base.valid = true; c->base.layout = layout; c->base.eps = g.eps;
         } else {
             ev_record(c, 0);
             ev_record(c, 1);
         }
-        const long long dmin = g.swap ? c->st.amin : 0;
-        const bool on_base = g.cut <= 0 || (g.swap && (long long)g.cut <= dmin);
+        const int nbase = c->base.rows;
         const int m1 = g.minPts - 1;
         const bool cacheable = !exact && c->reuse_counts && g.swap && m1 >= 1 && m1 <= 127;
-        const int thr_new = on_base ? 0 : g.cut - g.V0;
         enum { RC_NONE, RC_MAKE, RC_SAME, RC_REMAP } rcmode = RC_NONE;
         const bool want4 = level_cap >= 4 && cacheable;
         if (cacheable) {
@@ -2625,7 +2676,7 @@
             c->run.strip = c->base.strip.as<int>(); c->run.tile = c->base.tile.as<int>();
         } else {
             if (!g.swap) return fail(CL_ERR_ARG, "internal: layout reuse needs the v-band layout");
-            const int nb = nblocks(n, CMP_BLOCK);
+            const int nb = nblocks(std::max(1, nbase), CMP_BLOCK);
             const int nblk = nblocks(g.S + 1, 256);
             if ((rc = c->sel_tmp.ensure(((size_t)g.S + 2) * 8 + ((size_t)nblk + 2) * 8 + 64))) return rc;
             int* sloc = c->sel_tmp.as<int>();
@@ -2660,12 +2711,12 @@
             } else
             if (rcmode == RC_REMAP) {
                 const int nbb = nblocks(nblocks(g.S, KB_SB), CMP_TPB / 64);
-                hipLaunchKernelGGL(k_cut_copy<true>, dim3(nbb + nb), dim3(CMP_TPB), 0, c->stream, n, g.S, g.rbits, thr, bq, (const int*)(c->base.sp.as<int>() + SORT_PAD),
+                hipLaunchKernelGGL(k_cut_copy<true>, dim3(nbb + nb), dim3(CMP_TPB), 0, c->stream, n, nbase, g.S, g.rbits, thr, bq, (const int*)(c->base.sp.as<int>() + SORT_PAD),
                                    (const u32*)c->base.row.as<u32>(), (const int*)src0, (const int*)sloc, (const int*)sboffs, c->strip.as<int>(), wsv, wsa, c->vals_out.as<u32>(), c->tile_s0.as<int>(),
                                    d_M, c->run.m_exact ? c->run.m : -1, c->counters.as<int>(), (int*)nullptr, (const int*)c->rc.poff.as<int>(), c->rc.D.as<int>(),
                                    nbb, (const int2*)c->rc.blen.as<int2>(), c->cnt.as<int>(), g.eps, g.minPts, g.dbg);
             } else
-            hipLaunchKernelGGL(k_cut_copy<false>, dim3(nb), dim3(CMP_TPB), 0, c->stream, n, g.S, g.rbits, thr, bq, (const int*)(c->base.sp.as<int>() + SORT_PAD),
+            hipLaunchKernelGGL(k_cut_copy<false>, dim3(nb), dim3(CMP_TPB), 0, c->stream, n, nbase, g.S, g.rbits, thr, bq, (const int*)(c->base.sp.as<int>() + SORT_PAD),
                                (const u32*)c->base.row.as<u32>(), (const int*)src0, (const int*)sloc, (const int*)sboffs, c->strip.as<int>(), wsv, wsa, c->vals_out.as<u32>(), c->tile_s0.as<int>(),
                                d_M, c->run.m_exact ? c->run.m : -1, c->counters.as<int>(), rcmode == RC_MAKE ? c->rc.poff.as<int>() : (int*)nullptr,
                                (const int*)nullptr, (int*)nullptr, 0, (const int2*)nullptr, (int*)nullptr, 0, 0, 0);
@@ -2680,8 +2731,10 @@
         GridParams g0 = gk;
         g0.cut = 0;
         g0.qmin = c->rc.thr;
-        rc = cl_launch_region(c->stream, g0, n, n, false, c->base.q.as<int>() + SORT_PAD, c->base.sp.as<int>() + SORT_PAD, c->base.strip.as<int>(), c->base.tile.as<int>(),
-                              c->rc.cnt.as<int>());
+        const int nbase = c->base.rows;
+        if (nbase > 0)
+            rc = cl_launch_region(c->stream, g0, nbase, nbase, false, c->base.q.as<int>() + SORT_PAD, c->base.sp.as<int>() + SORT_PAD, c->base.strip.as<int>(),
+                                  c->base.tile.as<int>(), c->rc.cnt.as<int>());
         c->slot[c->cur].n_queried = c->run.m;
     } else if (!k2_skip && !k2_band && !SKIP(256)) {
         rc = cl_launch_region(c->stream, gk, n, c->run.m, exact, c->run.sv, c->run.sa, c->run.strip, c->run.tile, c->run.cnt);
diff --git a/cloops_amd/csrc/k_lists.hip b/cloops_amd/csrc/k_lists.hip
--- a/cloops_amd/csrc/k_lists.hip
+++ b/cloops_amd/csrc/k_lists.hip
@@ -1810,10 +1810,10 @@
 
 int lists_base_keys(cl_chrom* c, const GridParams& g)
 {
-    const int n = (int)c->n;
-    int rc = c->base.key.ensure((size_t)n * 4);
+    const int n = base_rows(c);
+    int rc = c->base.key.ensure((size_t)c->n * 4);
     if (rc) return rc;
-    hipLaunchKernelGGL(k_base_keys, dim3(nblocks(n, LT)), dim3(256), 0, c->stream, g, n, (const int*)(c->base.q.as<int>() + SORT_PAD),
+    if (n > 0) hipLaunchKernelGGL(k_base_keys, dim3(nblocks(n, LT)), dim3(256), 0, c->stream, g, n, (const int*)(c->base.q.as<int>() + SORT_PAD),
                        (const int*)(c->base.sp.as<int>() + SORT_PAD), (const u32*)c->base.row.as<u32>(), c->base.key.as<int>());
     HIP_TRY(hipGetLastError());
     return CL_OK;
@@ -1822,11 +1822,11 @@
 int lists_build_base(cl_chrom* c, const GridParams& g, int nm, ListRun* out)
 {
     fuse_knob(c);
-    const int n = (int)c->n;
+    const int n = base_rows(c);
     ListBufs b;
-    int rc = list_bufs(c, g, n, &b);
+    int rc = list_bufs(c, g, std::max(1, n), &b);
     if (rc) return rc;
-    const int nblk = nblocks(n, LT);
+    const int nblk = nblocks(std::max(1, n), LT);
     const bool v2 = g.variant == CL_VARIANT_CDBSCAN2;
     ListRun L{};
     list_views(c, b, &L);
@@ -1880,8 +1880,8 @@
 
 int lists_words_to_base(cl_chrom* c, const GridParams& g)
 {
-    const int n = (int)c->n;
-    LAUNCH(k_words_to_base, n, g, n, (const int*)(c->base.sp.as<int>() + SORT_PAD), (const int4*)c->l_tab.as<int4>(), (const int*)c->rc.poff.as<int>(),
+    const int n = base_rows(c);
+    if (n > 0) LAUNCH(k_words_to_base, n, g, n, (const int*)(c->base.sp.as<int>() + SORT_PAD), (const int4*)c->l_tab.as<int4>(), (const int*)c->rc.poff.as<int>(),
            (const int*)c->cnt.as<int>(), c->rc.cnt.as<int>());
     HIP_TRY(hipGetLastError());
     return CL_OK;
@@ -1940,7 +1940,7 @@
 #ifdef CLOOPS_DEVEL
     { const char* e = getenv("CLOOPS_BCAP"); if (e) kcap = atoi(e); queued = kcap > 0; e = getenv("CLOOPS_BQG"); if (e) bqg = atoi(e); }
 #endif
-    const int nt = nblocks(L.npos, (g.variant == CL_VARIANT_CDBSCAN1 || !queued) ? BNT : BNQ);
+    const int nt = nblocks(std::max(1, L.npos), (g.variant == CL_VARIANT_CDBSCAN1 || !queued) ? BNT : BNQ);
 #define LB_ARGS g, nt, L.npos, L.lcnt, L.cmask, L.cgrank, L.wgrank, (const int2*)L.cpair, (const int*)croot_of(c), (const int*)c->cellfirst.as<int>(),    \
                 (const int*)L.ckey, (const int*)L.cstrip, (const int2*)L.wpair, (const int*)L.wpos, (const int*)L.wenc, (const int*)c->compkey.as<int>(),                    \
                 (const int*)c->ncore.as<int>(), c->owner.as<int>(), c->bsize.as<int>(), c->usize.as<int>(), c->chainflag.as<int>() ,  \
@@ -2104,7 +2104,7 @@
         } else if (which == 1) {
             launch_make_lists(c, g, nblk, b, L);
         } else if (which == 6 || which == 7) {
-            const int n = (int)c->n;
+            const int n = std::max(1, base_rows(c));
             ListBufs bb;
             if ((rc = list_bufs(c, g, n, &bb))) return rc;
             const int nb4 = nblocks(n, LT);
@@ -2124,11 +2124,11 @@
         } else if (which == 4 || which == 3 || which == 5) {
             ListRun L2 = L;
             c->run.level = c->traversal >= 4 ? 4 : 3;
-            if (c->run.level == 4) { ListBufs bb; if ((rc = list_bufs(c, g, (int)c->n, &bb))) return rc; list_views(c, bb, &L2); L2.npos = (int)c->n; L2.pstrip = c->base.strip.as<int>(); }
+            if (c->run.level == 4) { ListBufs bb; if ((rc = list_bufs(c, g, std::max(1, base_rows(c)), &bb))) return rc; list_views(c, bb, &L2); L2.npos = base_rows(c); L2.pstrip = c->base.strip.as<int>(); }
             else { L2.npos = nm; L2.pstrip = c->run.strip; }
             if (which == 4) { if ((rc = lists_border(c, g, nm, L2))) return rc; }
             else if (which == 3) {
-                ListBufs bb; if ((rc = list_bufs(c, g, c->run.level == 4 ? (int)c->n : nm, &bb))) return rc;
+                ListBufs bb; if ((rc = list_bufs(c, g, c->run.level == 4 ? std::max(1, base_rows(c)) : nm, &bb))) return rc;
                 fuse_knob(c);
                 if (c->fuse_chains)
                     hipLaunchKernelGGL(k_prep_c, dim3(nblocks(std::max(nm, g.S + 2))), dim3(TPB), 0, c->stream, g, (const int*)L2.lcnt, (const int*)L2.pstrip,
diff --git a/include/cloops_hip.h b/include/cloops_hip.h
--- a/include/cloops_hip.h
+++ b/include/cloops_hip.h
@@ -249,6 +249,7 @@
 void cl_set_count_floor(cl_chrom* c, int32_t min_pts);
 void cl_set_count_thresholds(cl_chrom* c, const int32_t* min_pts, int32_t n);
 int cl_last_region_mode(const cl_chrom* c);
+int64_t cl_base_rows(const cl_chrom* c);
 
 void cl_set_traversal(cl_chrom* c, int level);
 
```

Measured after the change: 16.44 billion PETs/s, median of 6. 5.3% higher.
